# microsoft/SEAL

Hardware: AMD Instinct MI355X
Metric: CKKS multiply+relinearize+rescale ciphertexts/sec @ N=2^16, L=16 (higher is better)
Workload: dtype u64

## Files before the change

include/sealhip.h:

```cpp
#ifndef SEALHIP_H
#define SEALHIP_H

#include <stdbool.h>
#include <stddef.h>
#include <stdint.h>

#ifdef __cplusplus
extern "C" {
#endif

typedef long SHL_HRESULT;
#define SHL_S_OK ((SHL_HRESULT)0L)
#define SHL_S_FALSE ((SHL_HRESULT)1L)
#define SHL_E_POINTER ((SHL_HRESULT)0x80004003L)
#define SHL_E_INVALIDARG ((SHL_HRESULT)0x80070057L)
#define SHL_E_OUTOFMEMORY ((SHL_HRESULT)0x8007000EL)
#define SHL_E_UNEXPECTED ((SHL_HRESULT)0x8000FFFFL)
#define SHL_COR_E_IO ((SHL_HRESULT)0x80131620L)
#define SHL_COR_E_INVALIDOPERATION ((SHL_HRESULT)0x80131509L)
#define SHL_E_INVALID_INDEX ((SHL_HRESULT)0x80070585L)

#define SHL_FUNC SHL_HRESULT


// ... 195 lines not shown
SHL_FUNC ItemMap_Info(void *thisptr, uint64_t *rows, uint64_t *terms, uint64_t *longest_row, uint64_t *first_batch, uint64_t *second_batch);
SHL_FUNC Evaluator_SumItemsMapped(void *thisptr, void *encrypted, void *item_map, void *destination);
SHL_FUNC Evaluator_DotPlainMapped(void *thisptr, void *encrypted, const uint64_t *device_plain, uint64_t plain_count, void *item_map,
                                  double scale, void *destination);
SHL_FUNC Evaluator_DotItemsMapped(void *thisptr, void *encrypted1, void *encrypted2, void *item_map, void *destination);
SHL_FUNC CKKSEncoder_EncodeScalars(void *thisptr, uint64_t count, const double *values, uint64_t *parms_id, double scale, uint64_t *device_words);
SHL_FUNC CKKSEncoder_EncodeIntegerScalars(void *thisptr, uint64_t count, const int64_t *values, uint64_t *parms_id, uint64_t *device_words);
SHL_FUNC Evaluator_LiftScalars(void *thisptr, uint64_t count, const uint64_t *values_mod_t, uint64_t *parms_id, uint64_t *device_words);
SHL_FUNC Evaluator_DotScalarsDevice(void *thisptr, void *encrypted, const uint64_t *device_scalars, uint64_t rows, uint64_t batch, double scale,
                                    void *destination);
SHL_FUNC Evaluator_Square(void *thisptr, void *encrypted, void *destination, void *pool);
SHL_FUNC Evaluator_Relinearize(void *thisptr, void *encrypted, void *relinKeys, void *destination, void *pool);
SHL_FUNC Evaluator_ModSwitchToNext1(void *thisptr, void *encrypted, void *destination, void *pool);
SHL_FUNC Evaluator_ModSwitchTo1(void *thisptr, void *encrypted, uint64_t *parms_id, void *destination, void *pool);
SHL_FUNC Evaluator_RescaleToNext(void *thisptr, void *encrypted, void *destination, void *pool);
SHL_FUNC Evaluator_RescaleTo(void *thisptr, void *encrypted, uint64_t *parms_id, void *destination, void *pool);
SHL_FUNC Evaluator_ModReduceToNext(void *thisptr, void *encrypted, void *destination, void *pool);
SHL_FUNC Evaluator_ModReduceTo(void *thisptr, void *encrypted, uint64_t *parms_id, void *destination, void *pool);
SHL_FUNC Evaluator_TransformToNTT2(void *thisptr, void *encrypted, void *destination_ntt);
SHL_FUNC Evaluator_TransformFromNTT(void *thisptr, void *encrypted_ntt, void *destination);
SHL_FUNC Evaluator_ApplyGalois(void *thisptr, void *encrypted, uint32_t galois_elt, void *galoisKeys, void *destination, void *pool);
SHL_FUNC Evaluator_RotateRows(void *thisptr, void *encrypted, int steps, void *galoisKeys, void *destination, void *pool);
SHL_FUNC Evaluator_RotateColumns(void *thisptr, void *encrypted, void *galois_keys, void *destination, void *pool);
SHL_FUNC Evaluator_RotateVector(void *thisptr, void *encrypted, int steps, void *galoisKeys, void *destination, void *pool);
SHL_FUNC Evaluator_ComplexConjugate(void *thisptr, void *encrypted, void *galoisKeys, void *destination, void *pool);
SHL_FUNC Evaluator_ContextUsingKeyswitching(void *thisptr, bool *using_keyswitching);

SHL_FUNC Evaluator_SwitchKeyAccWords(void *thisptr, void *encrypted, uint64_t *words);
SHL_FUNC Evaluator_RelinearizePartial(void *thisptr, void *encrypted , void *relinKeys, uint64_t digit_first,
                                      uint64_t digit_count, uint64_t *device_acc);
SHL_FUNC Evaluator_RelinearizeFinish(void *thisptr, void *encrypted, uint64_t *device_acc, uint64_t parts);
SHL_FUNC Evaluator_ApplyGaloisPartial(void *thisptr, void *encrypted , uint32_t galois_elt, void *galoisKeys,
                                      uint64_t digit_first, uint64_t digit_count, uint64_t *device_acc);
SHL_FUNC Evaluator_ApplyGaloisFinish(void *thisptr, void *encrypted, uint64_t *device_acc, uint64_t parts);

SHL_FUNC Comm_GetUniqueId(uint8_t *id128);
SHL_FUNC Comm_RcclAvailable(bool *available);
SHL_FUNC Comm_Create(const uint8_t *id128, int nranks, int rank, void **comm);
SHL_FUNC Comm_Destroy(void *comm);
SHL_FUNC Comm_Info(void *comm, int *nranks, int *rank, bool *loopback);
SHL_FUNC Comm_DigitRange(void *comm, uint64_t digits, uint64_t *first, uint64_t *count);
SHL_FUNC Comm_AllReduceWords(void *comm, uint64_t *device_words, uint64_t count, void *hip_stream);
SHL_FUNC Comm_BroadcastWords(void *comm, uint64_t *device_words, uint64_t count, int root, void *hip_stream);
SHL_FUNC Evaluator_RelinearizeDigitParallel(void *thisptr, void *encrypted, void *relinKeys, void *comm, int exchange, void *destination);
SHL_FUNC Evaluator_ApplyGaloisDigitParallel(void *thisptr, void *encrypted, uint32_t galois_elt, void *galoisKeys, void *comm, int exchange,
                                            void *destination);
SHL_FUNC Evaluator_RotateVectorDigitParallel(void *thisptr, void *encrypted, int steps, void *galoisKeys, void *comm, int exchange,
                                             void *destination);
SHL_FUNC Evaluator_BroadcastKeyDigits(void *thisptr, void *kswitch_keys, uint64_t index, uint64_t *device_staging, void *comm, int root);
SHL_FUNC Evaluator_SwitchKeySlots(void *thisptr, void *encrypted, uint64_t nranks, uint64_t *slots);
SHL_FUNC Evaluator_SwitchKeyPackTargets(void *thisptr, void *encrypted, const uint64_t *device_acc, uint64_t nranks, uint64_t *device_send,
                                        uint64_t *device_special);
SHL_FUNC Evaluator_SwitchKeyFinishOwned(void *thisptr, void *encrypted, const uint64_t *device_recv, const uint64_t *device_special,
                                        uint64_t nranks, uint64_t rank, uint64_t *device_own);
SHL_FUNC Evaluator_SwitchKeyAddGathered(void *thisptr, void *encrypted, const uint64_t *device_all, uint64_t nranks);


SHL_FUNC shl_ntt_forward(void *context, uint64_t *data, uint64_t polys, uint64_t comps, uint64_t first_prime, int lazy, void *stream);
SHL_FUNC shl_ntt_inverse(void *context, uint64_t *data, uint64_t polys, uint64_t comps, uint64_t first_prime, int lazy, void *stream);
SHL_FUNC shl_dyadic_product(void *context, const uint64_t *a, const uint64_t *b, uint64_t *r, uint64_t polys, uint64_t comps, uint64_t first_prime, void *stream);
SHL_FUNC shl_reduce_items(void *context, uint64_t chain_index, const uint64_t *a, const uint64_t *plain, uint64_t *r, uint64_t size,
                          uint64_t batch, uint64_t group, uint64_t slices, uint64_t *scratch, uint64_t *slices_used, void *stream);
SHL_FUNC shl_reduce_flush_intervals(uint64_t *sum_terms, uint64_t *dot_terms);
SHL_FUNC shl_dot_items(void *context, uint64_t chain_index, const uint64_t *x, const uint64_t *y, uint64_t *r, uint64_t batch,
                       uint64_t group, uint64_t slices, uint64_t *scratch, uint64_t *slices_used, void *stream);
SHL_FUNC shl_dot_items_flush_interval(uint64_t *items);
SHL_FUNC shl_reduce_mapped(void *context, uint64_t chain_index, int kind, const uint64_t *a, uint64_t a_batch, const uint64_t *b,
                           uint64_t b_batch, uint64_t *r, uint64_t size, void *item_map, uint64_t slices, uint64_t *scratch,
                           uint64_t *slices_used, void *stream);
SHL_FUNC shl_dot_scalars(void *context, uint64_t chain_index, const uint64_t *a, const uint64_t *scalars, uint64_t *r, uint64_t size,
                         uint64_t rows, uint64_t batch, uint64_t slices, uint64_t *slices_used);
SHL_FUNC shl_dot_scalars_tile(void *context, uint64_t chain_index, const uint64_t *a, const uint64_t *scalars, uint64_t *r, uint64_t size,
                              uint64_t rows, uint64_t batch, uint64_t slices, uint64_t *slices_used, uint64_t row_tile, void *stream);
SHL_FUNC shl_dot_scalars_info(uint64_t *row_tile, uint64_t *flush);
SHL_FUNC shl_apply_galois(void *context, uint64_t chain_index, int ntt_form, uint32_t galois_elt, const uint64_t *in, uint64_t *out, uint64_t polys, void *stream);
SHL_FUNC shl_rns_stage(void *context, uint64_t chain_index, int which, const uint64_t *in, uint64_t *out, uint64_t polys, void *stream);
SHL_FUNC Ciphertext_Create4(void *context, uint64_t *parms_id, void *pool, void **cipher);
SHL_FUNC Ciphertext_Create5(void *context, uint64_t *parms_id, uint64_t capacity, void *pool, void **cipher);
SHL_FUNC Ciphertext_Reserve1(void *thisptr, void *context, uint64_t *parms_id, uint64_t size_capacity);
SHL_FUNC Ciphertext_Reserve2(void *thisptr, void *context, uint64_t size_capacity);
SHL_FUNC Ciphertext_Reserve3(void *thisptr, uint64_t size_capacity);
SHL_FUNC Ciphertext_SizeCapacity(void *thisptr, uint64_t *size_capacity);
SHL_FUNC Ciphertext_SetParmsId(void *thisptr, uint64_t *parms_id);
SHL_FUNC Ciphertext_Resize2(void *thisptr, void *context, uint64_t size);
SHL_FUNC Ciphertext_Resize3(void *thisptr, uint64_t size);
SHL_FUNC Ciphertext_Resize4(void *thisptr, uint64_t size, uint64_t polyModulusDegree, uint64_t coeffModCount);
SHL_FUNC Ciphertext_GetDataAt1(void *thisptr, uint64_t index, uint64_t *data);
SHL_FUNC Ciphertext_GetDataAt2(void *thisptr, uint64_t poly_index, uint64_t coeff_index, uint64_t *data);
SHL_FUNC Ciphertext_SetDataAt(void *thisptr, uint64_t index, uint64_t value);
SHL_FUNC Ciphertext_Release(void *thisptr);
SHL_FUNC KSwitchKeys_Create2(void *copy, void **kswitch_keys);
SHL_FUNC KSwitchKeys_Set(void *thisptr, void *assign);
SHL_FUNC KSwitchKeys_RawSize(void *thisptr, uint64_t *key_count);
SHL_FUNC KSwitchKeys_GetKeyList(void *thisptr, uint64_t index, uint64_t *count, void **key_list);
SHL_FUNC KSwitchKeys_ClearDataAndReserve(void *thisptr, uint64_t size);
SHL_FUNC KSwitchKeys_AddKeyList(void *thisptr, uint64_t count, void **key_list);
SHL_FUNC KSwitchKeys_GetParmsId(void *thisptr, uint64_t *parms_id);
SHL_FUNC KSwitchKeys_SetParmsId(void *thisptr, uint64_t *parms_id);
SHL_FUNC SEALContext_ParametersSet(void *thisptr, bool *params_set);
SHL_FUNC SEALContext_ParameterErrorName(void *thisptr, char *outstr, uint64_t *length);
SHL_FUNC SEALContext_ParameterErrorMessage(void *thisptr, char *outstr, uint64_t *length);
SHL_FUNC SEALContext_KeyContextData(void *thisptr, void **context_data);
SHL_FUNC SEALContext_FirstContextData(void *thisptr, void **context_data);
SHL_FUNC SEALContext_LastContextData(void *thisptr, void **context_data);
SHL_FUNC SEALContext_GetContextData(void *thisptr, uint64_t *parms_id, void **context_data);
SHL_FUNC ContextData_Destroy(void *thisptr);
SHL_FUNC ContextData_TotalCoeffModulus(void *thisptr, uint64_t *count, uint64_t *total_coeff_modulus);
SHL_FUNC ContextData_TotalCoeffModulusBitCount(void *thisptr, int *bit_count);
SHL_FUNC ContextData_Parms(void *thisptr, void **parms);
SHL_FUNC ContextData_Qualifiers(void *thisptr, void **epq);
SHL_FUNC ContextData_CoeffDivPlainModulus(void *thisptr, uint64_t *count, uint64_t *coeff_div);
SHL_FUNC ContextData_PlainUpperHalfThreshold(void *thisptr, uint64_t *puht);
SHL_FUNC ContextData_PlainUpperHalfIncrement(void *thisptr, uint64_t *count, uint64_t *puhi);
SHL_FUNC ContextData_UpperHalfThreshold(void *thisptr, uint64_t *count, uint64_t *uht);
SHL_FUNC ContextData_UpperHalfIncrement(void *thisptr, uint64_t *count, uint64_t *uhi);
SHL_FUNC ContextData_PrevContextData(void *thisptr, void **prev_data);
SHL_FUNC ContextData_NextContextData(void *thisptr, void **next_data);
SHL_FUNC ContextData_ChainIndex(void *thisptr, uint64_t *index);
SHL_FUNC ContextData_ParmsId(void *thisptr, uint64_t *parms_id);
SHL_FUNC EPQ_Destroy(void *thisptr);
SHL_FUNC EPQ_ParametersSet(void *thisptr, bool *parameters_set);
SHL_FUNC EPQ_UsingFFT(void *thisptr, bool *using_fft);
SHL_FUNC EPQ_UsingNTT(void *thisptr, bool *using_ntt);
SHL_FUNC EPQ_UsingBatching(void *thisptr, bool *using_batching);
SHL_FUNC EPQ_UsingFastPlainLift(void *thisptr, bool *using_fast_plain_lift);
SHL_FUNC EPQ_UsingDescendingModulusChain(void *thisptr, bool *using_descending_modulus_chain);
SHL_FUNC EPQ_SecLevel(void *thisptr, int *sec_level);
SHL_FUNC EncParams_Create2(void *copy, void **enc_params);
SHL_FUNC EncParams_Set(void *thisptr, void *assign);
SHL_FUNC EncParams_GetParmsId(void *thisptr, uint64_t *parms_id);
SHL_FUNC EncParams_GetPlainModulus(void *thisptr, uint64_t *plain_modulus);
SHL_FUNC EncParams_Equals(void *thisptr, void *otherptr, bool *result);
SHL_FUNC EncParams_SaveSize(void *thisptr, uint8_t compr_mode, int64_t *result);
SHL_FUNC EncParams_Save(void *thisptr, uint8_t *outptr, uint64_t size, uint8_t compr_mode, int64_t *out_bytes);
SHL_FUNC EncParams_Load(void *thisptr, uint8_t *inptr, uint64_t size, int64_t *in_bytes);
SHL_FUNC SecretKey_Create2(void *copy, void **secret_key);
SHL_FUNC SecretKey_Assign(void *thisptr, void *assign);
SHL_FUNC SecretKey_ParmsId(void *thisptr, uint64_t *parms_id);
SHL_FUNC SecretKey_SaveSize(void *thisptr, uint8_t compr_mode, int64_t *result);
SHL_FUNC SecretKey_Save(void *thisptr, uint8_t *outptr, uint64_t size, uint8_t compr_mode, int64_t *out_bytes);
SHL_FUNC PublicKey_Create2(void *copy, void **public_key);
SHL_FUNC PublicKey_Assign(void *thisptr, void *assign);
SHL_FUNC PublicKey_ParmsId(void *thisptr, uint64_t *parms_id);
SHL_FUNC PublicKey_SaveSize(void *thisptr, uint8_t compr_mode, int64_t *result);
SHL_FUNC PublicKey_Save(void *thisptr, uint8_t *outptr, uint64_t size, uint8_t compr_mode, int64_t *out_bytes);
SHL_FUNC SealHip_ReleasePool(void);
SHL_FUNC SealHip_SetStagedHostCopies(bool enabled);
SHL_FUNC SealHip_PoolStats(uint64_t *bytes_held, uint64_t *cross_stream_waits);
SHL_FUNC SealHip_InstallAbortTrace(const char *path);
SHL_FUNC SealHip_KsChunkStats(uint64_t *calls, uint64_t *chunks, uint64_t *scratch_bytes_max);
SHL_FUNC SealHip_TailStats(uint64_t *folded, uint64_t *plain, uint64_t *dropped);
SHL_FUNC SealHip_ProductStats(uint64_t *fused, uint64_t *formed, uint64_t *dropped);
SHL_FUNC SealHip_GaloisStats(uint64_t *gathered, uint64_t *permuted);
SHL_FUNC SealHip_XofStats(uint64_t *polynomials, uint64_t *replaced_words, uint64_t *host_walk_ns, uint64_t *total_ns);
SHL_FUNC shl_device_count(int *count);
SHL_FUNC shl_set_device(int device);
SHL_FUNC shl_stream_create(bool non_blocking, void **hip_stream);
SHL_FUNC shl_stream_destroy(void *hip_stream);
SHL_FUNC shl_malloc(uint64_t bytes, void **device_ptr);
SHL_FUNC shl_free(void *device_ptr);
SHL_FUNC shl_memcpy_h2d(void *device_dst, const void *host_src, uint64_t bytes);
SHL_FUNC KeyGenerator_Create1(void *context, const uint64_t *seed8, void **key_generator);
SHL_FUNC KeyGenerator_Create2(void *context, void *secret_key, const uint64_t *seed8, void **key_generator);
SHL_FUNC KeyGenerator_Destroy(void *thisptr);
SHL_FUNC KeyGenerator_SecretKey(void *thisptr, void *secret_key);
SHL_FUNC KeyGenerator_CreatePublicKey(void *thisptr, void *public_key);
SHL_FUNC KeyGenerator_CreateRelinKeys(void *thisptr, void *relin_keys);
SHL_FUNC KeyGenerator_CreateGaloisKeysFromElts(void *thisptr, uint64_t count, const uint32_t *galois_elts, void *galois_keys);
SHL_FUNC KeyGenerator_CreateGaloisKeysFromSteps(void *thisptr, uint64_t count, const int *steps, void *galois_keys);
SHL_FUNC KeyGenerator_CreateGaloisKeysAll(void *thisptr, void *galois_keys);
SHL_FUNC KeyGenerator_SeededSaveSize(void *thisptr, bool galois, uint64_t key_count, int64_t *result);
SHL_FUNC KeyGenerator_CreateRelinKeysSave(void *thisptr, uint8_t *outptr, uint64_t size, int64_t *out_bytes);
SHL_FUNC KeyGenerator_CreateGaloisKeysFromEltsSave(void *thisptr, uint64_t count, const uint32_t *galois_elts, uint8_t *outptr, uint64_t size,
                                                   int64_t *out_bytes);
SHL_FUNC KeyGenerator_KeyToHost(void *thisptr, uint32_t galois_elt, uint64_t *host_words, uint64_t capacity_words);
SHL_FUNC SecretKey_Get(void *thisptr, uint64_t *host_words);
SHL_FUNC PublicKey_Get(void *thisptr, uint64_t *host_words);
SHL_FUNC shl_memcpy_d2h(void *host_dst, const void *device_src, uint64_t bytes);
SHL_FUNC shl_device_synchronize(void);
SHL_FUNC shl_timer_create(void **timer);
SHL_FUNC shl_timer_destroy(void *timer);
SHL_FUNC shl_timer_start(void *timer, void *stream);
SHL_FUNC shl_timer_stop(void *timer, void *stream, float *milliseconds);

#ifdef __cplusplus
}
#endif
#endif
```

seal_amd/__init__.py:

```python
from .api import (CoeffModulus, PlainModulus, EncryptionParameters, SEALContext, ContextData, Ciphertext, Plaintext, KSwitchKeys,
                  RelinKeys, GaloisKeys, Evaluator, SecretKey, PublicKey, KeyGenerator, Decryptor, Encryptor, BatchEncoder, CKKSEncoder, Graph, ItemMap, DeviceBuffer, HipTimer, ntt_forward, ntt_inverse,
                  dyadic_product, apply_galois, rns_stage, device_synchronize, device_info, release_pool, pool_stats, tail_stats, product_stats, galois_stats, ks_chunk_stats, xof_stats, Stream, Comm, device_count, set_device,
                  set_staged_host_copies, install_abort_trace)
from ._native import SealHipError, InvalidArgument, LogicError, OutOfRange, DeviceError, load

__all__ = [
    "CoeffModulus", "PlainModulus", "EncryptionParameters", "SEALContext", "ContextData", "Ciphertext", "Plaintext", "KSwitchKeys",
    "RelinKeys", "GaloisKeys", "Evaluator", "SecretKey", "PublicKey", "KeyGenerator", "Decryptor", "Encryptor", "BatchEncoder", "CKKSEncoder", "Graph", "ItemMap", "DeviceBuffer", "HipTimer", "ntt_forward", "ntt_inverse",
    "dyadic_product", "apply_galois", "rns_stage", "device_synchronize", "device_info", "release_pool", "pool_stats", "tail_stats", "product_stats", "galois_stats", "ks_chunk_stats", "xof_stats", "Stream", "Comm", "device_count", "set_device", "set_staged_host_copies", "install_abort_trace", "SealHipError",
    "InvalidArgument", "LogicError", "OutOfRange", "DeviceError", "load",
]
```

seal_amd/_native.py:

```python
import ctypes as C
import os

_HERE = os.path.dirname(os.path.abspath(__file__))
DEFAULT_LIB = os.path.join(_HERE, "lib", "libsealhip.so")

S_OK = 0
E_POINTER = 0x80004003
E_INVALIDARG = 0x80070057
E_OUTOFMEMORY = 0x8007000E
E_UNEXPECTED = 0x8000FFFF
COR_E_IO = 0x80131620
COR_E_INVALIDOPERATION = 0x80131509
E_INVALID_INDEX = 0x80070585


class SealHipError(Exception):

    def __init__(self, hr, message):
        super().__init__("%s (HRESULT 0x%08X)" % (message, hr & 0xFFFFFFFF))
        self.hresult = hr & 0xFFFFFFFF
        self.message = message


class InvalidArgument(SealHipError, ValueError):
    pass


class LogicError(SealHipError, RuntimeError):
    pass


class OutOfRange(SealHipError, IndexError):
    pass


class DeviceError(SealHipError, OSError):
    pass


_ERR = {E_INVALIDARG: InvalidArgument, COR_E_INVALIDOPERATION: LogicError, E_INVALID_INDEX: OutOfRange,
        COR_E_IO: DeviceError}

SYMBOLS = """
SealHip_Version SealHip_DeviceInfo SealHip_LastError CoeffModulus_Create1 PlainModulus_Batching
EncParams_Create1 EncParams_Destroy EncParams_SetPolyModulusDegree EncParams_GetPolyModulusDegree
EncParams_SetCoeffModulus EncParams_GetCoeffModulus EncParams_SetPlainModulus2 EncParams_GetScheme
SEALContext_Create SEALContext_Destroy SEALContext_KeyParmsId SEALContext_FirstParmsId SEALContext_LastParmsId
SEALContext_UsingKeyswitching SEALContext_ChainIndex SEALContext_ParmsIdAt SEALContext_CoeffModulusAt
SEALContext_TotalCoeffModulusBitCount SEALContext_SetParmsId SEALContext_NTTRoot SEALContext_BaseBsk
Ciphertext_Create3 Ciphertext_CreateBatch Ciphertext_Create2 Ciphertext_Set Ciphertext_Destroy Ciphertext_Resize1
Ciphertext_Size Ciphertext_BatchCount Ciphertext_PolyModulusDegree Ciphertext_CoeffModulusSize Ciphertext_ParmsId
Ciphertext_IsNTTForm Ciphertext_SetIsNTTForm Ciphertext_Scale Ciphertext_SetScale Ciphertext_CorrectionFactor
Ciphertext_SetCorrectionFactor Ciphertext_IsTransparent Ciphertext_DevicePtr Ciphertext_CopyFromHost
Ciphertext_CopyToHost Ciphertext_CopyWordsToHost Ciphertext_CopyFromDevice
Ciphertext_SaveSize Ciphertext_Save Ciphertext_UnsafeLoad Ciphertext_Load Ciphertext_LoadItem Ciphertext_SaveItem
KSwitchKeys_UnsafeLoad KSwitchKeys_Load KSwitchKeys_SaveSize KSwitchKeys_Save
KeyGenerator_Create1 KeyGenerator_Create2 KeyGenerator_Destroy KeyGenerator_SecretKey KeyGenerator_CreatePublicKey
KeyGenerator_CreateRelinKeys KeyGenerator_CreateGaloisKeysFromSteps KeyGenerator_CreateGaloisKeysAll KeyGenerator_CreateGaloisKeysFromElts KeyGenerator_KeyToHost KeyGenerator_SeededSaveSize KeyGenerator_CreateRelinKeysSave KeyGenerator_CreateGaloisKeysFromEltsSave SecretKey_Get PublicKey_Get
SecretKey_Create SecretKey_Destroy SecretKey_Set SecretKey_UnsafeLoad SecretKey_Load Decryptor_Create Decryptor_Destroy
Decryptor_Decrypt Decryptor_InvariantNoiseBudget Decryptor_DecryptBatchWords Decryptor_DecryptBatch
CKKSEncoder_Create CKKSEncoder_Destroy CKKSEncoder_SlotCount CKKSEncoder_Encode1 CKKSEncoder_Encode2 CKKSEncoder_Encode3 CKKSEncoder_Encode4 CKKSEncoder_Encode5 CKKSEncoder_Decode1 CKKSEncoder_Decode2
CKKSEncoder_EncodeDevice CKKSEncoder_DecodeDevice
BatchEncoder_Create BatchEncoder_Destroy BatchEncoder_GetSlotCount BatchEncoder_Encode1 BatchEncoder_Encode2 BatchEncoder_Decode1
BatchEncoder_Decode2 BatchEncoder_EncodeDevice BatchEncoder_DecodeDevice
PublicKey_Create PublicKey_Destroy PublicKey_Set PublicKey_UnsafeLoad PublicKey_Load Encryptor_Encrypt Encryptor_EncryptZero1 Encryptor_EncryptZero2 Encryptor_EncryptZeroSymmetric2
Encryptor_Create Encryptor_Destroy Encryptor_SetSeed Encryptor_EncryptZeroSymmetric1 Encryptor_EncryptSymmetric
Encryptor_SymmetricSaveSize Encryptor_EncryptZeroSymmetricSave Encryptor_EncryptSymmetricSave
Encryptor_EncryptSymmetricDevice Encryptor_EncryptDevice
Plaintext_Create1 Plaintext_Create5 Plaintext_Destroy Plaintext_Set4 Plaintext_SetFromDevice Plaintext_CoeffCount
Plaintext_IsNTTForm Plaintext_GetParmsId Plaintext_SetParmsId Plaintext_Scale Plaintext_SetScale Plaintext_CopyToHost
Plaintext_SaveSize Plaintext_Save Plaintext_UnsafeLoad Plaintext_Load
Evaluator_AddMany Evaluator_AddPlain Evaluator_SubPlain Evaluator_MultiplyMany Evaluator_MultiplyPlain Evaluator_Exponentiate
Evaluator_TransformToNTT1 Evaluator_ModSwitchToNext2 Evaluator_ModSwitchTo2
Evaluator_AddPlainDevice Evaluator_SubPlainDevice Evaluator_MultiplyPlainDevice Evaluator_TransformPlainToNTTDevice
Evaluator_SumItems Evaluator_DotPlainDevice shl_reduce_items shl_reduce_flush_intervals
Evaluator_DotItems shl_dot_items shl_dot_items_flush_interval
ItemMap_Create ItemMap_Destroy ItemMap_Info Evaluator_SumItemsMapped Evaluator_DotPlainMapped Evaluator_DotItemsMapped shl_reduce_mapped
CKKSEncoder_EncodeScalars CKKSEncoder_EncodeIntegerScalars Evaluator_LiftScalars Evaluator_DotScalarsDevice
shl_dot_scalars shl_dot_scalars_tile shl_dot_scalars_info
KSwitchKeys_Create1 KSwitchKeys_Destroy KSwitchKeys_Size KSwitchKeys_SetKey KSwitchKeys_SetKeyFromDevice
KSwitchKeys_SetKeyDigits KSwitchKeys_HasKey KSwitchKeys_DeviceBytes RelinKeys_GetIndex GaloisKeys_GetIndex GaloisTool_GetEltFromStep
Evaluator_Create Evaluator_Destroy Evaluator_SetStream Evaluator_Synchronize Evaluator_CopyTo Evaluator_SetTransparentCheck
Evaluator_BeginCapture Evaluator_EndCapture Evaluator_LaunchGraph Graph_Destroy
Evaluator_Negate Evaluator_Add Evaluator_Sub Evaluator_Multiply Evaluator_Square Evaluator_Relinearize
Evaluator_ModSwitchToNext1 Evaluator_ModSwitchTo1 Evaluator_RescaleToNext Evaluator_RescaleTo
Evaluator_ModReduceToNext Evaluator_ModReduceTo Evaluator_TransformToNTT2 Evaluator_TransformFromNTT Evaluator_ApplyGalois
Evaluator_RotateRows Evaluator_RotateColumns Evaluator_RotateVector Evaluator_ComplexConjugate
Evaluator_ContextUsingKeyswitching
Evaluator_SwitchKeyAccWords Evaluator_RelinearizePartial Evaluator_RelinearizeFinish Evaluator_ApplyGaloisPartial
Evaluator_ApplyGaloisFinish
Comm_GetUniqueId Comm_RcclAvailable Comm_Create Comm_Destroy Comm_Info Comm_DigitRange Comm_AllReduceWords Comm_BroadcastWords
Evaluator_RelinearizeDigitParallel Evaluator_ApplyGaloisDigitParallel Evaluator_RotateVectorDigitParallel
Evaluator_BroadcastKeyDigits Evaluator_SwitchKeySlots Evaluator_SwitchKeyPackTargets Evaluator_SwitchKeyFinishOwned
Evaluator_SwitchKeyAddGathered
SealHip_ReleasePool SealHip_PoolStats SealHip_TailStats SealHip_ProductStats SealHip_GaloisStats SealHip_XofStats SealHip_KsChunkStats SealHip_SetStagedHostCopies SealHip_InstallAbortTrace shl_stream_create shl_stream_destroy shl_device_count shl_set_device
shl_ntt_forward shl_ntt_inverse shl_dyadic_product shl_apply_galois shl_rns_stage shl_malloc shl_free
shl_memcpy_h2d shl_memcpy_d2h shl_device_synchronize shl_timer_create shl_timer_destroy shl_timer_start
shl_timer_stop
Ciphertext_Create4 Ciphertext_Create5 Ciphertext_GetDataAt1 Ciphertext_GetDataAt2 Ciphertext_Release Ciphertext_Reserve1
Ciphertext_Reserve2 Ciphertext_Reserve3 Ciphertext_Resize2 Ciphertext_Resize3 Ciphertext_Resize4 Ciphertext_SetDataAt
Ciphertext_SetParmsId Ciphertext_SizeCapacity ContextData_ChainIndex ContextData_CoeffDivPlainModulus ContextData_Destroy ContextData_NextContextData
ContextData_Parms ContextData_ParmsId ContextData_PlainUpperHalfIncrement ContextData_PlainUpperHalfThreshold ContextData_PrevContextData ContextData_Qualifiers
ContextData_TotalCoeffModulus ContextData_TotalCoeffModulusBitCount ContextData_UpperHalfIncrement ContextData_UpperHalfThreshold EPQ_Destroy EPQ_ParametersSet
EPQ_SecLevel EPQ_UsingBatching EPQ_UsingDescendingModulusChain EPQ_UsingFFT EPQ_UsingFastPlainLift EPQ_UsingNTT
EncParams_Create2 EncParams_Equals EncParams_GetParmsId EncParams_GetPlainModulus EncParams_Load EncParams_Save
EncParams_SaveSize EncParams_Set KSwitchKeys_AddKeyList KSwitchKeys_ClearDataAndReserve KSwitchKeys_Create2 KSwitchKeys_GetKeyList
KSwitchKeys_GetParmsId KSwitchKeys_RawSize KSwitchKeys_Set KSwitchKeys_SetParmsId PublicKey_Assign PublicKey_Create2
PublicKey_ParmsId PublicKey_Save PublicKey_SaveSize SEALContext_FirstContextData SEALContext_GetContextData SEALContext_KeyContextData
SEALContext_LastContextData SEALContext_ParameterErrorMessage SEALContext_ParameterErrorName SEALContext_ParametersSet SecretKey_Assign SecretKey_Create2
SecretKey_ParmsId SecretKey_Save SecretKey_SaveSize
""".split()

_lib = None
_lib_path = None


def load(path=None):
    global _lib, _lib_path
    want = os.path.abspath(path or DEFAULT_LIB)
    if _lib is not None and _lib_path == want:
        return _lib
    if not os.path.exists(want):
        raise ImportError(
            "seal_amd: %s not found. Build it with `python -c 'import __graft_entry__ as g; g.build()'` "
            "(hipcc --offload-arch=gfx950). There is no CPU fallback." % want)
    lib = C.CDLL(want)
    for name in SYMBOLS:
        getattr(lib, name).restype = C.c_long
    _lib, _lib_path = lib, want
    return lib


def lib():
    return _lib if _lib is not None else load()


def check(hr):
    hr &= 0xFFFFFFFF
    if hr == S_OK:
        return
    n = C.c_uint64(0)
    lib().SealHip_LastError(None, C.byref(n))
    buf = C.create_string_buffer(max(int(n.value), 1))
    lib().SealHip_LastError(buf, C.byref(n))
    cls = _ERR.get(hr, SealHipError)
    if hr == E_OUTOFMEMORY:
        raise MemoryError(buf.value.decode())
    raise cls(hr, buf.value.decode(errors="replace"))
```

seal_amd/api.py:

```python
import ctypes as C
import os

import numpy as np

from . import _native as N

SCHEME = {"none": 0, "bfv": 1, "ckks": 2, "bgv": 3}


def _p(a):
    return a.ctypes.data_as(C.c_void_p)


class CoeffModulus:
    @staticmethod
    def Create(poly_modulus_degree, bit_sizes):
        bits = (C.c_int * len(bit_sizes))(*bit_sizes)
        out = np.zeros(len(bit_sizes), dtype=np.uint64)
        N.check(N.lib().CoeffModulus_Create1(C.c_uint64(poly_modulus_degree), C.c_uint64(len(bit_sizes)), bits, _p(out)))
        return [int(x) for x in out]


class PlainModulus:
    @staticmethod
# ... 1569 lines not shown
        N.check(N.lib().Comm_AllReduceWords(self._h, C.c_void_p(device_ptr), C.c_uint64(words), C.c_void_p(stream or 0)))

    def broadcast(self, device_ptr, words, root=0, stream=None):
        N.check(N.lib().Comm_BroadcastWords(self._h, C.c_void_p(device_ptr), C.c_uint64(words), C.c_int(root), C.c_void_p(stream or 0)))


class DeviceBuffer:

    def __init__(self, words):
        self.words = int(words)
        self._ptr = C.c_void_p()
        N.check(N.lib().shl_malloc(C.c_uint64(self.words * 8), C.byref(self._ptr)))

    def __del__(self):
        if getattr(self, "_ptr", None) and self._ptr.value:
            N.lib().shl_free(self._ptr)
            self._ptr = None

    @property
    def ptr(self):
        return self._ptr.value

    @staticmethod
    def from_numpy(a):
        a = np.ascontiguousarray(a, dtype=np.uint64)
        b = DeviceBuffer(a.size)
        N.check(N.lib().shl_memcpy_h2d(b._ptr, _p(a), C.c_uint64(a.size * 8)))
        return b

    def to_numpy(self, shape):
        out = np.zeros(shape, dtype=np.uint64)
        N.check(N.lib().shl_memcpy_d2h(_p(out), self._ptr, C.c_uint64(out.size * 8)))
        return out

    @staticmethod
    def from_array(a):
        a = np.ascontiguousarray(a)
        if a.dtype.itemsize not in (8, 16):
            raise TypeError("from_array takes 8-byte or complex128 elements, not %s" % a.dtype)
        b = DeviceBuffer(max(a.nbytes // 8, 1))
        N.check(N.lib().shl_memcpy_h2d(b._ptr, _p(a), C.c_uint64(a.nbytes)))
        return b

    def to_array(self, shape, dtype=np.float64):
        out = np.zeros(shape, dtype=dtype)
        N.check(N.lib().shl_memcpy_d2h(_p(out), self._ptr, C.c_uint64(out.nbytes)))
        return out


def ntt_forward(context, buf, polys, comps, first_prime=0, lazy=False, stream=None):
    N.check(N.lib().shl_ntt_forward(context._h, C.c_void_p(buf.ptr), C.c_uint64(polys), C.c_uint64(comps),
                                    C.c_uint64(first_prime), C.c_int(int(lazy)), C.c_void_p(stream or 0)))


def ntt_inverse(context, buf, polys, comps, first_prime=0, lazy=False, stream=None):
    N.check(N.lib().shl_ntt_inverse(context._h, C.c_void_p(buf.ptr), C.c_uint64(polys), C.c_uint64(comps),
                                    C.c_uint64(first_prime), C.c_int(int(lazy)), C.c_void_p(stream or 0)))


def dyadic_product(context, a, b, r, polys, comps, first_prime=0, stream=None):
    N.check(N.lib().shl_dyadic_product(context._h, C.c_void_p(a.ptr), C.c_void_p(b.ptr), C.c_void_p(r.ptr),
                                       C.c_uint64(polys), C.c_uint64(comps), C.c_uint64(first_prime),
                                       C.c_void_p(stream or 0)))


def apply_galois(context, chain_index, ntt_form, galois_elt, src, dst, polys, stream=None):
    N.check(N.lib().shl_apply_galois(context._h, C.c_uint64(chain_index), C.c_int(int(ntt_form)), C.c_uint32(galois_elt),
                                     C.c_void_p(src.ptr), C.c_void_p(dst.ptr), C.c_uint64(polys), C.c_void_p(stream or 0)))


RNS_STAGE = {"fastbconv_m_tilde": 0, "sm_mrq": 1, "fast_floor": 2, "fastbconv_sk": 3,
             "divide_and_round_q_last": 4, "divide_and_round_q_last_ntt": 5}


def rns_stage(context, chain_index, which, src, dst, polys, stream=None):
    N.check(N.lib().shl_rns_stage(context._h, C.c_uint64(chain_index), C.c_int(RNS_STAGE[which]), C.c_void_p(src.ptr),
                                  C.c_void_p(dst.ptr), C.c_uint64(polys), C.c_void_p(stream or 0)))


class Stream:

    def __init__(self, non_blocking=True):
        self._h = C.c_void_p()
        N.check(N.lib().shl_stream_create(C.c_bool(non_blocking), C.byref(self._h)))

    @property
    def handle(self):
        return self._h.value

    def __del__(self):
        if getattr(self, "_h", None) and self._h.value:
            N.lib().shl_stream_destroy(self._h)
            self._h = None


def device_count():
    n = C.c_int()
    N.check(N.lib().shl_device_count(C.byref(n)))
    return n.value


def set_device(index):
    N.check(N.lib().shl_set_device(C.c_int(index)))


def release_pool():
    N.check(N.lib().SealHip_ReleasePool())


def set_staged_host_copies(enabled):
    N.check(N.lib().SealHip_SetStagedHostCopies(C.c_bool(enabled)))


def install_abort_trace(path):
    N.check(N.lib().SealHip_InstallAbortTrace(C.c_char_p(os.fsencode(path))))


def pool_stats():
    a, b = C.c_uint64(), C.c_uint64()
    N.check(N.lib().SealHip_PoolStats(C.byref(a), C.byref(b)))
    return a.value, b.value


def tail_stats():
    a, b, c = C.c_uint64(), C.c_uint64(), C.c_uint64()
    N.check(N.lib().SealHip_TailStats(C.byref(a), C.byref(b), C.byref(c)))
    return a.value, b.value, c.value


def product_stats():
    a, b, c = C.c_uint64(), C.c_uint64(), C.c_uint64()
    N.check(N.lib().SealHip_ProductStats(C.byref(a), C.byref(b), C.byref(c)))
    return a.value, b.value, c.value


def galois_stats():
    a, b = C.c_uint64(), C.c_uint64()
    N.check(N.lib().SealHip_GaloisStats(C.byref(a), C.byref(b)))
    return a.value, b.value


def xof_stats():
    v = [C.c_uint64() for _ in range(4)]
    N.check(N.lib().SealHip_XofStats(*[C.byref(x) for x in v]))
    return tuple(x.value for x in v)


def ks_chunk_stats():
    a, b, c = C.c_uint64(), C.c_uint64(), C.c_uint64()
    N.check(N.lib().SealHip_KsChunkStats(C.byref(a), C.byref(b), C.byref(c)))
    return a.value, b.value, c.value


def device_synchronize():
    N.check(N.lib().shl_device_synchronize())


def device_info():
    name = C.create_string_buffer(256)
    cus = C.c_int()
    mem = C.c_uint64()
    N.check(N.lib().SealHip_DeviceInfo(name, C.c_uint64(256), C.byref(cus), C.byref(mem)))
    return name.value.decode(), cus.value, mem.value


class HipTimer:

    def __init__(self):
        self._h = C.c_void_p()
        N.check(N.lib().shl_timer_create(C.byref(self._h)))

    def __del__(self):
        if getattr(self, "_h", None):
            N.lib().shl_timer_destroy(self._h)
            self._h = None

    def start(self, stream=None):
        N.check(N.lib().shl_timer_start(self._h, C.c_void_p(stream or 0)))

    def stop(self, stream=None):
        ms = C.c_float()
        N.check(N.lib().shl_timer_stop(self._h, C.c_void_p(stream or 0), C.byref(ms)))
        return ms.value
```

seal_amd/csrc/capi_kernels.cpp:

```cpp
#include "capi_common.h"
#include "batch_reduce_kernels.h"
#include <memory>

namespace
{
    template <class Launch>
    SHL_HRESULT raw_reduce(void *context, uint64_t chain_index, const char *shape_error, uint64_t grid_planes, uint64_t out_items,
                           const ItemWalk &walk, uint64_t slices, uint64_t *slices_used, const uint64_t *r, bool operands,
                           const uint64_t *scratch, Launch launch)
    {
        IfNullRet(context, SHL_E_POINTER);
        SHL_TRY
        auto c = as<Context>(context);
        auto l = c->level_by_chain_index(chain_index);
        if (!l)
            throw std::out_of_range("chain_index");
        if (shape_error)
            throw std::invalid_argument(shape_error);
        const size_t words = (size_t)l->K * c->n();
        if (!slices)
            slices = batch_reduce_slices(grid_planes * out_items * words / 2, walk);
        if (slices > walk.longest || slices > 64)
            throw std::invalid_argument("1 <= slices <= min(group or longest row, 64)");
        if (slices_used)
// ... 180 lines not shown
        if (hr != SHL_S_OK || !r)
            return hr;
        SHL_TRY
        hip_ok(hipStreamSynchronize(nullptr), "dot_scalars sync");
        SHL_CATCH
    }
    SHL_FUNC shl_dot_scalars_info(uint64_t *row_tile, uint64_t *flush)
    {
        IfNullRet(row_tile, SHL_E_POINTER);
        IfNullRet(flush, SHL_E_POINTER);
        *row_tile = dot_scalars_row_tile();
        *flush = batch_reduce_dot_flush();
        return SHL_S_OK;
    }
    SHL_FUNC shl_apply_galois(
        void *context, uint64_t chain_index, int ntt_form, uint32_t galois_elt, const uint64_t *in, uint64_t *out, uint64_t polys,
        void *stream)
    {
        IfNullRet(context, SHL_E_POINTER);
        IfNullRet(in, SHL_E_POINTER);
        IfNullRet(out, SHL_E_POINTER);
        SHL_TRY
        auto c = as<Context>(context);
        auto l = c->level_by_chain_index(chain_index);
        if (!l)
            throw std::out_of_range("chain_index");
        if (!(galois_elt & 1) || galois_elt >= 2 * c->n())
            throw std::invalid_argument("Galois element is not valid");
        if (in == out)
            throw std::invalid_argument("result cannot point to the same value as operand");
        PlaneGeom g{ (unsigned)c->log_n(), l->K, (unsigned)polys };
        hip_ok(k_apply_galois(c->dev_mods(), in, out, galois_elt, ntt_form, g, 1, (hipStream_t)stream), "apply_galois");
        SHL_CATCH
    }
    SHL_FUNC shl_rns_stage(void *context, uint64_t chain_index, int which, const uint64_t *in, uint64_t *out, uint64_t polys, void *stream)
    {
        IfNullRet(context, SHL_E_POINTER);
        IfNullRet(in, SHL_E_POINTER);
        IfNullRet(out, SHL_E_POINTER);
        SHL_TRY
        auto c = as<Context>(context);
        auto l = c->level_by_chain_index(chain_index);
        if (!l)
            throw std::out_of_range("chain_index");
        hipStream_t s = (hipStream_t)stream;
        const unsigned n_log = (unsigned)c->log_n();
        if (which >= 0 && which <= 3)
        {
            if (c->scheme() != Scheme::bfv)
                throw std::logic_error("BEHZ stages exist only for BFV contexts");
            hip_ok(k_behz_stage(c->dev_mods(), l->dev, which, in, out, n_log, polys, s), "behz stage");
        }
        else if (which == 4)
        {
            if (l->K < 2)
                throw std::invalid_argument("level has a single modulus");
            hip_ok(k_bfv_modswitch(c->dev_mods(), l->dev, in, out, n_log, polys, s), "divide_and_round_q_last");
        }
        else if (which == 5)
        {
            if (l->K < 2)
                throw std::invalid_argument("level has a single modulus");
            const unsigned K = l->K;
            const size_t N = c->n();
            Scratch copy(polys * K * N), tt(polys * (K - 1) * N);
            hip_ok(hipMemcpyAsync(copy.p, in, polys * K * N * 8, hipMemcpyDeviceToDevice, s), "copy");
            uint64_t *last = copy.p + (size_t)(K - 1) * N;
            NttBatch bi{};
            bi.data = last;
            bi.outer_stride = (size_t)K * N;
            bi.ncomp = 1;
            bi.nouter = (unsigned)polys;
            bi.prime_first = K - 1;
            hip_ok(ntt_inverse(c->ntt_tables(), bi, 0, s), "intt last");
            NttBatch b{};
            b.data = tt.p;
            b.outer_stride = (size_t)(K - 1) * N;
            b.ncomp = K - 1;
            b.nouter = (unsigned)polys;
            b.src = last;
            b.src_outer_stride = (size_t)K * N;
            b.src_ncomp = 1;
            b.src_mode = 2;
            b.src_half = l->dev.half_q_last;
            b.src_q = l->dev.q_last;
            b.src_fix = l->dev.round_fix;
            hip_ok(ntt_forward(c->ntt_tables(), b, 1, s), "ntt correction");
            hip_ok(k_rescale_combine(c->dev_mods(), l->dev.inv_q_last_mod_q, copy.p, tt.p, out, n_log, K, polys, s), "combine");
            hip_ok(hipStreamSynchronize(s), "sync");
        }
        else
            throw std::invalid_argument("unknown stage");
        SHL_CATCH
    }
    SHL_FUNC SealHip_SetStagedHostCopies(bool enabled)
    {
        set_staged_host_copies(enabled);
        return SHL_S_OK;
    }
    SHL_FUNC SealHip_ReleasePool(void)
    {
        SHL_TRY
        DevicePool::global().release_all();
        SHL_CATCH
    }
    SHL_FUNC SealHip_PoolStats(uint64_t *bytes_held, uint64_t *cross_stream_waits)
    {
        SHL_TRY
        if (bytes_held)
            *bytes_held = DevicePool::global().bytes_held();
        if (cross_stream_waits)
            *cross_stream_waits = DevicePool::global().cross_stream_waits();
        SHL_CATCH
    }
    SHL_FUNC SealHip_KsChunkStats(uint64_t *calls, uint64_t *chunks, uint64_t *scratch_bytes_max)
    {
        SHL_TRY
        uint64_t w = 0;
        ks_chunk_stats(calls, chunks, &w);
        if (scratch_bytes_max)
            *scratch_bytes_max = w * 8;
        SHL_CATCH
    }
    SHL_FUNC SealHip_XofStats(uint64_t *polynomials, uint64_t *replaced_words, uint64_t *host_walk_ns, uint64_t *total_ns)
    {
        SHL_TRY
        xof_stats(polynomials, replaced_words, host_walk_ns, total_ns);
        SHL_CATCH
    }
    SHL_FUNC SealHip_ProductStats(uint64_t *fused, uint64_t *formed, uint64_t *dropped)
    {
        SHL_TRY
        uint64_t f, p, d;
        lazy_product_stats(f, p, d);
        if (fused)
            *fused = f;
        if (formed)
            *formed = p;
        if (dropped)
            *dropped = d;
        SHL_CATCH
    }
    SHL_FUNC SealHip_GaloisStats(uint64_t *gathered, uint64_t *permuted)
    {
        SHL_TRY
        uint64_t g, p;
        galois_path_stats(g, p);
        if (gathered)
            *gathered = g;
        if (permuted)
            *permuted = p;
        SHL_CATCH
    }
    SHL_FUNC SealHip_TailStats(uint64_t *folded, uint64_t *plain, uint64_t *dropped)
    {
        SHL_TRY
        uint64_t f, p, d;
        lazy_tail_stats(f, p, d);
        if (folded)
            *folded = f;
        if (plain)
            *plain = p;
        if (dropped)
            *dropped = d;
        SHL_CATCH
    }
    SHL_FUNC shl_device_count(int *count)
    {
        IfNullRet(count, SHL_E_POINTER);
        SHL_TRY
        *count = 0;
        if (hipGetDeviceCount(count) != hipSuccess)
            *count = 0;
        SHL_CATCH
    }
    SHL_FUNC shl_set_device(int device)
    {
        SHL_TRY
        hip_ok(hipSetDevice(device), "hipSetDevice");
        SHL_CATCH
    }
    SHL_FUNC shl_stream_create(bool non_blocking, void **hip_stream)
    {
        IfNullRet(hip_stream, SHL_E_POINTER);
        SHL_TRY
        hipStream_t s = nullptr;
        hip_ok(hipStreamCreateWithFlags(&s, non_blocking ? hipStreamNonBlocking : hipStreamDefault), "hipStreamCreateWithFlags");
        *hip_stream = s;
        SHL_CATCH
    }
    SHL_FUNC shl_stream_destroy(void *hip_stream)
    {
        SHL_TRY
        hip_ok(hipStreamSynchronize((hipStream_t)hip_stream), "hipStreamSynchronize");
        hip_ok(hipStreamDestroy((hipStream_t)hip_stream), "hipStreamDestroy");
        SHL_CATCH
    }
    SHL_FUNC shl_malloc(uint64_t bytes, void **device_ptr)
    {
        IfNullRet(device_ptr, SHL_E_POINTER);
        SHL_TRY
        if (hipMalloc(device_ptr, bytes) != hipSuccess)
            throw std::bad_alloc();
        SHL_CATCH
    }
    SHL_FUNC shl_free(void *device_ptr)
    {
        SHL_TRY
        hip_ok(hipFree(device_ptr), "hipFree");
        SHL_CATCH
    }
    SHL_FUNC shl_memcpy_h2d(void *device_dst, const void *host_src, uint64_t bytes)
    {
        SHL_TRY
        hip_ok(hipMemcpy(device_dst, host_src, bytes, hipMemcpyHostToDevice), "H2D");
        SHL_CATCH
    }
    SHL_FUNC shl_memcpy_d2h(void *host_dst, const void *device_src, uint64_t bytes)
    {
        SHL_TRY
        hip_ok(hipDeviceSynchronize(), "sync");
        hip_ok(hipMemcpy(host_dst, device_src, bytes, hipMemcpyDeviceToHost), "D2H");
        SHL_CATCH
    }
    SHL_FUNC shl_device_synchronize(void)
    {
        SHL_TRY
        hip_ok(hipDeviceSynchronize(), "hipDeviceSynchronize");
        SHL_CATCH
    }
    SHL_FUNC shl_timer_create(void **timer)
    {
        IfNullRet(timer, SHL_E_POINTER);
        SHL_TRY
        auto t = new Timer();
        hip_ok(hipEventCreate(&t->e0), "hipEventCreate");
        hip_ok(hipEventCreate(&t->e1), "hipEventCreate");
        *timer = t;
        SHL_CATCH
    }
    SHL_FUNC shl_timer_destroy(void *timer)
    {
        IfNullRet(timer, SHL_E_POINTER);
        auto t = as<Timer>(timer);
        (void)hipEventDestroy(t->e0);
        (void)hipEventDestroy(t->e1);
        delete t;
        return SHL_S_OK;
    }
    SHL_FUNC shl_timer_start(void *timer, void *stream)
    {
        IfNullRet(timer, SHL_E_POINTER);
        SHL_TRY
        hip_ok(hipEventRecord(as<Timer>(timer)->e0, (hipStream_t)stream), "hipEventRecord");
        SHL_CATCH
    }
    SHL_FUNC shl_timer_stop(void *timer, void *stream, float *milliseconds)
    {
        IfNullRet(timer, SHL_E_POINTER);
        IfNullRet(milliseconds, SHL_E_POINTER);
        SHL_TRY
        auto t = as<Timer>(timer);
        hip_ok(hipEventRecord(t->e1, (hipStream_t)stream), "hipEventRecord");
        hip_ok(hipEventSynchronize(t->e1), "hipEventSynchronize");
        hip_ok(hipEventElapsedTime(milliseconds, t->e0, t->e1), "hipEventElapsedTime");
        SHL_CATCH
    }
}
```

seal_amd/csrc/evaluator.h:

```cpp
#pragma once
#include "context.h"
#include "poly_kernels.h"
#include "pool.h"
#include "comm.h"
#include "ntt2_kernels.h"
#include <functional>
#include <map>
#include <memory>
#include <mutex>
#include <stdexcept>
#include <vector>

namespace sealhip
{
    class Evaluator;
    struct LazyTail
    {
        const Evaluator *owner;
        uint64_t *acc;
        bool with_addend = false;
    };
    class Ciphertext;
    struct LazyProduct
    {
        const Evaluator *owner;
        const Ciphertext *x, *y;
        uint64_t *own;
        const uint64_t *xw() const;
        const uint64_t *yw() const;
    };
    void lazy_product_stats(uint64_t &fused, uint64_t &formed, uint64_t &dropped);
    void galois_path_stats(uint64_t &gathered, uint64_t &permuted);
    void lazy_tail_stats(uint64_t &folded, uint64_t &plain, uint64_t &dropped);
    void ks_chunk_stats(uint64_t *calls, uint64_t *chunks, uint64_t *scratch_words_max);

    struct KsPlan
    {
        unsigned chunk;
        unsigned lanes;
        unsigned chunks(unsigned batch) const { return (batch + chunk - 1) / chunk; }
    };
    struct KsRoute
    {
        bool fused = false;
        unsigned split = 1;
        bool fold = false;
        bool defer = false;
        KsPlan plan{ 0, 1 };
        unsigned j0 = 0, j1 = 0;
        bool takes_product() const { return fused && fold && split == 1; }
        bool reads_through_map() const;
    };
    struct KsAddend
    {
        bool folds = false;
        bool c1_zero = false;
        uint32_t galois_elt = 0;
        const uint64_t *c0 = nullptr;
        const LazyProduct *prod = nullptr;
        static KsAddend nothing() { return {}; }
        static KsAddend planes(bool c1_zero_unwritten = false) { return { true, c1_zero_unwritten, 0, nullptr, nullptr }; }
        static KsAddend galois(uint32_t elt, const uint64_t *operand_c0) { return { true, true, elt, operand_c0, nullptr }; }
        static KsAddend product(const LazyProduct &p) { return { true, false, 0, nullptr, &p }; }
    };

    class Ciphertext
    {
    public:
        explicit Ciphertext(const Context &ctx, size_t batch = 1) : ctx_(&ctx), batch_(batch ? batch : 1) {}
        ~Ciphertext();
        Ciphertext(const Ciphertext &o);
        Ciphertext &operator=(const Ciphertext &o);

        const Context &context() const { return *ctx_; }
        size_t batch() const { return batch_; }
        size_t size() const { return size_; }
        const Level *level() const { return level_; }
        size_t coeff_modulus_size() const { return level_ ? level_->K : 0; }
        size_t poly_modulus_degree() const { return level_ ? ctx_->n() : 0; }
        bool &is_ntt_form() { return is_ntt_form_; }
        bool is_ntt_form() const { return is_ntt_form_; }
        double &scale() { return scale_; }
        double scale() const { return scale_; }
        uint64_t &correction_factor() { return correction_factor_; }
        uint64_t correction_factor() const { return correction_factor_; }
        uint64_t *data()
        {
            settle();
            before_write();
            return data_;
        }
        const uint64_t *data() const
        {
            settle();
            return data_;
        }
        size_t plane_words() const { return level_ ? batch_ * level_->K * ctx_->n() : 0; }
        size_t word_count() const { return size_ * plane_words(); }
        uint64_t *plane(size_t p) { return data() + p * plane_words(); }
        const uint64_t *plane(size_t p) const { return data() + p * plane_words(); }
        bool has_lazy_tail() const { return lazy_ != nullptr; }
        bool has_lazy_product() const { return lazy_prod_ != nullptr; }
        bool has_storage() const { return data_ != nullptr; }

        void resize(const Level *level, size_t size, hipStream_t stream);
        void adopt(const Level *level, size_t size, uint64_t *slab, size_t capacity_words);
        void reshape_uninitialized(const Level *level, size_t size);
        size_t capacity_words() const { return capacity_words_; }
        void release();
        void reserve(const Level *level, size_t size_capacity, hipStream_t stream);
        size_t size_capacity() const { return plane_words() ? capacity_words_ / plane_words() : 0; }
        void set_level_unchecked(const Level *level)
        {
            settle();
            before_write();
            level_ = level;
        }

    private:
        const Context *ctx_;
        size_t batch_;
        size_t size_ = 0;
        const Level *level_ = nullptr;
        bool is_ntt_form_ = false;
        double scale_ = 1.0;
        uint64_t correction_factor_ = 1;
        uint64_t *data_ = nullptr;
        size_t capacity_words_ = 0;
        mutable LazyTail *lazy_ = nullptr;
        void settle() const;
        void drop_lazy();
        mutable LazyProduct *lazy_prod_ = nullptr;
        mutable std::vector<const Ciphertext *> prod_readers_;
        mutable unsigned prod_reader_count_ = 0;
        void settle_product() const;
        void drop_product();
        void before_write() const
        {
            if (__atomic_load_n(&prod_reader_count_, __ATOMIC_ACQUIRE))
                settle_readers();
        }
        void settle_readers() const;
        uint64_t *exchange_slab(const Level *level, size_t size, uint64_t *slab, size_t capacity_words);
        friend class Evaluator;
        friend struct LazyProduct;
        friend void lazy_product_link(const Ciphertext *, const LazyProduct &);
        friend void lazy_product_unlink(const Ciphertext *, const LazyProduct &);
    };

    void lazy_product_link(const Ciphertext *dest, const LazyProduct &p);
    void lazy_product_unlink(const Ciphertext *dest, const LazyProduct &p);

    class Plaintext
    {
    public:
        explicit Plaintext(const Context &ctx) : ctx_(&ctx) {}
        ~Plaintext();
        Plaintext(const Plaintext &o);
        Plaintext &operator=(const Plaintext &o);

        const Context &context() const { return *ctx_; }
        size_t coeff_count() const { return coeff_count_; }
        const Level *level() const { return level_; }
        void set_level(const Level *l) { level_ = l; }
        bool is_ntt_form() const { return level_ != nullptr; }
        double &scale() { return scale_; }
        double scale() const { return scale_; }
        uint64_t *data() { return data_; }
        const uint64_t *data() const { return data_; }
        void resize(size_t coeff_count, hipStream_t stream);
        void set(const uint64_t *words, size_t count, bool from_device);
        void adopt(uint64_t *slab, size_t count, size_t capacity_words);
        void adopt_count(size_t count) { coeff_count_ = count; }

    private:
        const Context *ctx_;
        size_t coeff_count_ = 0;
        const Level *level_ = nullptr;
        double scale_ = 1.0;
        uint64_t *data_ = nullptr;
        size_t capacity_words_ = 0;
    };

    class KSwitchKeys
    {
    public:
        struct Key
        {
            uint64_t *dev = nullptr;
            size_t digits = 0;
            size_t digit0 = 0;
            bool register_order = false;
        };
        ~KSwitchKeys();
        void set_key(const Context &ctx, size_t index, size_t digits, const uint64_t *words, bool from_device, size_t digit0 = 0);
        void set_key_with(const Context &ctx, size_t index, size_t digits, const std::function<void(uint64_t *)> &upload, size_t digit0 = 0);
        void key_words(size_t index, uint64_t *device_out) const;
        void digit_words(size_t index, size_t digit, uint64_t *device_out) const;
        size_t device_bytes() const;
        void clear();
        bool has_key(size_t index) const { return index < keys_.size() && keys_[index].dev != nullptr; }
        const Key &key(size_t index) const { return keys_[index]; }
// ... 237 lines not shown
```

seal_amd/csrc/evaluator_common.h:

```cpp
#pragma once
#include "evaluator.h"
#include "plain_batch_kernels.h"
#include <atomic>
#include <cmath>
#include <cstdio>
#include <cstdlib>
#include <algorithm>
#include <cstring>
#include <limits>

namespace sealhip
{
    namespace
    {
        void ck(hipError_t e, const char *what)
        {
            if (e != hipSuccess)
                throw std::runtime_error(std::string("HIP failure in ") + what + ": " + hipGetErrorString(e));
        }

        bool are_close(double a, double b)
        {
            double scale_factor = std::max({ std::fabs(a), std::fabs(b), 1.0 });
            return std::fabs(a - b) < std::numeric_limits<double>::epsilon() * scale_factor;
        }

        std::vector<int> naf(int value)
        {
            std::vector<int> res;
            bool sign = value < 0;
            value = std::abs(value);
            for (int i = 0; value; i++)
            {
                int zi = (value & 1) ? 2 - (value & 3) : 0;
                value = (value - zi) >> 1;
                if (zi)
                    res.push_back((sign ? -zi : zi) * (1 << i));
            }
            return res;
        }

        void balance_correction_factors(uint64_t factor1, uint64_t factor2, uint64_t t, uint64_t &f, uint64_t &e1, uint64_t &e2)
        {
            const uint64_t c1 = factor1 % t, c2 = factor2 % t;
            if (c1 == 0 || std::__gcd(c1, t) != 1)
                throw std::logic_error("invalid correction factor1");
            const uint64_t rho = host::mulmod(host::invmod(c1, t), c2, t);
            const auto residue = [t](int64_t v) {
                const uint64_t m = static_cast<uint64_t>(v < 0 ? -v : v) % t;
                return (v < 0 && m) ? t - m : m;
            };
            const auto centred_abs = [t](uint64_t x) {
                return static_cast<int64_t>(x > t / 2 ? t - x : x);
            };
            struct Row
            {
                int64_t r, s;
            };
            Row above{ static_cast<int64_t>(t), 0 }, here{ static_cast<int64_t>(rho), 1 };
            e1 = rho;
            e2 = 1;
            int64_t best = centred_abs(e1) + centred_abs(e2);
            while (here.r != 0)
            {
                const int64_t quot = above.r / here.r;
                const Row below{ above.r - quot * here.r, above.s - quot * here.s };
                above = here;
                here = below;
                const uint64_t r = residue(here.r), sc = residue(here.s);
                if (r == 0 || std::__gcd(r, t) != 1)
                    continue;
                const int64_t norm = centred_abs(r) + centred_abs(sc);
                if (norm < best)
                {
                    best = norm;
                    e1 = r;
                    e2 = sc;
                }
            }
            f = host::mulmod(e1, c1, t);
        }

        bool words_overlap(const void *a, size_t a_bytes, const void *b, size_t b_bytes)
        {
            const uintptr_t a0 = (uintptr_t)a, b0 = (uintptr_t)b;
            return a_bytes && b_bytes && a0 < b0 + b_bytes && b0 < a0 + a_bytes;
        }
        BfvPlainConst bfv_plain_const(const Context &ctx, const Level &lvl)
        {
            return BfvPlainConst{ host::make_mod(ctx.plain_modulus()), lvl.dev.q_mod_t, lvl.dev.plain_upper_half_threshold, lvl.dev.delta_mod_q };
        }

        NttBatch plain_batch(uint64_t *data, size_t outer_stride, unsigned ncomp, unsigned nouter, unsigned prime_first)
        {
            NttBatch b{};
            b.data = data;
            b.outer_stride = outer_stride;
            b.ncomp = ncomp;
            b.nouter = nouter;
            b.comp_prime = nullptr;
            b.prime_first = prime_first;
            b.src = nullptr;
            return b;
        }
    }

    struct KsSwitches
    {
        bool eager_tail, no_fold, class_fork, trace, galois_kernels, skip_tensor;
        static unsigned split(unsigned chosen);
        static unsigned chunk(unsigned chosen);
        static unsigned lanes();
        static unsigned scratch_cap_mib();
        static bool lazy_product();
        static bool lazy_product_min_wgs(size_t &min_wgs);
    };
    const KsSwitches &ks_switches();

    extern std::atomic<uint64_t> g_tail_folded, g_tail_plain, g_tail_dropped;
}
```

seal_amd/csrc/evaluator_keyswitch.cpp:

```cpp
#include "evaluator_common.h"
#include <map>
#include <memory>

namespace sealhip
{
    namespace
    {
        KsPlan ks_plan(unsigned batch, size_t words_per_item, size_t wgs_per_item, bool may_chunk, bool may_lane)
        {
            KsPlan p{ batch, 1 };
            if (!may_chunk || batch < 2)
                return p;
            unsigned chunk = (unsigned)((8192 + wgs_per_item - 1) / (wgs_per_item ? wgs_per_item : 1));
            chunk = KsSwitches::chunk(chunk < 8 ? 8 : chunk);
            unsigned lanes = KsSwitches::lanes();
            if (lanes < 1 || !may_lane)
                lanes = 1;
            if (lanes > 4)
                lanes = 4;
            if (chunk == 0 || 2 * chunk > batch + chunk / 2)
                return p;
            const double cap = (double)KsSwitches::scratch_cap_mib() * 1048576.0;
            while (chunk > 1 && (double)lanes * chunk * words_per_item * 8.0 > cap)
            {
                if (lanes > 2)
                    lanes--;
                else
                    chunk = (chunk + 1) / 2;
            }
            p.chunk = chunk;
            p.lanes = lanes;
            if (p.chunks(batch) < p.lanes)
                p.lanes = p.chunks(batch);
            return p;
        }
        struct KsLanes
        {
            static constexpr unsigned kSide = 3;
            hipStream_t stream[kSide] = { nullptr, nullptr, nullptr };
            hipEvent_t join[kSide] = { nullptr, nullptr, nullptr };
            hipEvent_t fork = nullptr;
            unsigned made = 0;
            int device = -1;
            KsLanes() = default;
            KsLanes(const KsLanes &) = delete;
            KsLanes &operator=(const KsLanes &) = delete;
            ~KsLanes()
            {
                for (unsigned i = 0; i < kSide; i++)
                {
                    if (stream[i])
                        (void)hipStreamDestroy(stream[i]);
                    if (join[i])
                        (void)hipEventDestroy(join[i]);
                }
                if (fork)
                    (void)hipEventDestroy(fork);
            }
            bool ensure(unsigned side)
            {
                if (!fork && hipEventCreateWithFlags(&fork, hipEventDisableTiming) != hipSuccess)
                    return false;
                while (made < side && made < kSide)
                {
                    hipStream_t st = nullptr;
                    hipEvent_t ev = nullptr;
                    if (hipStreamCreateWithFlags(&st, hipStreamNonBlocking) != hipSuccess)
                        return false;
                    if (hipEventCreateWithFlags(&ev, hipEventDisableTiming) != hipSuccess)
                    {
                        (void)hipStreamDestroy(st);
                        return false;
                    }
                    stream[made] = st;
                    join[made] = ev;
                    made++;
                }
                return made >= side;
            }
        };
        KsLanes *ks_lanes()
        {
            static thread_local std::map<int, std::unique_ptr<KsLanes>> sets;
            int dev = -1;
            if (hipGetDevice(&dev) != hipSuccess)
                return nullptr;
            std::unique_ptr<KsLanes> &slot = sets[dev];
            if (!slot)
            {
                slot.reset(new KsLanes());
                slot->device = dev;
            }
            return slot.get();
        }
        std::atomic<uint64_t> g_ks_chunked_calls{ 0 }, g_ks_chunks{ 0 }, g_ks_scratch_words_max{ 0 };
    }
    void ks_chunk_stats(uint64_t *calls, uint64_t *chunks, uint64_t *scratch_words_max)
    {
        if (calls)
            *calls = g_ks_chunked_calls.load();
        if (chunks)
            *chunks = g_ks_chunks.load();
        if (scratch_words_max)
            *scratch_words_max = g_ks_scratch_words_max.exchange(0);
    }

    const KsSwitches &ks_switches()
    {
        static const KsSwitches sw{ std::getenv("SEALHIP_KS_EAGER_TAIL") != nullptr,   shl_ab_getenv("SEALHIP_KS_NO_FOLD") != nullptr,
                                    shl_ab_getenv("SEALHIP_KS_CLASS_FORK") != nullptr, shl_ab_getenv("SEALHIP_KS_TRACE") != nullptr,
                                    shl_ab_getenv("SEALHIP_GALOIS_KERNELS") != nullptr, shl_ab_getenv("SEALHIP_AB_SKIP_TENSOR") != nullptr };
        return sw;
    }
    static unsigned env_unsigned(const char *name, unsigned fallback)
    {
        const char *v = std::getenv(name);
        return v && *v ? (unsigned)std::strtoul(v, nullptr, 10) : fallback;
    }
    unsigned KsSwitches::split(unsigned chosen)
    {
        const char *v = std::getenv("SEALHIP_KS_SPLIT");
        return v ? (unsigned)std::atoi(v) : chosen;
    }
    unsigned KsSwitches::chunk(unsigned chosen) { return env_unsigned("SEALHIP_KS_CHUNK", chosen); }
    unsigned KsSwitches::lanes() { return env_unsigned("SEALHIP_KS_LANES", 3); }
    unsigned KsSwitches::scratch_cap_mib() { return env_unsigned("SEALHIP_KS_SCRATCH_CAP_MIB", 16384); }
    bool KsSwitches::lazy_product()
    {
        const char *v = std::getenv("SEALHIP_LAZY_PRODUCT");
        return !(v && std::atoi(v) == 0);
    }
    bool KsSwitches::lazy_product_min_wgs(size_t &min_wgs)
    {
        const char *v = std::getenv("SEALHIP_LAZY_PRODUCT_MIN_WGS");
        if (v)
            min_wgs = (size_t)std::atol(v);
        return v != nullptr;
    }

    unsigned Evaluator::ks_shape_split(const Level &lvl, size_t batch) const
    {
        const size_t wgs = batch * (size_t)(lvl.K + 1) * (context_.n() >> 12);
        return (unsigned)(2048 / (wgs ? wgs : 1));
    }
    KsRoute Evaluator::ks_route(const Level &lvl, size_t batch) const
    {
        const KsSwitches &sw = ks_switches();
        const Scheme sch = context_.scheme();
        KsRoute r;
        r.defer = !sw.eager_tail && (sch == Scheme::ckks || sch == Scheme::bfv) && ntt2_supports(context_.log_n()) && lvl.K >= 2;
        r.fold = r.defer && !sw.no_fold && sch == Scheme::ckks;
        r.plan = KsPlan{ (unsigned)batch, 1 };
        return r;
    }
    KsRoute Evaluator::ks_route(const Level &lvl, size_t batch, const KSwitchKeys &keys, size_t key_index, unsigned j0, unsigned j1,
                                bool digit_parallel) const
    {
        const unsigned K = lvl.K;
        KsRoute r = ks_route(lvl, batch);
        r.j0 = j0;
        r.j1 = j1;
        r.fused = keys.context() == &context_ && key_index < keys.slots() && keys.has_key(key_index) && keys.key(key_index).register_order;
        r.fold = r.fold && r.fused && !digit_parallel;
        if (!r.fused)
            return r;
        if (!digit_parallel)
        {
            const unsigned shape = ks_shape_split(lvl, batch);
            r.split = KsSwitches::split(shape > 4 ? 4 : shape);
            r.split = std::max(1u, std::min({ r.split, 8u, K }));
        }
        r.plan = ks_plan((unsigned)batch, (size_t)(K + 1) * K * context_.n(), (size_t)(K + 1) * (context_.n() >> 12), r.split == 1, !capturing_);
        return r;
    }
    bool KsRoute::reads_through_map() const { return takes_product() && !ks_switches().galois_kernels; }

    void Evaluator::relinearize_inplace(Ciphertext &e, const KSwitchKeys &relin_keys) const
    {
        StreamScope pool_scope(stream_);
        if (&e.context() != &context_ || !e.level())
            throw std::invalid_argument("encrypted is not valid for encryption parameters");
        if (relin_keys.context() != &context_)
            throw std::invalid_argument("relin_keys is not valid for encryption parameters");
        size_t size = e.size();
        const size_t destination_size = 2;
        if (destination_size > size)
            throw std::invalid_argument("destination_size must be at least 2 and less than or equal to current count");
        if (relin_keys.size() < size - 2)
            throw std::invalid_argument("not enough relinearization keys");
        if (destination_size == size)
            return;
        if (size == 3 && e.has_lazy_product() && relinearize_from_product(e, relin_keys))
            return;
        size_t relins_needed = size - destination_size;
        for (size_t I = 0; I < relins_needed; I++)
        {
            const size_t key_index = relin_index(size - 1 - I);
            switch_key_inplace(e, e.plane(size - 1), relin_keys, key_index, ks_route(*e.level(), e.batch(), relin_keys, key_index, 0, e.level()->K));
        }
        e.resize(e.level(), destination_size, stream_);
        throw_if_transparent(e);
    }

    void lazy_product_count_fused();
    bool Evaluator::relinearize_from_product(Ciphertext &e, const KSwitchKeys &relin_keys) const
    {
        const size_t key_index = relin_index(2);
        const LazyProduct *pending = e.lazy_prod_;
        const unsigned K = e.level()->K;
        const KsRoute route = ks_route(*e.level(), e.batch(), relin_keys, key_index, 0, K);
        if (!pending || pending->owner != this || capturing_ || !e.is_ntt_form() || !context_.using_keyswitching() || !route.takes_product())
            return false;
        const KSwitchKeys::Key &key = relin_keys.key(key_index);
        if (key.digit0 != 0 || key.digits < K)
            return false;
        const LazyProduct p = detach_product(e);
        lazy_product_count_fused();
        uint64_t *target = e.data_ + 2 * e.plane_words();
        StreamScope pool_scope(stream_);
        try
        {
            Scratch acc(switch_key_acc_words(e));
            switch_key_partial(e, target, relin_keys, key_index, acc.p, route, KsAddend::product(p));
            defer_tail(e, acc.release(), true);
        }
        catch (...)
        {
            try
            {
                PlaneGeom g{ (unsigned)context_.log_n(), K, (unsigned)e.batch() };
                (void)k_ckks_multiply_2x2(context_.dev_mods(), context_.ntt_tables().fpd, nullptr, p.xw(), p.yw(), e.data_, g, stream_);
            }
            catch (...)
            {
            }
            DevicePool::global().free_words(p.own, stream_);
            throw;
        }
        DevicePool::global().free_words(p.own, stream_);
        e.resize(e.level(), 2, stream_);
        throw_if_transparent(e);
        return true;
    }

    void Evaluator::relinearize_partial(Ciphertext &e, const KSwitchKeys &relin_keys, unsigned j0, unsigned j1, uint64_t *acc) const
    {
        StreamScope pool_scope(stream_);
        if (&e.context() != &context_ || !e.level())
            throw std::invalid_argument("encrypted is not valid for encryption parameters");
        if (relin_keys.context() != &context_ && !(j0 == j1 && !relin_keys.context()))
            throw std::invalid_argument("relin_keys is not valid for encryption parameters");
        if (e.size() != 3)
            throw std::invalid_argument("digit-parallel relinearization takes a size-3 ciphertext");
        switch_key_partial(e, e.plane(2), relin_keys, relin_index(2), acc, ks_route(*e.level(), e.batch(), relin_keys, relin_index(2), j0, j1, true));
    }
    void Evaluator::relinearize_finish(Ciphertext &e, uint64_t *acc, unsigned parts) const
    {
        StreamScope pool_scope(stream_);
        if (&e.context() != &context_ || !e.level() || e.size() != 3)
            throw std::invalid_argument("encrypted is not valid for encryption parameters");
        switch_key_finish(e, acc, parts, false, true);
        e.resize(e.level(), 2, stream_);
        throw_if_transparent(e);
    }
    void Evaluator::apply_galois_partial(
        Ciphertext &e, uint32_t galois_elt, const KSwitchKeys &galois_keys, unsigned j0, unsigned j1, uint64_t *acc) const
    {
        StreamScope pool_scope(stream_);
        check_valid(e, "encrypted");
        if (galois_keys.context() != &context_ && !(j0 == j1 && !galois_keys.context()))
            throw std::invalid_argument("galois_keys is not valid for encryption parameters");
        uint64_t m = 2 * (uint64_t)context_.n();
        if (!(galois_elt & 1) || galois_elt >= m)
            throw std::invalid_argument("Galois element is not valid");
        if (j0 < j1 && !galois_keys.has_key(galois_index(galois_elt)))
            throw std::invalid_argument("Galois key not present");
        if (e.size() != 2)
            throw std::invalid_argument("encrypted size must be 2");
        const Scheme scheme = context_.scheme();
        PlaneGeom g{ (unsigned)context_.log_n(), e.level()->K, (unsigned)e.batch() };
        const int ntt_form = scheme == Scheme::bfv ? 0 : 1;
        check_native_form(e);
        Scratch perm(2 * g.words());
        ck(k_apply_galois(context_.dev_mods(), e.data(), perm.p, galois_elt, ntt_form, g, 2, stream_), "apply_galois");
        ck(hipMemcpyAsync(e.plane(0), perm.p, g.words() * 8, hipMemcpyDeviceToDevice, stream_), "galois copy c0");
        ck(hipMemsetAsync(e.plane(1), 0, g.words() * 8, stream_), "galois zero c1");
        switch_key_partial(e, perm.p + g.words(), galois_keys, galois_index(galois_elt), acc,
                           ks_route(*e.level(), e.batch(), galois_keys, galois_index(galois_elt), j0, j1, true));
    }
    void Evaluator::apply_galois_finish(Ciphertext &e, uint64_t *acc, unsigned parts) const
    {
        StreamScope pool_scope(stream_);
        if (&e.context() != &context_ || !e.level() || e.size() != 2)
            throw std::invalid_argument("encrypted is not valid for encryption parameters");
        switch_key_finish(e, acc, parts, false, true);
        throw_if_transparent(e);
    }

    size_t Evaluator::switch_key_acc_words(const Ciphertext &e) const
    {
        if (&e.context() != &context_ || !e.level())
            throw std::invalid_argument("encrypted is not valid for encryption parameters");
        return (size_t)e.batch() * 2 * (e.level()->K + 1) * context_.n();
    }

    void Evaluator::switch_key_partial(const Ciphertext &e, const uint64_t *target, const KSwitchKeys &keys, size_t key_index, uint64_t *acc_out,
                                       const KsRoute &route, const KsAddend &addend) const
    {
        StreamScope pool_scope(stream_);
        check_valid(e, "encrypted");
        if (!target)
            throw std::invalid_argument("target_iter");
        if (!acc_out)
            throw std::invalid_argument("acc");
        if (!context_.using_keyswitching())
            throw std::logic_error("keyswitching is not supported by the context");
        const unsigned j0 = route.j0, j1 = route.j1, split = route.split;
        if (keys.context() != &context_ && !(j0 == j1 && !keys.context()))
            throw std::invalid_argument("parameter mismatch");
        if (j0 == j1 && j0 <= e.level()->K)
        {
            ck(hipMemsetAsync(acc_out, 0, switch_key_acc_words(e) * 8 * split, stream_), "ks zero partial sums");
            return;
        }
        if (key_index >= keys.slots())
            throw std::out_of_range("kswitch_keys_index");
        const Scheme scheme = context_.scheme();
        check_native_form(e);
        if (!keys.has_key(key_index))
            throw std::invalid_argument("kswitch_keys is not valid for encryption parameters");
        const KSwitchKeys::Key &key = keys.key(key_index);
        const Level &lvl = *e.level();
        const Level &klvl = context_.key_level();
        const unsigned K = lvl.K, L = klvl.K;
        if (j1 > K || j0 > j1)
            throw std::invalid_argument("digit range");
        const bool folds = addend.folds;
        if (folds && !(route.takes_product() && j0 == 0 && j1 == K))
            throw std::invalid_argument("fold_addend");
        if (j0 < j1 && (key.digit0 > j0 || key.digit0 + key.digits < j1))
            throw std::invalid_argument("kswitch_keys inner dimension is too small");
        if (e.size() < 2)
            throw std::invalid_argument("encrypted size must be at least 2");
        const LazyProduct *product = addend.prod;
        if (product && !((!product->x || (product->x->level() == e.level() && product->x->batch() == e.batch())) &&
                         (!product->y || (product->y->level() == e.level() && product->y->batch() == e.batch())) &&
                         (product->own || (product->x && product->y))))
            throw std::invalid_argument("product");
        const uint64_t *prod_xw = product ? product->xw() : nullptr, *prod_yw = product ? product->yw() : nullptr;

        const size_t N = context_.n();
        const unsigned B = (unsigned)e.batch();
        const unsigned n_log = (unsigned)context_.log_n();
        const NttTables &tb = context_.ntt_tables();
        const ModDesc *mods = context_.dev_mods();
        const uint32_t *map = ks_comp_prime(K);
        const size_t poly_words = (size_t)K * N;
        const bool ntt_target = scheme == Scheme::ckks || scheme == Scheme::bgv;
        const bool read_in_place = !ntt_target && route.fused;
        Scratch t(read_in_place ? 1 : (size_t)B * poly_words);
        const uint64_t *digits = read_in_place ? target : t.p;
        const KsPlan &plan = route.plan;
        const bool chunked = plan.chunk < B;
        const bool inverse_in_lane = chunked && !read_in_place && ntt_target;
        const auto inverse_batch = [&](unsigned b0, unsigned nb) {
            NttBatch bt = plain_batch(t.p + b0 * poly_words, poly_words, K, nb, 0);
            bt.src = target + b0 * poly_words;
            bt.src_outer_stride = poly_words;
            bt.src_galois_elt = addend.galois_elt;
            if (product)
            {
                bt.prod_x = prod_xw;
                bt.prod_y = prod_yw;
                bt.prod_batch = B;
                bt.prod_outer0 = 2 * B + b0;
            }
            return bt;
        };
        if (ntt_target && !inverse_in_lane && ntt2_supports(context_.log_n()))
            ck(ntt_inverse(tb, inverse_batch(0, B), 0, stream_), "ks intt target");
        else if (!read_in_place && !inverse_in_lane)
        {
            ck(hipMemcpyAsync(t.p, target, (size_t)B * poly_words * 8, hipMemcpyDeviceToDevice, stream_), "ks copy target");
            if (ntt_target)
                ck(ntt_inverse(tb, plain_batch(t.p, poly_words, K, B, 0), 0, stream_), "ks intt target");
        }

        if (route.fused)
        {
            const KsTargets &kt = ks_targets(K);
            const size_t ks_item_words = (size_t)(K + 1) * poly_words;
            if (ks_switches().trace)
                std::fprintf(stderr, "[ks] split %u (K %u, digits %u..%u)\n", split, K, j0, j1);
            Scratch mid((size_t)plan.lanes * plan.chunk * ks_item_words);
            Scratch inv_mid(inverse_in_lane ? (size_t)plan.lanes * plan.chunk * poly_words : 1);
            {
                uint64_t w = (uint64_t)plan.lanes * plan.chunk * ks_item_words, seen = g_ks_scratch_words_max.load();
                while (w > seen && !g_ks_scratch_words_max.compare_exchange_weak(seen, w))
                    ;
            }
            const auto fused_args = [&](unsigned b0, unsigned nb, unsigned lane) {
                KsFusedArgs ka{};
                ka.t = digits + b0 * poly_words;
                ka.target_ntt = ntt_target && !product ? target + b0 * poly_words : nullptr;
                ka.key = key.dev;
                ka.mid = mid.p + (size_t)lane * plan.chunk * ks_item_words;
                ka.acc = acc_out + (size_t)b0 * 2 * (K + 1) * N;
                ka.targets1 = kt.dev;
                ka.targets2 = kt.dev + 2 * (kt.n_int + kt.n_fp);
                ka.ntargets = kt.n_int + kt.n_fp;
                ka.n_int = kt.n_int;
                ka.K = K;
                ka.L = L;
                ka.batch = nb;
                ka.j0 = j0;
                ka.j1 = j1;
                ka.key_digit0 = (unsigned)key.digit0;
                ka.parts = split;
                if (folds)
                    ka.fold_pm = klvl.dev.inv_q_last_mod_q;
                if (product)
                {
                    ka.fold_x = prod_xw + b0 * poly_words;
                    ka.fold_y = prod_yw + b0 * poly_words;
                    ka.fold_plane = e.plane_words();
                }
                else if (folds)
                {
                    ka.fold_c0 = (addend.galois_elt ? addend.c0 : e.plane(0)) + b0 * poly_words;
                    ka.fold_c1 = addend.c1_zero ? nullptr : e.plane(1) + b0 * poly_words;
                    ka.galois_elt = addend.galois_elt;
                }
                return ka;
            };
            if (!chunked)
                ck(ks_fused(tb, fused_args(0, B, 0), stream_), "ks fused");
            else
            {
                KsLanes *ln = ks_lanes();
                unsigned lanes = plan.lanes;
                if (lanes > 1 && (!ln || !ln->ensure(lanes - 1)))
                    lanes = 1;
                if (ks_switches().trace)
                    std::fprintf(stderr, "[ks] batch %u in chunks of %u on %u lane(s)\n", B, plan.chunk, lanes);
                if (lanes > 1)
                {
                    ck(hipEventRecord(ln->fork, stream_), "ks lanes fork");
                    for (unsigned l = 1; l < lanes; l++)
                        ck(hipStreamWaitEvent(ln->stream[l - 1], ln->fork, 0), "ks lanes fork");
                }
                unsigned c = 0;
                auto join_lanes = [&](bool nothrow) {
                    for (unsigned l = 1; l < lanes; l++)
                    {
                        const hipError_t e1 = hipEventRecord(ln->join[l - 1], ln->stream[l - 1]);
                        const hipError_t e2 = e1 == hipSuccess ? hipStreamWaitEvent(stream_, ln->join[l - 1], 0) : e1;
                        if (e2 != hipSuccess)
                        {
                            if (!nothrow)
                                ck(e2, "ks lanes join");
                            (void)hipStreamSynchronize(ln->stream[l - 1]);
                        }
                    }
                };
                try
                {
                    for (unsigned b0 = 0; b0 < B; b0 += plan.chunk, c++)
                    {
                        const unsigned nb = B - b0 < plan.chunk ? B - b0 : plan.chunk;
                        const unsigned l = c % lanes;
                        hipStream_t st = l == 0 ? stream_ : ln->stream[l - 1];
                        if (inverse_in_lane)
                            ck(ntt2_inverse(tb, inverse_batch(b0, nb), 0, inv_mid.p + (size_t)l * plan.chunk * poly_words, st), "ks intt target (chunk)");
                        KsFusedArgs kc = fused_args(b0, nb, l);
                        kc.order1 = (size_t)B * (j1 - j0) * (N >> 12) >= 4096 ? 1 : 0;
                        kc.no_class_fork = lanes > 1 && !ks_switches().class_fork;
                        ck(ks_fused(tb, kc, st), "ks fused (chunk)");
                    }
                }
                catch (...)
                {
                    join_lanes(true);
                    throw;
                }
                join_lanes(false);
                g_ks_chunked_calls++;
                g_ks_chunks += c;
            }
        }
        else
        {
            Scratch u((size_t)B * (K + 1) * K * N);
            NttBatch b{};
            b.data = u.p;
            b.outer_stride = (size_t)(K + 1) * K * N;
            b.ncomp = (K + 1) * K;
            b.nouter = B;
            b.comp_prime = map;
            b.prime_first = 0;
            b.src = digits;
            b.src_outer_stride = (size_t)K * N;
            b.src_ncomp = K;
            b.src_mode = 1;
            ck(ntt_forward(tb, b, 0, stream_), "ks ntt digits");
            ck(k_keyswitch_mac(mods, u.p, key.dev, acc_out, n_log, K, L, B, j0, j1, (unsigned)key.digit0, stream_), "ks mac");
        }
    }

    void Evaluator::switch_key_finish(Ciphertext &e, uint64_t *acc, unsigned parts, bool acc_has_addend, bool may_defer) const
    {
        StreamScope pool_scope(stream_);
        check_valid(e, "encrypted");
        if (!acc)
            throw std::invalid_argument("acc");
        if (!context_.using_keyswitching())
            throw std::logic_error("keyswitching is not supported by the context");
        if (e.size() < 2)
            throw std::invalid_argument("encrypted size must be at least 2");
        if (parts < 1 || parts > 8)
            throw std::invalid_argument("parts");
        if (acc_has_addend && !(parts == 1 && context_.scheme() == Scheme::ckks && ntt2_supports(context_.log_n())))
            throw std::invalid_argument("acc_has_addend");
        const Scheme scheme = context_.scheme();
        const Level &lvl = *e.level();
        const Level &klvl = context_.key_level();
        const unsigned K = lvl.K, L = klvl.K;
        const size_t N = context_.n();
        const unsigned B = (unsigned)e.batch();
        const unsigned n_log = (unsigned)context_.log_n();
        const NttTables &tb = context_.ntt_tables();
        const ModDesc *mods = context_.dev_mods();
        const uint32_t *map = ks_comp_prime(K);
        if (may_defer && !acc_has_addend && ks_route(lvl, B).fold)
        {
            const size_t words = switch_key_acc_words(e);
            uint64_t *own = DevicePool::global().alloc_words(words, stream_);
            const hipError_t err = k_keyswitch_reduce(mods, acc, n_log, K, L, B, stream_, 1, e.plane(0), e.plane(1),
                                                      klvl.dev.inv_q_last_mod_q, own);
            if (err != hipSuccess)
            {
                DevicePool::global().free_words(own, stream_);
                ck(err, "ks reduce partial sums + addend");
            }
            defer_tail(e, own, true);
            return;
        }
        if (parts > 1)
            ck(k_keyswitch_reduce(mods, acc, n_log, K, L, B, stream_), "ks reduce partial sums");

        const uint64_t P = context_.coeff_modulus()[L - 1];
        if (scheme == Scheme::bgv)
        {
            NttBatch bi = plain_batch(acc + (size_t)K * N, (size_t)(K + 1) * N, 1, 2 * B, L - 1);
            ck(ntt_inverse(tb, bi, 0, stream_), "ks intt special");
            Scratch delta((size_t)B * 2 * K * N);
            ck(k_bgv_delta(mods, host::make_mod(context_.plain_modulus()), klvl.dev.inv_q_last_mod_t, klvl.dev.q_last_mod_q,
                           acc + (size_t)K * N, (size_t)(K + 1) * N, delta.p, n_log, K, (size_t)2 * B, stream_),
               "ks bgv delta");
            bgv_correct_and_combine(delta, acc, (size_t)(K + 1) * N, klvl.dev.inv_q_last_mod_q, K, 2 * B, e.plane(0), e.plane(1),
                                    (size_t)K * N, 2);
        }
        else if (scheme == Scheme::ckks)
        {
            NttBatch bi = plain_batch(acc + (size_t)K * N, (size_t)(K + 1) * N, 1, 2 * B, L - 1);
            ck(ntt_inverse(tb, bi, 0, stream_), "ks intt special");
            Scratch tt(ntt2_supports(context_.log_n()) ? 1 : (size_t)B * 2 * K * N);
            NttBatch b{};
            b.data = tt.p;
            b.outer_stride = (size_t)K * N;
            b.ncomp = K;
            b.nouter = 2 * B;
            b.comp_prime = nullptr;
            b.prime_first = 0;
            b.src = acc + (size_t)K * N;
            b.src_outer_stride = (size_t)(K + 1) * N;
            b.src_ncomp = 1;
            b.src_mode = 2;
            b.src_half = P >> 1;
            b.src_q = P;
            b.src_fix = klvl.dev.round_fix;
            if (ntt2_supports(context_.log_n()))
            {
                b.data = nullptr;
                b.epi = acc_has_addend ? 3 : 2;
                b.epi_a = acc;
                b.epi_a_stride = (size_t)(K + 1) * N;
                b.epi_mul = klvl.dev.inv_q_last_mod_q;
                b.epi_out0 = e.plane(0);
                b.epi_out1 = e.plane(1);
                b.epi_out_stride = (size_t)K * N;
                ck(ntt_forward(tb, b, 1, stream_), "ks ntt correction + tail");
            }
            else
            {
                ck(ntt_forward(tb, b, 1, stream_), "ks ntt correction");
                ck(k_keyswitch_tail_ckks(mods, klvl.dev.inv_q_last_mod_q, e.plane(0), e.plane(1), acc, tt.p, n_log, K, B, stream_),
                   "ks tail");
            }
        }
        else
        {
            NttBatch bi = plain_batch(acc, (size_t)(K + 1) * N, K + 1, 2 * B, 0);
            bi.comp_prime = map + (size_t)(K + 1) * K;
            bi.cls_hint = ks_class_hint(K);
            ck(ntt_inverse(tb, bi, 0, stream_), "ks intt all");
            ck(k_keyswitch_tail_bfv(
                   mods, klvl.dev.inv_q_last_mod_q, klvl.dev.round_fix, P >> 1, P, e.plane(0), e.plane(1), acc, n_log, K, B,
                   stream_),
               "ks tail bfv");
        }
    }

    void Evaluator::switch_key_inplace(Ciphertext &e, const uint64_t *target, const KSwitchKeys &keys, size_t key_index, const KsRoute &route,
                                       const KsAddend &addend) const
    {
        StreamScope pool_scope(stream_);
        if (&e.context() != &context_ || !e.level())
            throw std::invalid_argument("encrypted is not valid for encryption parameters");
        const unsigned K = e.level()->K, split = route.split;
        const bool fold = route.fold;
        if (addend.c1_zero && !fold)
            ck(hipMemsetAsync(e.plane(1), 0, e.plane_words() * 8, stream_), "zero c1");
        Scratch acc(switch_key_acc_words(e) * split);
        const bool own_planes = !addend.galois_elt && !addend.prod;
        switch_key_partial(e, target, keys, key_index, acc.p, route, own_planes && !route.takes_product() ? KsAddend::nothing() : addend);
        if (split > 1)
            ck(k_keyswitch_reduce(context_.dev_mods(), acc.p, (unsigned)context_.log_n(), K, context_.key_level().K, (unsigned)e.batch(),
                                  stream_, split, fold ? e.plane(0) : nullptr, fold && !addend.c1_zero ? e.plane(1) : nullptr,
                                  context_.key_level().dev.inv_q_last_mod_q),
               "ks add digit groups");
        if (route.defer)
            defer_tail(e, acc.release(), fold);
        else
            switch_key_finish(e, acc.p, 1);
    }

    void Evaluator::switch_key_finish_modswitch_bfv(Ciphertext &e, uint64_t *acc_p, const Level *next) const
    {
        StreamScope pool_scope(stream_);
        const Level &lvl = *e.level();
        const Level &klvl = context_.key_level();
        const unsigned K = lvl.K, L = klvl.K;
        const size_t N = context_.n();
        const unsigned B = (unsigned)e.batch();
        const NttTables &tb = context_.ntt_tables();
        const uint64_t P = context_.coeff_modulus()[L - 1];
        if (ks_switches().trace)
            std::fprintf(stderr, "[ks] folded tail (bfv)\n");
        g_tail_folded++;
        NttBatch bi = plain_batch(acc_p, (size_t)(K + 1) * N, K + 1, 2 * B, 0);
        bi.comp_prime = ks_comp_prime(K) + (size_t)(K + 1) * K;
        bi.cls_hint = ks_class_hint(K);
        ck(ntt_inverse(tb, bi, 0, stream_), "ks intt all");
        const size_t words = (size_t)2 * B * (K - 1) * N;
        uint64_t *out = DevicePool::global().alloc_words(words, stream_);
        const uint64_t *c0 = e.data_, *c1 = e.data_ + (size_t)B * K * N;
        hipError_t err = k_keyswitch_tail_modswitch_bfv(context_.dev_mods(), klvl.dev, P >> 1, P, lvl.dev, c0, c1, acc_p, out,
                                                        (unsigned)context_.log_n(), K, B, stream_);
        if (err != hipSuccess)
        {
            DevicePool::global().free_words(out, stream_);
            ck(err, "ks tail + mod switch (bfv)");
        }
        e.adopt(next, 2, out, words);
    }

    void Evaluator::switch_key_finish_rescale(Ciphertext &e, uint64_t *acc_p, const Level *next, double destination_scale, bool acc_has_addend) const
    {
        StreamScope pool_scope(stream_);
        const Level &lvl = *e.level();
        const Level &klvl = context_.key_level();
        const unsigned K = lvl.K, L = klvl.K;
        const size_t N = context_.n();
        const unsigned B = (unsigned)e.batch();
        const NttTables &tb = context_.ntt_tables();
        const uint64_t P = context_.coeff_modulus()[L - 1];
        uint64_t *c0 = e.data_, *c1 = e.data_ + (size_t)B * K * N;
        if (ks_switches().trace)
            std::fprintf(stderr, acc_has_addend ? "[ks] folded tail, addend in the sums\n" : "[ks] folded tail\n");
        g_tail_folded++;

        NttBatch bi = plain_batch(acc_p + (size_t)K * N, (size_t)(K + 1) * N, 1, 2 * B, L - 1);
        bi.out_add = P >> 1;
        ck(ntt_inverse(tb, bi, 0, stream_), "ks intt special");

        if (acc_has_addend)
        {
            NttBatch bw = plain_batch(acc_p + (size_t)(K - 1) * N, (size_t)(K + 1) * N, 1, 2 * B, K - 1);
            ck(ntt_inverse(tb, bw, 0, stream_), "ks intt last component");
            ck(k_ks_last_coeff(context_.dev_mods(), K - 1, klvl.dev.inv_q_last_mod_q + (K - 1), klvl.dev.round_fix + (K - 1),
                               lvl.dev.half_q_last, acc_p, (unsigned)context_.log_n(), K, (size_t)2 * B, stream_),
               "ks last component, coefficient form");
        }
        else
        {
            NttBatch b{};
            b.data = nullptr;
            b.outer_stride = N;
            b.ncomp = 1;
            b.nouter = 2 * B;
            b.comp_prime = nullptr;
            b.prime_first = K - 1;
            b.src = acc_p + (size_t)K * N;
            b.src_outer_stride = (size_t)(K + 1) * N;
            b.src_ncomp = 1;
            b.src_mode = 3;
            b.src_half = P >> 1;
            b.src_q = P;
            b.src_fix = klvl.dev.round_fix + (K - 1);
            b.epi = 2;
            b.epi_a = acc_p + (size_t)(K - 1) * N;
            b.epi_a_stride = (size_t)(K + 1) * N;
            b.epi_mul = klvl.dev.inv_q_last_mod_q + (K - 1);
            b.epi_out0 = c0 + (size_t)(K - 1) * N;
            b.epi_out1 = c1 + (size_t)(K - 1) * N;
            b.epi_out_stride = (size_t)K * N;
            ck(ntt_forward(tb, b, 1, stream_), "ks ntt correction + tail, last component");
        }
        if (!acc_has_addend)
        {
            NttBatch bl = plain_batch(c0 + (size_t)(K - 1) * N, (size_t)K * N, 1, 2 * B, K - 1);
            bl.out_add = lvl.dev.half_q_last;
            ck(ntt_inverse(tb, bl, 0, stream_), "rescale intt last");
        }

        const size_t words = (size_t)2 * B * (K - 1) * N;
        uint64_t *out = DevicePool::global().alloc_words(words);
        try
        {
            NttTail2 t2{};
            t2.src2_0 = c0 + (size_t)(K - 1) * N;
            t2.src2_1 = c1 + (size_t)(K - 1) * N;
            t2.src2_stride = (size_t)K * N;
            t2.src2_half = lvl.dev.half_q_last;
            t2.src2_q = lvl.dev.q_last;
            t2.src2_fix = lvl.dev.round_fix;
            t2.pmul = klvl.dev.inv_q_last_mod_q;
            t2.c0 = c0;
            t2.c1 = c1;
            t2.c_stride = (size_t)K * N;
            t2.halves_added = 1;
            if (acc_has_addend)
            {
                t2.src2_0 = acc_p + (size_t)(K - 1) * N;
                t2.src2_1 = acc_p + (size_t)(K + 1) * N + (size_t)(K - 1) * N;
                t2.src2_stride = (size_t)2 * (K + 1) * N;
                t2.a_has_c = 1;
            }
            NttBatch b{};
            b.data = nullptr;
            b.outer_stride = (size_t)(K - 1) * N;
            b.ncomp = K - 1;
            b.nouter = 2 * B;
            b.comp_prime = nullptr;
            b.prime_first = 0;
            b.src = acc_p + (size_t)K * N;
            b.src_outer_stride = (size_t)(K + 1) * N;
            b.src_ncomp = 1;
            b.src_mode = 3;
            b.src_half = P >> 1;
            b.src_q = P;
            b.src_fix = klvl.dev.round_fix;
            b.epi = 0;
            b.epi_a = acc_p;
            b.epi_a_stride = (size_t)(K + 1) * N;
            b.epi_mul = lvl.dev.inv_q_last_mod_q;
            b.epi_out0 = out;
            b.epi_out1 = out + (size_t)B * (K - 1) * N;
            b.epi_out_stride = (size_t)(K - 1) * N;
            b.tail2 = &t2;
            ck(ntt_forward(tb, b, 1, stream_), "mod-down + rescale in one transform");
        }
        catch (...)
        {
            DevicePool::global().free_words(out);
            throw;
        }
        e.adopt(next, 2, out, words);
        e.scale() = destination_scale;
    }

    unsigned Evaluator::switch_key_slots(const Ciphertext &e, unsigned nranks) const
    {
        if (&e.context() != &context_ || !e.level())
            throw std::invalid_argument("encrypted is not valid for encryption parameters");
        if (nranks < 1 || nranks > 8)
            throw std::invalid_argument("nranks");
        return (e.level()->K + nranks - 1) / nranks;
    }

    void Evaluator::switch_key_pack_targets(const Ciphertext &e, const uint64_t *acc, unsigned nranks, uint64_t *send, uint64_t *sp) const
    {
        StreamScope pool_scope(stream_);
        const unsigned m = switch_key_slots(e, nranks);
        if (!acc || !send || !sp)
            throw std::invalid_argument("buffer");
        ck(k_ks_pack_targets(acc, send, sp, (unsigned)context_.log_n(), e.level()->K, nranks, m, (unsigned)e.batch(), stream_), "ks pack targets");
    }

    void Evaluator::switch_key_finish_owned(
        const Ciphertext &e, const uint64_t *recv, const uint64_t *sp, unsigned nranks, unsigned rank, uint64_t *own) const
    {
        StreamScope pool_scope(stream_);
        const unsigned m = switch_key_slots(e, nranks);
        if (rank >= nranks)
            throw std::invalid_argument("rank");
        if (!recv || !sp || !own)
            throw std::invalid_argument("buffer");
        if (context_.scheme() != Scheme::ckks)
            throw std::logic_error("the reduce-scatter exchange is built for CKKS; BFV / BGV use the all-reduce exchange");
        if (!context_.using_keyswitching())
            throw std::logic_error("keyswitching is not supported by the context");
        const Level &lvl = *e.level();
        const Level &klvl = context_.key_level();
        const unsigned K = lvl.K, L = klvl.K, B = (unsigned)e.batch(), n_log = (unsigned)context_.log_n();
        const size_t N = context_.n();
        const NttTables &tb = context_.ntt_tables();
        const ModDesc *mods = context_.dev_mods();
        unsigned first, count;
        comm_split(K, nranks, rank, first, count);
        if (!count)
        {
            ck(hipMemsetAsync(own, 0, (size_t)m * B * 2 * N * 8, stream_), "ks zero own");
            return;
        }
        Scratch acc3((size_t)B * 2 * (count + 1) * N);
        ck(k_ks_unpack_owned(mods, recv, sp, acc3.p, n_log, L, first, count, B, stream_), "ks unpack owned");
        const uint64_t P = context_.coeff_modulus()[L - 1];
        NttBatch bi = plain_batch(acc3.p + (size_t)count * N, (size_t)(count + 1) * N, 1, 2 * B, L - 1);
        ck(ntt_inverse(tb, bi, 0, stream_), "ks intt special");
        Scratch inc((size_t)2 * B * count * N);
        ck(hipMemsetAsync(inc.p, 0, (size_t)2 * B * count * N * 8, stream_), "ks zero increments");
        Scratch tt(ntt2_supports(context_.log_n()) ? 1 : (size_t)B * 2 * count * N);
        NttBatch b{};
        b.data = tt.p;
        b.outer_stride = (size_t)count * N;
        b.ncomp = count;
        b.nouter = 2 * B;
        b.comp_prime = nullptr;
        b.prime_first = first;
        b.src = acc3.p + (size_t)count * N;
        b.src_outer_stride = (size_t)(count + 1) * N;
        b.src_ncomp = 1;
        b.src_mode = 2;
        b.src_half = P >> 1;
// ... 158 lines not shown
```

seal_amd/csrc/ntt2_kernels.h:

```cpp
#pragma once
#include "ntt_kernels.h"

namespace sealhip
{
    bool ntt2_supports(int log_n);

    size_t ntt2_ring_words(const NttTables &t, const NttBatch &b);
    hipError_t ntt2_forward(const NttTables &t, const NttBatch &b, int out_lazy, uint64_t *mid, hipStream_t stream, uint64_t *ring = nullptr, size_t ring_words = 0);

    struct NttRingRun
    {
        uint64_t *data;
        size_t outer_stride;
        const uint32_t *comp_prime;
        unsigned prime_first, ncomp, c0, nc, nouter;
        int lazy;
        unsigned teams_per_comp;
        uint64_t *ring;
        size_t ring_words;
    };
    unsigned ntt2_ring_teams(unsigned nc, unsigned nouter);
    size_t ntt2_ring_run_words(unsigned nc, unsigned teams_per_comp);
    bool ntt2_ring_stream_ok(hipStream_t stream);
    hipError_t ntt2_ring_launch(const NttTables &t, const NttRingRun &run, hipStream_t stream);

    hipError_t ntt2_inverse(const NttTables &t, const NttBatch &b, int out_lazy, uint64_t *mid, hipStream_t stream);

    struct KsFusedArgs
    {
        const uint64_t *t;
        const uint64_t *target_ntt;
        const uint64_t *key;
        uint64_t *mid;
        uint64_t *acc;
        const uint32_t *targets1, *targets2;
        unsigned ntargets, n_int;
        unsigned K, L, batch;
        unsigned j0, j1, key_digit0;
        unsigned parts;
        const uint64_t *fold_c0 = nullptr, *fold_c1 = nullptr;
        const ShoupOp *fold_pm = nullptr;
        const uint64_t *fold_x = nullptr, *fold_y = nullptr;
        size_t fold_plane = 0;
        uint32_t galois_elt = 0;
        int order1 = -1;
        bool no_class_fork = false;
    };
    hipError_t ks_fused(const NttTables &t, const KsFusedArgs &k, hipStream_t stream);

    inline unsigned key_comp_units(const NttTables &t, unsigned comp)
    {
        return t.fp_host && t.fp_host[comp] ? 2u : 4u;
    }
    inline unsigned key_comp_offset_units(const NttTables &t, unsigned comp)
    {
        unsigned u = 0;
        for (unsigned c = 0; c < comp; c++)
            u += key_comp_units(t, c);
        return u;
    }
    inline unsigned key_digit_units(const NttTables &t, unsigned L)
    {
        return key_comp_offset_units(t, L);
    }
    inline size_t key_register_order_words(const NttTables &t, unsigned L, size_t digits)
    {
        return (digits * key_digit_units(t, L)) << t.log_n;
    }
    hipError_t key_to_register_order(const NttTables &t, const uint64_t *in, uint64_t *out, unsigned L, size_t digits, hipStream_t stream);
    hipError_t key_from_register_order(const NttTables &t, const uint64_t *in, uint64_t *out, unsigned L, size_t digits, hipStream_t stream);
}
```

seal_amd/csrc/ntt2_kernels.hip:

```cpp
#include "ntt2_device.h"
#include <algorithm>
#include <atomic>
#include <cstdio>
#include <mutex>
#include <cstdlib>
#include <type_traits>
#include <vector>



namespace sealhip
{
    namespace
    {

        template <bool FP, int D1, int ICLS = 0, bool PACK = false>
        __device__ __forceinline__ void fwd_p1_body(const FwdArgs &a, unsigned prime, unsigned comp, unsigned outer, uint64_t *lds, unsigned tile)
        {
            typedef Field<FP> F;
            typedef Geo<D1> G;
            const unsigned tid = threadIdx.x, cg = tile;
            const typename F::Mod m = F::make_mod(ld_uniform_mod(&a.t.mods[prime]), ld_uniform_fpd(&a.t.fpd[prime]));
            const typename F::tw_t *tab = tw_table<FP>(a.t, false, prime);
            SrcMap sm{ 0, 0, 0, 0 };
// ... 388 lines not shown
        {
            HIP_DYNAMIC_SHARED(uint64_t, lds)
            const Blk blk = spread_blocks();
            const unsigned comp = blk.y + a.f.comp0, outer = blk.z;
            const unsigned prime = SHL_UNIFORM(a.f.prime_first + comp);
            if constexpr (CLS == 1)
                tail2_p2_body<true, D1, 0>(a, prime, comp, outer, lds, blk.tile);
            else if constexpr (CLS == 0)
                with_int_class(a.f.t, prime, [&](auto ic) { tail2_p2_body<false, D1, decltype(ic)::value>(a, prime, comp, outer, lds, blk.tile); });
            else if (a.f.t.fpd[prime].qi)
                tail2_p2_body<true, D1, 0>(a, prime, comp, outer, lds, blk.tile);
            else
                tail2_p2_body<false, D1, 2>(a, prime, comp, outer, lds, blk.tile);
        }

        __device__ __forceinline__ uint64_t resident_word(uint64_t v)
        {
#if defined(__HIP_DEVICE_COMPILE__)
            asm volatile("" : "+v"(v));
#endif
            return v;
        }

        template <bool FP, int D1, bool TWO, bool SMALL2>
        __device__ __forceinline__ void src_p1t_body(const Tail2Args &t2, unsigned nc, uint64_t *lds)
        {
            static_assert(!SMALL2 || (FP && TWO), "SMALL2 is a property of the double-precision launch of the folded tail");
            typedef Field<FP> F;
            typedef Geo<D1> G;
            const FwdArgs &a = t2.f;
            const unsigned tid = threadIdx.x;
            const unsigned grp = blockIdx.x;
            if (grp >= a.nouter * G::TILES)
                return;
            const unsigned cg = grp % G::TILES, outer = grp / G::TILES;
            const unsigned c = tid & (G::C - 1), rbl = tid >> G::LC;
            const size_t col = (size_t)cg * G::C + c;
            const uint64_t *in1 = a.src + (size_t)outer * a.src_outer_stride + col;
            [[maybe_unused]] const uint64_t *in2 = nullptr;
            if constexpr (TWO)
                in2 = ((outer & 1) ? t2.x.src2_1 : t2.x.src2_0) + (size_t)(outer >> 1) * t2.x.src2_stride + col;
            uint64_t r1[16];
            [[maybe_unused]] uint64_t r2[16];
#pragma unroll
            for (int e = 0; e < 16; e++)
            {
                const unsigned ra = e >> (4 - G::rA), rbh = e & ((1 << (4 - G::rA)) - 1);
                const unsigned R = ra * 16 + (rbh << G::rA) + rbl;
                r1[e] = in1[(size_t)R * 256];
                if constexpr (TWO)
                    r2[e] = in2[(size_t)R * 256];
            }
            const bool add_half = TWO ? !t2.x.halves_added : a.src_mode == 2;
            if (add_half)
            {
#pragma unroll
                for (int e = 0; e < 16; e++)
                {
                    r1[e] = csub(r1[e] + a.src_half, a.src_q);
                    if constexpr (TWO)
                        r2[e] = csub(r2[e] + t2.x.src2_half, t2.x.src2_q);
                }
            }
            if constexpr (SMALL2)
            {
#pragma unroll
                for (int e = 0; e < 16; e++)
                    r2[e] = fp_to_bits(fp_from_u52(r2[e]));
            }
#pragma nounroll
            for (unsigned it = 0; it < nc; it++)
            {
                const unsigned comp = a.comp0 + it;
                const unsigned prime = SHL_UNIFORM(a.comp_prime ? a.comp_prime[comp] : a.prime_first + comp);
                uint64_t *mid_tr = a.mid + (((size_t)outer * a.ncomp + comp) << G::n);
                auto one = [&](auto ic) {
                    constexpr int ICLS = decltype(ic)::value;
                    const typename F::Mod m = F::make_mod(ld_uniform_mod(&a.t.mods[prime]), ld_uniform_fpd(&a.t.fpd[prime]));
                    const typename F::tw_t *tab = tw_table<FP>(a.t, false, prime);
                    TwRegs<FP> tw;
                    p1_load_tw<FP, D1>(tw, tab, tid);
                    const SrcMap s1{ 3, 0, 0, a.src_fix[comp] };
                    typename F::elem x[16];
                    if constexpr (!TWO)
                    {
#pragma unroll
                        for (int e = 0; e < 16; e++)
                            x[e] = map_src<FP>(resident_word(r1[e]), s1, m);
                        p1_tile<FP, D1, 256, SEALHIP_P1_PLAIN_LEAN && FP && G::rA == 4, ICLS>(x, m, tab, tw, lds, mid_tr, cg, tid);
                    }
                    else
                    {
                        const ShoupOp pm = t2.x.pmul[comp];
                        const uint64_t q = a.t.mods[prime].q;
                        if constexpr (FP)
                        {
                            const double pinv = pm.w > q / 2 ? -(double)(q - pm.w) : (double)pm.w;
                            const double f1 = fp_from_u52(s1.fix), f2 = fp_from_u52(t2.x.src2_fix[comp]);
#pragma unroll
                            for (int e = 0; e < 16; e++)
                            {
                                const double v = F::from_any(resident_word(r1[e]), m) + f1;
                                const double u = (SMALL2 ? fp_from_bits(r2[e]) : F::from_any(resident_word(r2[e]), m)) + f2;
                                x[e] = fp_mulmod(v, pinv, m.q, m.qinv) + u;
                                F::fix(x[e], m);
                            }
                        }
                        else
                        {
                            const SrcMap s2{ 3, 0, 0, t2.x.src2_fix[comp] };
#pragma unroll
                            for (int e = 0; e < 16; e++)
                            {
                                const typename F::elem v = map_src<FP>(resident_word(r1[e]), s1, m), u = map_src<FP>(resident_word(r2[e]), s2, m);
                                x[e] = mul_shoup(v, pm.w, pm.wq, q) + u;
                            }
                        }
                        p1_tile<FP, D1, 256, FP && G::rA == 4, ICLS>(x, m, tab, tw, lds, mid_tr, cg, tid);
                    }
                };
                if constexpr (FP)
                    one(std::integral_constant<int, 0>());
                else
                    with_int_class(a.t, prime, one);
            }
        }

#ifndef SEALHIP_SRC_P1T_FP2_WGS
#define SEALHIP_SRC_P1T_FP2_WGS 2
#endif
        template <int D1, int CLS, bool TWO, bool SMALL2 = false>
        __global__ void __launch_bounds__(kThreads, SMALL2 ? SEALHIP_SRC_P1T_FP2_WGS : 2) ntt2_src_p1t(Tail2Args a, unsigned nc)
        {
            static_assert(CLS == 0 || CLS == 1, "single-class runs only");
            HIP_DYNAMIC_SHARED(uint64_t, lds)
            src_p1t_body<CLS == 1, D1, TWO, SMALL2>(a, nc, lds);
        }

        struct InvArgs
        {
            uint64_t *data;
            size_t outer_stride;
            const uint64_t *src;
            size_t src_outer_stride;
            uint64_t *mid;
            const uint32_t *comp_prime;
            int cls_hint;
            unsigned prime_first;
            unsigned ncomp;
            unsigned comp0;
            unsigned nouter;
            int lazy;
            uint64_t out_add;
            const uint64_t *prod_x, *prod_y;
            unsigned prod_batch, prod_outer0;
            uint64_t *prod_out;
            size_t prod_out_stride;
            uint32_t src_gal;
            NttTables t;
        };

        template <int ICLS>
        constexpr int kInvE1 = inv_phase_exp<ICLS>(0, 4, 0);
        template <int ICLS>
        constexpr int kInvE2 = inv_phase_exp<ICLS>(kInvE1<ICLS>, 4, 0);
        template <int ICLS>
        constexpr int kInvE3 = inv_phase_exp<ICLS>(kInvE2<ICLS>, 4, 0);

        template <bool FP, int D1, int ICLS = 2>
        __device__ __forceinline__ void inv_pa_body(const InvArgs &a, unsigned prime, unsigned comp, unsigned outer, uint64_t *lds, unsigned tile)
        {
            typedef Field<FP> F;
            typedef Geo<D1> G;
            const unsigned tid = threadIdx.x, hg = tile;
            const unsigned v = tid & 15, u = tid >> 4, ul = u & 3;
            const unsigned h = hg * 16 + u;
            const typename F::Mod m = F::make_mod(ld_uniform_mod(&a.t.mods[prime]), ld_uniform_fpd(&a.t.fpd[prime]));
            const typename F::tw_t *tab = tw_table<FP>(a.t, true, prime);
            uint64_t *lds_wave = lds + (tid >> 6) * (4 * kRowWords);
            uint64_t raw[16];
            typename F::elem x[16];
            bool have_x = false;
            const size_t rows = ((size_t)comp << G::n) + ((size_t)(hg * 16 + (tid >> 6) * 4) << 8);
            if (a.prod_x)
            {
                const unsigned go = outer + a.prod_outer0, pp = go / a.prod_batch, b = go - pp * a.prod_batch;
                const size_t plane = (size_t)a.prod_batch * a.src_outer_stride, off = (size_t)b * a.src_outer_stride + rows;
                [[maybe_unused]] const ModDesc md = ld_uniform_mod(&a.t.mods[prime]);
                uint64_t rb[16];
                load_rows(raw, lds_wave, a.prod_x + (pp == 2 ? plane : 0) + off, tid);
                load_rows(rb, lds_wave, a.prod_y + (pp == 0 ? 0 : plane) + off, tid);
                if constexpr (FP)
                {
#pragma unroll
                    for (int e = 0; e < 16; e++)
                        x[e] = fp_mulmod(fp_from_u52(raw[e]), fp_from_u52(rb[e]), m.q, m.qinv);
                    if (pp == 1)
                    {
                        uint64_t rc[16];
                        load_rows(rc, lds_wave, a.prod_x + plane + off, tid);
                        load_rows(rb, lds_wave, a.prod_y + off, tid);
#pragma unroll
                        for (int e = 0; e < 16; e++)
                            x[e] += fp_mulmod(fp_from_u52(rc[e]), fp_from_u52(rb[e]), m.q, m.qinv);
                    }
#pragma unroll
                    for (int e = 0; e < 16; e++)
                        F::fix(x[e], m);
                    if (a.prod_out)
                    {
#pragma unroll
                        for (int e = 0; e < 16; e++)
                            raw[e] = fp_to_canon(x[e], m);
                        store_rows(raw, lds_wave, a.prod_out + (size_t)outer * a.prod_out_stride + rows, tid);
                    }
                    have_x = true;
                }
                else
                {
#pragma unroll
                    for (int e = 0; e < 16; e++)
                        raw[e] = mul_mod(raw[e], rb[e], md);
                    if (pp == 1)
                    {
                        uint64_t rc[16];
                        load_rows(rc, lds_wave, a.prod_x + plane + off, tid);
                        load_rows(rb, lds_wave, a.prod_y + off, tid);
#pragma unroll
                        for (int e = 0; e < 16; e++)
                            raw[e] = add_mod(raw[e], mul_mod(rc[e], rb[e], md), md.q);
                    }
                    if (a.prod_out)
                        store_rows(raw, lds_wave, a.prod_out + (size_t)outer * a.prod_out_stride + rows, tid);
                }
            }
            else if (a.src_gal)
                load_rows_galois(raw, lds_wave, a.src + (size_t)outer * a.src_outer_stride + ((size_t)comp << G::n), (hg * 16 + (tid >> 6) * 4) << 8, a.src_gal, G::n, tid);
            else
                load_rows(raw, lds_wave, a.src + (size_t)outer * a.src_outer_stride + rows, tid);
            if (!have_x)
            {
#pragma unroll
                for (int e = 0; e < 16; e++)
                {
                    x[e] = F::from_canon(raw[e], m);
                    F::fix(x[e], m);
                }
            }
            {
                TwRegs<FP> tw;
                load_tw<FP, 4>(tw, tab, [&](int t) { return (1u << (D1 + 4 + t)) + ((h * 16 + v) << t); });
                phase_inv<FP, 4, 0, ICLS, 0>(x, m, [&](int t, int g) { return tw.get((1 << t) + g); });
            }
#pragma unroll
            for (int e = 0; e < 16; e++)
                F::fix(x[e], m);
#pragma unroll
            for (int e = 0; e < 16; e++)
                lds_wave[ul * kRowWords + v * 18 + e] = F::raw(x[e]);
            __builtin_amdgcn_wave_barrier();
#pragma unroll
            for (int e = 0; e < 16; e++)
                x[e] = F::unraw(lds_wave[ul * kRowWords + e * 18 + v]);
            {
                TwRegs<FP> tw;
                load_tw<FP, 4>(tw, tab, [&](int t) { return (1u << (D1 + t)) + (h << t); });
                phase_inv<FP, 4, 0, ICLS, kInvE1<ICLS>>(x, m, [&](int t, int g) { return tw.get((1 << t) + g); });
            }
#pragma unroll
            for (int e = 0; e < 16; e++)
                F::fix(x[e], m);
            uint64_t *mid_tr = a.mid + (((size_t)outer * a.ncomp + comp) << G::n) + ((size_t)hg << 12);
#pragma unroll
            for (int e = 0; e < 16; e++)
                mid_st<8>(mid_tr + e * 256 + tid, F::raw(x[e]));
        }

        template <int D1, int CLS>
        __global__ void __launch_bounds__(kThreads) ntt2_inv_pa(InvArgs a)
        {
            HIP_DYNAMIC_SHARED(uint64_t, lds)
            const Blk blk = spread_blocks();
            const unsigned comp = blk.y + a.comp0, outer = blk.z;
            const unsigned prime = SHL_UNIFORM(a.comp_prime ? a.comp_prime[comp] : a.prime_first + comp);
            if constexpr (CLS == 1)
                inv_pa_body<true, D1>(a, prime, comp, outer, lds, blk.tile);
            else if constexpr (CLS == 0)
                with_int_class(a.t, prime, [&](auto ic) { inv_pa_body<false, D1, decltype(ic)::value>(a, prime, comp, outer, lds, blk.tile); });
            else if (a.t.fpd[prime].qi)
                inv_pa_body<true, D1>(a, prime, comp, outer, lds, blk.tile);
            else
                inv_pa_body<false, D1, 2>(a, prime, comp, outer, lds, blk.tile);
        }

        template <bool FP, int D1, int ICLS = 2>
        __device__ __forceinline__ void inv_pb_body(const InvArgs &a, unsigned prime, unsigned comp, unsigned outer, uint64_t *lds, unsigned tile)
        {
            typedef Field<FP> F;
            typedef Geo<D1> G;
            static_assert(G::rA >= 1, "the N^-1 stage is handled in phase A");
            const unsigned tid = threadIdx.x, cg = tile;
            const unsigned c = tid & (G::C - 1), hi = tid >> G::LC;
            const typename F::Mod m = F::make_mod(ld_uniform_mod(&a.t.mods[prime]), ld_uniform_fpd(&a.t.fpd[prime]));
            const typename F::tw_t *tab = tw_table<FP>(a.t, true, prime);
            const unsigned col = cg * G::C + c;
            const uint64_t *i = a.mid + (((size_t)outer * a.ncomp + comp) << G::n) + ((size_t)(hi * 16 + (col >> 4)) << 8) + (col & 15);
            typename F::elem x[16];
#pragma unroll
            for (int rb = 0; rb < 16; rb++)
                x[rb] = F::unraw(mid_ld<8>(i + rb * 16));
            {
                TwRegs<FP> tw;
                load_tw<FP, 4>(tw, tab, [&](int t) { return (1u << (G::rA + t)) + (hi << t); });
                phase_inv<FP, 4, 0, ICLS, kInvE2<ICLS>>(x, m, [&](int t, int g) { return tw.get((1 << t) + g); });
            }
#pragma unroll
            for (int e = 0; e < 16; e++)
                F::fix(x[e], m);
#pragma unroll
            for (int rb = 0; rb < 16; rb++)
                lds[(hi * 16 + rb) * G::CP + c] = F::raw(x[rb]);
            __syncthreads();
#pragma unroll
            for (int e = 0; e < 16; e++)
            {
                const unsigned ra = e >> (4 - G::rA), rbh = e & ((1 << (4 - G::rA)) - 1);
                const unsigned R = ra * 16 + (rbh << G::rA) + hi;
                x[e] = F::unraw(lds[R * G::CP + c]);
            }
            phase_inv<FP, G::rA, 1, ICLS, kInvE3<ICLS>>(x, m, [&](int t, int g) { return ld_uniform(tab, (1u << t) + g); });
            {
                typename F::tw_t ni, nw;
                if constexpr (FP)
                {
                    ni = ld_uniform(a.t.ninv_d, 2 * prime);
                    nw = ld_uniform(a.t.ninv_d, 2 * prime + 1);
                }
                else
                {
                    ni = ld_uniform(a.t.ninv, 2 * prime);
                    nw = ld_uniform(a.t.ninv, 2 * prime + 1);
                }
                inv_last_stage<FP, G::rA, ICLS, kInvE3<ICLS>>(x, m, ni, nw);
            }
            uint64_t *o = a.data + (size_t)outer * a.outer_stride + ((size_t)comp << G::n);
#pragma unroll
            for (int e = 0; e < 16; e++)
            {
                F::fix(x[e], m);
                const unsigned ra = e >> (4 - G::rA), rbh = e & ((1 << (4 - G::rA)) - 1);
                const unsigned R = ra * 16 + (rbh << G::rA) + hi;
                uint64_t v = a.lazy ? F::inv_to_lazy(x[e], m) : F::inv_to_canon(x[e], m);
                if (a.out_add)
                    v = csub(v + a.out_add, a.t.mods[prime].q);
                mid_st<16>(o + (size_t)R * 256 + col, v);
            }
        }

        template <int D1, int CLS>
        __global__ void __launch_bounds__(kThreads) ntt2_inv_pb(InvArgs a)
        {
            HIP_DYNAMIC_SHARED(uint64_t, lds)
            const Blk blk = spread_blocks();
            const unsigned comp = blk.y + a.comp0, outer = blk.z;
            const unsigned prime = SHL_UNIFORM(a.comp_prime ? a.comp_prime[comp] : a.prime_first + comp);
            if constexpr (CLS == 1)
                inv_pb_body<true, D1>(a, prime, comp, outer, lds, blk.tile);
            else if constexpr (CLS == 0)
                with_int_class(a.t, prime, [&](auto ic) { inv_pb_body<false, D1, decltype(ic)::value>(a, prime, comp, outer, lds, blk.tile); });
            else if (a.t.fpd[prime].qi)
                inv_pb_body<true, D1>(a, prime, comp, outer, lds, blk.tile);
            else
                inv_pb_body<false, D1, 2>(a, prime, comp, outer, lds, blk.tile);
        }

        template <int D1, int TWW = 1>
        struct FusedGeo
        {
            typedef Geo<D1> G;
            static_assert(G::LC >= 6, "pass 1's phase-B row index must be wave-uniform");
            static_assert(G::lds1_words <= kLds2Words, "pass 1's exchange buffer lives in the team's pass-2 area");
            static constexpr int TEAMS = G::TILES;
            static constexpr int BS = 272;
            static constexpr size_t mid_words = (size_t)TEAMS * 16 * BS;
            static constexpr size_t xch_words = (size_t)TEAMS * kLds2Words;
            static constexpr size_t main_words = mid_words > xch_words ? mid_words : xch_words;
            static constexpr size_t lds_bytes = (main_words + (size_t)TEAMS * 240 * TWW) * 8;
        };
#ifndef SEALHIP_FINT_FWD_TWB
#define SEALHIP_FINT_FWD_TWB 0
#endif
#ifndef SEALHIP_FINT_FWD_PF13
#define SEALHIP_FINT_FWD_PF13 0
#endif
#ifndef SEALHIP_FINT_FWD_PF14
#define SEALHIP_FINT_FWD_PF14 1
#endif
#ifndef SEALHIP_FINT_FWD_WAVES
#define SEALHIP_FINT_FWD_WAVES 4
#endif
#ifndef SEALHIP_FINT_INV_TWB
#define SEALHIP_FINT_INV_TWB 1
#endif
#ifndef SEALHIP_FINT_INV_PF
#define SEALHIP_FINT_INV_PF 0
#endif
#ifndef SEALHIP_FINT_INV_WAVES
#define SEALHIP_FINT_INV_WAVES 4
#endif

        template <bool FP, int D1, int ICLS = 0>
        __device__ __forceinline__ void fwd_fused2_body(const FwdArgs &a, unsigned prime, unsigned comp, unsigned outer, uint64_t *lds)
        {
            typedef Field<FP> F;
            typedef Geo<D1> G;
            typedef FusedGeo<D1, F::tw_words> FG;
            typedef typename F::tw_t tw_t;
            constexpr bool TWB_REGS = FP || (D1 == 5 && SEALHIP_FINT_FWD_TWB == 2);
            constexpr bool TWB_EARLY = !FP && D1 == 5 && SEALHIP_FINT_FWD_TWB == 1;
#ifndef SEALHIP_FP_FWD_PF13
#define SEALHIP_FP_FWD_PF13 0
#endif
            constexpr bool PF = FP ? (D1 != 5 || SEALHIP_FP_FWD_PF13) : ((D1 == 6 && SEALHIP_FINT_FWD_PF14) || (D1 == 5 && SEALHIP_FINT_FWD_PF13));
            const unsigned team = threadIdx.x >> 8, tid = threadIdx.x & 255;
            const typename F::Mod m = F::make_mod(ld_uniform_mod(&a.t.mods[prime]), ld_uniform_fpd(&a.t.fpd[prime]));
            const tw_t *tab = tw_table<FP>(a.t, false, prime);
            uint64_t *mid = lds;
            uint64_t *xch = lds + team * kLds2Words;
            uint64_t *lds_wave = xch + (tid >> 6) * (4 * kRowWords);
            tw_t *twa = reinterpret_cast<tw_t *>(lds + FG::main_words) + team * 240;
            stage_twa<D1>(twa, tab, team, tid);
            const unsigned c = tid & (G::C - 1);
            const unsigned hi = SHL_UNIFORM(tid >> G::LC);
            TwRegs<FP> twb, unused;
            if constexpr (TWB_REGS)
            {
                const unsigned h = team * 16 + (tid >> 4), v = tid & 15;
                load_tw<FP, 4>(twb, tab, [&](int t) { return (1u << (D1 + 4 + t)) + ((h * 16 + v) << t); });
            }
            uint64_t *base = a.data + ((size_t)comp << G::n);
            const uint64_t *in_base = a.src ? a.src + ((size_t)(comp % a.src_ncomp) << G::n) : base;
            const size_t in_stride = a.src ? a.src_outer_stride : a.outer_stride;
            uint64_t nxt[16];
            auto fetch = [&](unsigned z) {
                const uint64_t *in = in_base + (size_t)z * in_stride + team * G::C + c;
#pragma unroll
                for (int e = 0; e < 16; e++)
                {
                    const unsigned ra = e >> (4 - G::rA), rbh = e & ((1 << (4 - G::rA)) - 1);
                    const unsigned R = ra * 16 + (rbh << G::rA) + hi;
                    nxt[e] = in[(size_t)R * 256];
                }
            };
            const unsigned ostride = gridDim.z;
            if constexpr (PF)
                fetch(outer);
            for (; outer < a.nouter; outer += ostride)
            {
                typename F::elem x[16];
                if constexpr (!PF)
                    fetch(outer);
#pragma unroll
                for (int e = 0; e < 16; e++)
                    x[e] = F::from_canon(nxt[e], m);
                if constexpr (PF)
                {
                    if (outer + ostride < a.nouter)
                        fetch(outer + ostride);
                }
                phase_fwd_end<FP, G::rA, true, ICLS, 4>(x, m, [&](int t, int g) { return ld_uniform(tab, (1u << t) + g); });
                __syncthreads();
#pragma unroll
                for (int e = 0; e < 16; e++)
                {
                    const unsigned ra = e >> (4 - G::rA), rbh = e & ((1 << (4 - G::rA)) - 1);
                    const unsigned R = ra * 16 + (rbh << G::rA) + hi;
                    xch[R * G::CP + c] = F::raw(x[e]);
                }
                __syncthreads();
#pragma unroll
                for (int rb = 0; rb < 16; rb++)
                    x[rb] = F::unraw(xch[(hi * 16 + rb) * G::CP + c]);
                phase_fwd_end<FP, 4, true, ICLS, IntBounds<ICLS>::fwd_after(4, G::rA)>(
                    x, m, [&](int t, int g) { return ld_uniform(tab, (1u << (G::rA + t)) + (hi << t) + g); });
                __syncthreads();
                {
                    const unsigned col = team * G::C + c;
                    uint64_t *o = mid + (size_t)(hi * 16 + (col >> 4)) * FG::BS + (col & 15);
#pragma unroll
                    for (int rb = 0; rb < 16; rb++)
                        o[rb * 16] = F::raw(x[rb]);
                }
                __syncthreads();
                {
                    const uint64_t *mp = mid + (size_t)(team * 16) * FG::BS + tid;
#pragma unroll
                    for (int e = 0; e < 16; e++)
                        x[e] = F::unraw(mp[e * FG::BS]);
                }
                if constexpr (TWB_EARLY)
                {
                    const unsigned h = team * 16 + (tid >> 4), v = tid & 15;
                    load_tw<FP, 4>(twb, tab, [&](int t) { return (1u << (D1 + 4 + t)) + ((h * 16 + v) << t); });
                }
                __syncthreads();
                if constexpr (TWB_REGS || TWB_EARLY)
                    p2_tile<FP, D1, false, false, true, true, false, ICLS, kP1Out<ICLS, D1>>(x, m, tab, twa, nullptr, lds_wave, team, tid, &unused, &twb);
// ... 2 lines not shown
                uint64_t val[16];
#pragma unroll
                for (int e = 0; e < 16; e++)
                    val[e] = a.lazy ? fwd_out_lazy<FP, ICLS, kP2Out<ICLS, D1>>(x[e], m) : fwd_out_canon<FP, ICLS, kP2Out<ICLS, D1>>(x[e], m);
                store_rows(val, lds_wave, base + (size_t)outer * a.outer_stride + ((size_t)(team * 16 + (tid >> 6) * 4) << 8), tid);
            }
        }

        template <int D1, int CLS>
        __global__ void __launch_bounds__(FusedGeo<D1>::TEAMS *kThreads, CLS == 1 ? 4 : SEALHIP_FINT_FWD_WAVES) ntt2_fwd_fused2(FwdArgs a)
        {
            HIP_DYNAMIC_SHARED(uint64_t, lds)
            const unsigned comp = blockIdx.y + a.comp0, outer = blockIdx.z;
            const unsigned prime = SHL_UNIFORM(a.comp_prime ? a.comp_prime[comp] : a.prime_first + comp);
            if constexpr (CLS == 1)
                fwd_fused2_body<true, D1>(a, prime, comp, outer, lds);
            else
                with_int_class(a.t, prime, [&](auto ic) { fwd_fused2_body<false, D1, decltype(ic)::value>(a, prime, comp, outer, lds); });
        }

        template <bool FP, int D1, int ICLS = 2>
        __device__ __forceinline__ void inv_fused2_body(const InvArgs &a, unsigned prime, unsigned comp, unsigned outer, uint64_t *lds)
        {
            typedef Field<FP> F;
            typedef Geo<D1> G;
            typedef FusedGeo<D1, F::tw_words> FG;
            typedef typename F::tw_t tw_t;
            static_assert(G::rA >= 1, "the N^-1 stage is handled in phase A");
#ifndef SEALHIP_FP_INV_PF
#define SEALHIP_FP_INV_PF 0
#endif
            constexpr bool PF = FP ? (SEALHIP_FP_INV_PF || D1 != 5) : (D1 == 5 && SEALHIP_FINT_INV_PF);
            const unsigned team = threadIdx.x >> 8, tid = threadIdx.x & 255;
            const unsigned v = tid & 15, u = tid >> 4, ul = u & 3, lane = tid & 63;
            const unsigned h = team * 16 + u;
            const typename F::Mod m = F::make_mod(ld_uniform_mod(&a.t.mods[prime]), ld_uniform_fpd(&a.t.fpd[prime]));
            const tw_t *tab = tw_table<FP>(a.t, true, prime);
            uint64_t *mid = lds;
            uint64_t *xch = lds + team * kLds2Words;
            uint64_t *lds_wave = xch + (tid >> 6) * (4 * kRowWords);
            tw_t *twa = reinterpret_cast<tw_t *>(lds + FG::main_words) + team * 240;
            stage_twa<D1>(twa, tab, team, tid);
            const unsigned c = tid & (G::C - 1);
            const unsigned hi = SHL_UNIFORM(tid >> G::LC);
            const unsigned col = team * G::C + c;
            tw_t ni, nw;
            if constexpr (FP)
            {
                ni = ld_uniform(a.t.ninv_d, 2 * prime);
                nw = ld_uniform(a.t.ninv_d, 2 * prime + 1);
            }
            else
            {
                ni = ld_uniform(a.t.ninv, 2 * prime);
                nw = ld_uniform(a.t.ninv, 2 * prime + 1);
            }
            const size_t comp_off = (size_t)comp << G::n;
            const size_t row_off = comp_off + ((size_t)(team * 16 + (tid >> 6) * 4) << 8);
            uint64_t nxt[16];
            auto fetch = [&](unsigned z) {
                const uint64_t *rows = a.src + (size_t)z * a.src_outer_stride + row_off;
#pragma unroll
                for (int k = 0; k < 16; k++)
                    nxt[k] = rows[(k >> 2) * 256 + (k & 3) * 64 + lane];
            };
            const unsigned ostride = gridDim.z;
            if constexpr (PF)
                fetch(outer);
            __syncthreads();
            for (; outer < a.nouter; outer += ostride)
            {
                if constexpr (!PF)
                    fetch(outer);
                TwRegs<FP> twb_early;
                if constexpr (!FP && SEALHIP_FINT_INV_TWB == 1)
                    load_tw<FP, 4>(twb_early, tab, [&](int t) { return (1u << (D1 + 4 + t)) + ((h * 16 + v) << t); });
#pragma unroll
                for (int k = 0; k < 16; k++)
                {
                    const unsigned row = k >> 2, cc = (k & 3) * 64 + lane;
                    lds_wave[row * kRowWords + cc + 2 * (cc >> 4)] = nxt[k];
                }
                __builtin_amdgcn_wave_barrier();
                typename F::elem x[16];
#pragma unroll
                for (int e = 0; e < 16; e++)
                {
                    x[e] = F::from_canon(lds_wave[ul * kRowWords + v * 18 + e], m);
                    F::fix(x[e], m);
                }
                __builtin_amdgcn_wave_barrier();
                {
                    if constexpr (FP)
                    {
                        TwRegs<FP> twb;
                        load_tw<FP, 4>(twb, tab, [&](int t) { return (1u << (D1 + 4 + t)) + ((h * 16 + v) << t); });
                        phase_inv<FP, 4, 0, ICLS, 0>(x, m, [&](int t, int g) { return twb.get((1 << t) + g); });
                    }
                    else if constexpr (SEALHIP_FINT_INV_TWB == 1)
                        phase_inv<FP, 4, 0, ICLS, 0>(x, m, [&](int t, int g) { return twb_early.get((1 << t) + g); });
                    else
                        phase_inv<FP, 4, 0, ICLS, 0>(x, m, [&](int t, int g) { return tab[(1u << (D1 + 4 + t)) + ((h * 16 + v) << t) + g]; });
                }
#pragma unroll
                for (int e = 0; e < 16; e++)
                    F::fix(x[e], m);
                if constexpr (PF)
                {
                    if (outer + ostride < a.nouter)
                        fetch(outer + ostride);
                }
#pragma unroll
                for (int e = 0; e < 16; e++)
                    lds_wave[ul * kRowWords + v * 18 + e] = F::raw(x[e]);
                __builtin_amdgcn_wave_barrier();
#pragma unroll
                for (int e = 0; e < 16; e++)
                    x[e] = F::unraw(lds_wave[ul * kRowWords + e * 18 + v]);
                phase_inv<FP, 4, 0, ICLS, kInvE1<ICLS>>(x, m, [&](int t, int g) { return twa[(16u << t) - 16u + (u << t) + g]; });
#pragma unroll
                for (int e = 0; e < 16; e++)
                    F::fix(x[e], m);
                __syncthreads();
#pragma unroll
                for (int e = 0; e < 16; e++)
                    mid[(size_t)(team * 16 + e) * FG::BS + tid] = F::raw(x[e]);
                __syncthreads();
                {
                    const uint64_t *i = mid + (size_t)(hi * 16 + (col >> 4)) * FG::BS + (col & 15);
#pragma unroll
                    for (int rb = 0; rb < 16; rb++)
                        x[rb] = F::unraw(i[rb * 16]);
                }
                phase_inv<FP, 4, 0, ICLS, kInvE2<ICLS>>(x, m, [&](int t, int g) { return ld_uniform(tab, (1u << (G::rA + t)) + (hi << t) + g); });
#pragma unroll
                for (int e = 0; e < 16; e++)
                    F::fix(x[e], m);
                __syncthreads();
#pragma unroll
                for (int rb = 0; rb < 16; rb++)
                    xch[(hi * 16 + rb) * G::CP + c] = F::raw(x[rb]);
                __syncthreads();
#pragma unroll
                for (int e = 0; e < 16; e++)
                {
                    const unsigned ra = e >> (4 - G::rA), rbh = e & ((1 << (4 - G::rA)) - 1);
                    const unsigned R = ra * 16 + (rbh << G::rA) + hi;
                    x[e] = F::unraw(xch[R * G::CP + c]);
                }
                __syncthreads();
                phase_inv<FP, G::rA, 1, ICLS, kInvE3<ICLS>>(x, m, [&](int t, int g) { return ld_uniform(tab, (1u << t) + g); });
                inv_last_stage<FP, G::rA, ICLS, kInvE3<ICLS>>(x, m, ni, nw);
                uint64_t *o = a.data + (size_t)outer * a.outer_stride + comp_off;
#pragma unroll
                for (int e = 0; e < 16; e++)
                {
                    F::fix(x[e], m);
                    const unsigned ra = e >> (4 - G::rA), rbh = e & ((1 << (4 - G::rA)) - 1);
                    const unsigned R = ra * 16 + (rbh << G::rA) + hi;
                    uint64_t v = a.lazy ? F::inv_to_lazy(x[e], m) : F::inv_to_canon(x[e], m);
                    if (a.out_add)
                        v = csub(v + a.out_add, a.t.mods[prime].q);
                    o[(size_t)R * 256 + col] = v;
                }
            }
        }

        template <int D1, int CLS>
        __global__ void __launch_bounds__(FusedGeo<D1>::TEAMS *kThreads, CLS == 1 ? 4 : SEALHIP_FINT_INV_WAVES) ntt2_inv_fused2(InvArgs a)
        {
            HIP_DYNAMIC_SHARED(uint64_t, lds)
            const unsigned comp = blockIdx.y + a.comp0, outer = blockIdx.z;
            const unsigned prime = SHL_UNIFORM(a.comp_prime ? a.comp_prime[comp] : a.prime_first + comp);
            if constexpr (CLS == 1)
                inv_fused2_body<true, D1>(a, prime, comp, outer, lds);
            else
                with_int_class(a.t, prime, [&](auto ic) { inv_fused2_body<false, D1, decltype(ic)::value>(a, prime, comp, outer, lds); });
        }

#ifdef SEALHIP_KS_LEAN_OFF
        template <int D1>
        constexpr bool kLeanKs = false;
#else
        template <int D1>
        constexpr bool kLeanKs = D1 == 8;
#endif
        constexpr double kLeanEntry = 1.13;

        struct Ks1Args
        {
            const uint64_t *t;
            uint64_t *mid;
            const uint32_t *targets;
            unsigned ntargets;
            unsigned K;
            unsigned batch;
            unsigned j0, j1;
            unsigned parts;
            int skip_diag;
            NttTables tb;
        };

        template <bool FP, int D1>
        __device__ __forceinline__ void ks1_map(const uint64_t (&nxt)[16], typename Field<FP>::elem (&x)[16], uint64_t src_q, const typename Field<FP>::Mod &m)
        {
            typedef Field<FP> F;
            if constexpr (FP)
            {
                if (src_q >> 52)
                {
#pragma unroll
                    for (int e = 0; e < 16; e++)
                    {
                        x[e] = F::from_any(nxt[e], m);
                        if constexpr (kLeanKs<D1>)
                            F::fix(x[e], m);
                    }
                }
                else
                {
#pragma unroll
                    for (int e = 0; e < 16; e++)
                        x[e] = fp_from_u52(nxt[e]);
                    if (!kLeanKs<D1> || (double)src_q > kLeanEntry * m.q)
                    {
#pragma unroll
                        for (int e = 0; e < 16; e++)
                            F::fix(x[e], m);
                    }
                }
            }
            else
            {
                if (src_q < 4 * m.q)
                {
#pragma unroll
                    for (int e = 0; e < 16; e++)
                        x[e] = nxt[e];
                }
                else
                {
#pragma unroll
                    for (int e = 0; e < 16; e++)
                        x[e] = F::from_any(nxt[e], m);
                }
            }
        }

        template <bool FP, int D1, int ICLS = 0>
        __device__ __forceinline__ void ks1_body(const Ks1Args &a, uint64_t *lds, unsigned I, unsigned prime, unsigned b, unsigned cg, unsigned j0, unsigned j1)
        {
            typedef Field<FP> F;
            typedef Geo<D1> G;
            const unsigned tid = threadIdx.x;
            const typename F::Mod m = F::make_mod(ld_uniform_mod(&a.tb.mods[prime]), ld_uniform_fpd(&a.tb.fpd[prime]));
            const typename F::tw_t *tab = tw_table<FP>(a.tb, false, prime);
            TwRegs<FP> tw;
            p1_load_tw<FP, D1>(tw, tab, tid);
            const unsigned c = tid & (G::C - 1), rbl = tid >> G::LC;
            const uint64_t *in0 = a.t + (((size_t)b * a.K) << G::n) + cg * G::C + c;
            uint64_t nxt[16];
            auto fetch = [&](unsigned J) {
                const uint64_t *in = in0 + ((size_t)J << G::n);
#pragma unroll
                for (int e = 0; e < 16; e++)
                {
                    const unsigned ra = e >> (4 - G::rA), rbh = e & ((1 << (4 - G::rA)) - 1);
                    const unsigned R = ra * 16 + (rbh << G::rA) + rbl;
#ifdef SEALHIP_KS_NOMEM
                    nxt[e] = (uint64_t)((tid << 4) + (unsigned)e + J * 4099u + R);
#else
                    nxt[e] = in[(size_t)R * 256];
#endif
                }
            };
            const unsigned Jskip = a.skip_diag ? I : ~0u;
            unsigned J = Jskip == j0 ? j0 + 1 : j0;
            if (J < j1)
                fetch(J);
            while (J < j1)
            {
                const uint64_t src_q = a.tb.mods[J].q;
                typename F::elem x[16];
                ks1_map<FP, D1>(nxt, x, src_q, m);
                unsigned Jn = J + 1;
                if (Jn == Jskip)
                    Jn++;
                if (Jn < j1)
                    fetch(Jn);
                uint64_t *mid_tr = a.mid + ((((size_t)b * (a.K + 1) + I) * a.K + J) << G::n);
                p1_tile<FP, D1, 256, FP && kLeanKs<D1>, ICLS>(x, m, tab, tw, lds, mid_tr, cg, tid);
                J = Jn;
            }
        }

        template <bool FP, int D1>
        __global__ void __launch_bounds__(kThreads) ks1_kernel(Ks1Args a)
        {
            typedef Geo<D1> G;
            HIP_DYNAMIC_SHARED(uint64_t, lds)
            const unsigned bid = blockIdx.x;
            const unsigned low = bid & 7, rest = bid >> 3;
            const unsigned it = rest % a.ntargets, grp = (rest / a.ntargets) * 8 + low;
            if (grp >= a.batch * a.parts * G::TILES)
                return;
            const unsigned vb = grp / G::TILES, cg = grp % G::TILES;
            const unsigned b = vb % a.batch, dg = vb / a.batch;
            const unsigned jlen = (a.j1 - a.j0 + a.parts - 1) / a.parts;
            const unsigned j0 = a.j0 + dg * jlen, j1 = j0 + jlen < a.j1 ? j0 + jlen : a.j1;
            const unsigned I = SHL_UNIFORM(a.targets[2 * it]), prime = SHL_UNIFORM(a.targets[2 * it + 1]);
            if constexpr (FP)
                ks1_body<FP, D1>(a, lds, I, prime, b, cg, j0, j1);
            else
                with_int_class(a.tb, prime, [&](auto ic) { ks1_body<FP, D1, decltype(ic)::value>(a, lds, I, prime, b, cg, j0, j1); });
        }

        template <bool FP, int D1, bool SMALL = false>
        __global__ void __launch_bounds__(kThreads, 2) ks1t_kernel(Ks1Args a)
        {
            static_assert(FP || !SMALL, "SMALL is a property of the double-precision launch");
            typedef Field<FP> F;
            typedef Geo<D1> G;
            HIP_DYNAMIC_SHARED(uint64_t, lds)
            const unsigned tid = threadIdx.x;
            const unsigned ndig = a.j1 - a.j0;
            const unsigned grp = blockIdx.x;
            if (grp >= a.batch * ndig * G::TILES)
                return;
            const unsigned cg = grp % G::TILES, bj = grp / G::TILES;
            const unsigned J = a.j0 + bj % ndig, b = bj / ndig;
            const unsigned c = tid & (G::C - 1), rbl = tid >> G::LC;
            const uint64_t *in = a.t + (((size_t)b * a.K + J) << G::n) + cg * G::C + c;
            uint64_t raw[16];
#pragma unroll
            for (int e = 0; e < 16; e++)
            {
                const unsigned ra = e >> (4 - G::rA), rbh = e & ((1 << (4 - G::rA)) - 1);
                const unsigned R = ra * 16 + (rbh << G::rA) + rbl;
                raw[e] = in[(size_t)R * 256];
            }
            const uint64_t src_q = a.tb.mods[J].q;
            const bool as_doubles = SMALL || (FP && !(src_q >> 52));
            if (as_doubles)
            {
#pragma unroll
                for (int e = 0; e < 16; e++)
                    raw[e] = fp_to_bits(fp_from_u52(raw[e]));
            }
#pragma nounroll
            for (unsigned it = 0; it < a.ntargets; it++)
            {
                const unsigned I = SHL_UNIFORM(a.targets[2 * it]), prime = SHL_UNIFORM(a.targets[2 * it + 1]);
                if (a.skip_diag && I == J)
                    continue;
                uint64_t *mid_tr = a.mid + ((((size_t)b * (a.K + 1) + I) * a.K + J) << G::n);
                auto one = [&](auto ic) {
                    constexpr int ICLS = decltype(ic)::value;
                    const typename F::Mod m = F::make_mod(ld_uniform_mod(&a.tb.mods[prime]), ld_uniform_fpd(&a.tb.fpd[prime]));
                    const typename F::tw_t *tab = tw_table<FP>(a.tb, false, prime);
                    TwRegs<FP> tw;
                    p1_load_tw<FP, D1>(tw, tab, tid);
                    typename F::elem x[16];
                    if constexpr (FP)
                    {
                        if (as_doubles)
                        {
#pragma unroll
                            for (int e = 0; e < 16; e++)
                                x[e] = fp_from_bits(raw[e]);
                            if (!kLeanKs<D1> || (double)src_q > kLeanEntry * m.q)
                            {
#pragma unroll
                                for (int e = 0; e < 16; e++)
                                    F::fix(x[e], m);
                            }
                        }
                        else if constexpr (!SMALL)
                            ks1_map<FP, D1>(raw, x, src_q, m);
                    }
                    else
                        ks1_map<FP, D1>(raw, x, src_q, m);
                    p1_tile<FP, D1, 256, FP && kLeanKs<D1>, ICLS>(x, m, tab, tw, lds, mid_tr, cg, tid);
                };
                if constexpr (FP)
                    one(std::integral_constant<int, 0>());
                else
                    with_int_class(a.tb, prime, one);
            }
        }

        struct Ks2Args
        {
            const uint64_t *mid;
            const uint64_t *target;
            const uint64_t *key;
            size_t key_digit_words;
            uint64_t *acc;
            const uint32_t *targets;
            unsigned ntargets;
            unsigned K, L;
            unsigned batch;
            unsigned j0, j1, key_digit0;
            unsigned parts;
            const uint64_t *fold_c0, *fold_c1;
            const ShoupOp *fold_pm;
            const uint64_t *fold_x, *fold_y;
            size_t fold_plane;
            uint32_t gal;
            NttTables tb;
        };

#ifndef SEALHIP_KS2_INT_TWB3
#define SEALHIP_KS2_INT_TWB3 1
#endif
        template <bool FP, int D1, int ICLS = 0>
        __device__ __forceinline__ void ks2_body(const Ks2Args &a, uint64_t *lds, unsigned I, unsigned prime, unsigned koff, unsigned b, unsigned hg,
                                                 unsigned j0, unsigned j1, uint64_t *acc_part)
        {
            typedef Field<FP> F;
            typedef Geo<D1> G;
            const unsigned tid = threadIdx.x;
            const typename F::Mod m = F::make_mod(ld_uniform_mod(&a.tb.mods[prime]), ld_uniform_fpd(&a.tb.fpd[prime]));
            const typename F::tw_t *tab = tw_table<FP>(a.tb, false, prime);

            uint64_t *lds_wave = lds + (tid >> 6) * (4 * kRowWords);
            const typename F::tw_t *twa = nullptr, *twb = nullptr;
            if constexpr (!FP)
            {
                typename F::tw_t *la = reinterpret_cast<typename F::tw_t *>(lds + kLds2Words);
                if (tid < 240)
                {
                    const unsigned t = 31 - __builtin_clz(tid / 16 + 1);
                    const unsigned r = tid - ((16u << t) - 16u);
                    la[tid] = tab[(1u << (D1 + t)) + ((hg * 16) << t) + r];
                }
                twa = la;
#if SEALHIP_KS2_INT_TWB3
                typename F::tw_t *lb = la + 240;
#pragma unroll
                for (int g = 0; g < 8; g++)
                    lb[g * 256 + tid] = tab[(1u << (D1 + 7)) + ((hg * 256 + tid) << 3) + g];
                twb = lb;
#endif
                __syncthreads();
            }
            if constexpr (FP)
            {
                typename F::tw_t *la = reinterpret_cast<typename F::tw_t *>(lds + kLds2Words);
                typename F::tw_t *lb = la + 240;
                if (tid < 240)
                {
                    const unsigned t = 31 - __builtin_clz(tid / 16 + 1);
                    const unsigned r = tid - ((16u << t) - 16u);
                    la[tid] = tab[(1u << (D1 + t)) + ((hg * 16) << t) + r];
                }
#pragma unroll
                for (int t = 0; t < 4; t++)
#pragma unroll
                    for (int g = 0; g < (1 << t); g++)
                        lb[((256u << t) - 256u) + g * 256 + tid] = tab[(1u << (D1 + 4 + t)) + ((hg * 256 + tid) << t) + g];
                twa = la;
                twb = lb;
                __syncthreads();
            }

            typedef typename std::conditional<FP, typename F::Acc, uint64_t>::type acc_t;
            constexpr unsigned kAccRun = ICLS == 2 ? 1 : IntBounds<ICLS>::lim / 4 - 1;
            acc_t acc0[16], acc1[16];
#pragma unroll
            for (int e = 0; e < 16; e++)
            {
                if constexpr (FP)
                {
                    acc0[e] = F::acc_zero();
                    acc1[e] = F::acc_zero();
                }
                else
                {
                    acc0[e] = 0;
                    acc1[e] = 0;
                }
            }
            const size_t N = (size_t)1 << G::n;
            const uint64_t *mid0 = a.mid + ((((size_t)b * (a.K + 1) + I) * a.K) << G::n) + ((size_t)hg << 12);
            const uint64_t *mid0_lane = mid0 + mid_lane(tid);
            const bool diag_prod = a.fold_x && !a.target && I < a.K;
            const bool has_diag = (a.target || diag_prod) && I < a.K;
            const size_t diag_off = (((size_t)b * a.K + I) << G::n) + ((size_t)hg << 12);
            const UniformView diag_view = uniform_view(diag_prod ? a.fold_x + a.fold_plane + diag_off : has_diag ? a.target + diag_off : a.mid);
            uint64_t nxt[16];
            auto fetch = [&](unsigned J) {
                if (has_diag && J == I)
// ... 632 lines not shown
                        const unsigned z = ntt2_ring_teams(r.nc, nouter);
                        if (z && ntt2_ring_run_words(r.nc, z) <= a.ring_words && ntt2_ring_stream_ok(st))
                        {
                            const NttRingRun run{ a.data, a.outer_stride, a.comp_prime, a.prime_first, a.ncomp, r.c0, r.nc, nouter, a.lazy, z, a.ring, a.ring_words };
                            return ntt2_ring_launch(a.t, run, st);
                        }
                    }
                }
                if constexpr (D1 == 8)
                {
                    if (g.mid_pack)
                    {
                        hipLaunchKernelGGL((ntt2_fwd_p1<D1, 5>), grid, dim3(kThreads), l1, st, g);
                        hipError_t ep = hipGetLastError();
                        if (ep != hipSuccess)
                            return ep;
                        hipLaunchKernelGGL((ntt2_fwd_p2<D1, 5>), grid, dim3(kThreads), (kLds2Words + 240) * 8, st, g);
                        return hipGetLastError();
                    }
                }
                if (a.src && (a.src_mode == 2 || a.src_mode == 3) && a.src_ncomp == 1 && src_resident(G::TILES, nouter, r))
                {
                    hipError_t e1 = launch_src_p1t<D1, false>(Tail2Args{ g, NttTail2{} }, r, nouter, st);
                    if (e1 != hipSuccess)
                        return e1;
                }
                else if (r.cls == 1)
                    hipLaunchKernelGGL((ntt2_fwd_p1<D1, 1>), grid, dim3(kThreads), l1, st, g);
                else if (r.cls == 0)
                    hipLaunchKernelGGL((ntt2_fwd_p1<D1, 0>), grid, dim3(kThreads), l1, st, g);
                else
                    hipLaunchKernelGGL((ntt2_fwd_p1<D1, 2>), grid, dim3(kThreads), l1, st, g);
                hipError_t e = hipGetLastError();
                if (e != hipSuccess)
                    return e;
                static const int p2_hoist = shl_ab_getenv("SEALHIP_P2_HOIST") ? std::atoi(shl_ab_getenv("SEALHIP_P2_HOIST")) : 4;
                if (r.cls == 1 && a.epi == 0 && chunks < nouter && p2_hoist == 4)
                    hipLaunchKernelGGL((ntt2_fwd_p2<D1, 4>), grid, dim3(kThreads), (kLds2Words + 240) * 8, st, g);
                else if (r.cls == 1 && a.epi == 0 && chunks < nouter && p2_hoist == 3)
                    hipLaunchKernelGGL((ntt2_fwd_p2<D1, 3>), grid, dim3(kThreads), kLds2Words * 8, st, g);
                else if (r.cls == 1)
                    hipLaunchKernelGGL((ntt2_fwd_p2<D1, 1>), grid, dim3(kThreads), kLds2Words * 8, st, g);
                else if (r.cls == 0)
                    hipLaunchKernelGGL((ntt2_fwd_p2<D1, 0>), grid, dim3(kThreads), kLds2Words * 8, st, g);
                else
                    hipLaunchKernelGGL((ntt2_fwd_p2<D1, 2>), grid, dim3(kThreads), kLds2Words * 8, st, g);
                return hipGetLastError();
            }, !(fused && fused_int()) || (D1 == 6 && SEALHIP_FUSED_FORK14));
        }

        template <int D1>
        hipError_t launch_tail2(const Tail2Args &a, unsigned nouter, hipStream_t s)
        {
            typedef Geo<D1> G;
            unsigned per = G::TILES * a.f.ncomp;
#ifndef SEALHIP_TAIL2_WG_TARGET
#define SEALHIP_TAIL2_WG_TARGET 4096
#endif
            unsigned chunks = (SEALHIP_TAIL2_WG_TARGET + per - 1) / per;
            if (chunks > nouter)
                chunks = nouter;
            if (chunks > 65535)
                chunks = 65535;
            const size_t l1 = G::rA > 0 ? G::lds1_words * 8 : 8;
            return launch_runs(comp_runs(a.f.t, nullptr, a.f.prime_first, a.f.ncomp), s, [&](const CompRun &r, hipStream_t st) {
                Tail2Args g = a;
                g.f.comp0 = r.c0;
                dim3 grid(G::TILES, r.nc, chunks);
                if (src_resident(G::TILES, nouter, r))
                {
                    hipError_t e1 = launch_src_p1t<D1, true>(g, r, nouter, st);
                    if (e1 != hipSuccess)
                        return e1;
                }
                else if (r.cls == 1)
                    hipLaunchKernelGGL((ntt2_tail2_p1<D1, 1>), grid, dim3(kThreads), l1, st, g);
                else if (r.cls == 0)
                    hipLaunchKernelGGL((ntt2_tail2_p1<D1, 0>), grid, dim3(kThreads), l1, st, g);
                else
                    hipLaunchKernelGGL((ntt2_tail2_p1<D1, 2>), grid, dim3(kThreads), l1, st, g);
                hipError_t e = hipGetLastError();
                if (e != hipSuccess)
                    return e;
                if (r.cls == 1)
                    hipLaunchKernelGGL((ntt2_tail2_p2<D1, 1>), grid, dim3(kThreads), kLds2Words * 8, st, g);
                else if (r.cls == 0)
                    hipLaunchKernelGGL((ntt2_tail2_p2<D1, 0>), grid, dim3(kThreads), kLds2Words * 8, st, g);
                else
                    hipLaunchKernelGGL((ntt2_tail2_p2<D1, 2>), grid, dim3(kThreads), kLds2Words * 8, st, g);
                return hipGetLastError();
            });
        }

        template <int D1>
        hipError_t launch_inv(const InvArgs &a, unsigned nouter, hipStream_t s)
        {
            typedef Geo<D1> G;
            bool fused = false;
            unsigned fchunks = 1;
            if constexpr (D1 == 5 || D1 == 6)
            {
                static const bool fused_ok = !shl_ab_getenv("SEALHIP_NTT_NOFUSED");
                if (fused_ok && !a.prod_x && !a.src_gal)
                {
                    static bool raised = false;
                    if (!raised)
                    {
                        if (hipFuncSetAttribute(reinterpret_cast<const void *>(&ntt2_inv_fused2<D1, 1>), hipFuncAttributeMaxDynamicSharedMemorySize, (int)FusedGeo<D1>::lds_bytes) != hipSuccess ||
                            hipFuncSetAttribute(reinterpret_cast<const void *>(&ntt2_inv_fused2<D1, 0>), hipFuncAttributeMaxDynamicSharedMemorySize, (int)(FusedGeo<D1, 2>::lds_bytes)) != hipSuccess)
                            return hipErrorInvalidValue;
                        raised = true;
                    }
                    fused = true;
                    const unsigned want = D1 == 5 ? 2048 : 1024;
                    fchunks = (want + a.ncomp - 1) / a.ncomp;
                    if (D1 == 5 && nouter / 4 > fchunks)
                        fchunks = nouter / 4;
                    if (const char *f = std::getenv("SEALHIP_NTT_FCHUNKS"))
                        fchunks = (unsigned)std::atoi(f) ? (unsigned)std::atoi(f) : 1;
                    if (fchunks > nouter)
                        fchunks = nouter;
                    if (fchunks > 65535)
                        fchunks = 65535;
                }
            }
            return launch_runs(comp_runs(a.t, a.comp_prime, a.prime_first, a.ncomp, a.cls_hint), s, [&](const CompRun &r, hipStream_t st) {
                InvArgs g = a;
                g.comp0 = r.c0;
                g.nouter = nouter;
                if constexpr (D1 == 5 || D1 == 6)
                {
                    if (fused && r.cls == 1)
                    {
                        hipLaunchKernelGGL((ntt2_inv_fused2<D1, 1>), dim3(1, r.nc, fchunks), dim3(FusedGeo<D1>::TEAMS * kThreads), FusedGeo<D1>::lds_bytes, st, g);
                        return hipGetLastError();
                    }
                    if (fused && r.cls == 0 && fused_int())
                    {
                        constexpr size_t lds_int = FusedGeo<D1, 2>::lds_bytes;
                        hipLaunchKernelGGL((ntt2_inv_fused2<D1, 0>), dim3(1, r.nc, fchunks), dim3(FusedGeo<D1>::TEAMS * kThreads), lds_int, st, g);
                        return hipGetLastError();
                    }
                }
                dim3 grid(G::TILES, r.nc, nouter);
                if (r.cls == 1)
                    hipLaunchKernelGGL((ntt2_inv_pa<D1, 1>), grid, dim3(kThreads), kLds2Words * 8, st, g);
                else if (r.cls == 0)
                    hipLaunchKernelGGL((ntt2_inv_pa<D1, 0>), grid, dim3(kThreads), kLds2Words * 8, st, g);
                else
                    hipLaunchKernelGGL((ntt2_inv_pa<D1, 2>), grid, dim3(kThreads), kLds2Words * 8, st, g);
                hipError_t e = hipGetLastError();
                if (e != hipSuccess)
                    return e;
                static const char *skip_env = shl_ab_getenv("SEALHIP_AB_SKIP_INV_PB");
                static long skip_after = skip_env ? std::atol(skip_env) : -1;
                static std::atomic<long> inv_launches{ 0 };
                if (skip_after >= 0 && inv_launches.fetch_add(1) >= skip_after)
                    return (hipError_t)hipSuccess;
                if (r.cls == 1)
                    hipLaunchKernelGGL((ntt2_inv_pb<D1, 1>), grid, dim3(kThreads), G::lds1_words * 8, st, g);
                else if (r.cls == 0)
                    hipLaunchKernelGGL((ntt2_inv_pb<D1, 0>), grid, dim3(kThreads), G::lds1_words * 8, st, g);
                else
                    hipLaunchKernelGGL((ntt2_inv_pb<D1, 2>), grid, dim3(kThreads), G::lds1_words * 8, st, g);
                return hipGetLastError();
            }, !(fused && fused_int()) || (D1 == 6 && SEALHIP_FUSED_FORK14));
        }

        template <int D1>
        hipError_t launch_ks(const Ks1Args &a1, const Ks2Args &a2, unsigned batch, unsigned n_int, hipStream_t s, int order1, bool no_class_fork)
        {
            typedef Geo<D1> G;
            if (a1.ntargets == 0)
                return hipSuccess;
            const size_t l1 = G::rA > 0 ? G::lds1_words * 8 : 8;
            const unsigned vbatch = batch * a1.parts;
            const unsigned groups = vbatch * G::TILES;
            const unsigned n_fp = a1.ntargets - n_int;
            const size_t l2_fp = kLds2Words * 8 + (240 + 3840) * sizeof(double);
            const size_t l2_int = kLds2Words * 8 + (240 + (SEALHIP_KS2_INT_TWB3 ? 2048 : 0)) * sizeof(ShoupOp);
            if (n_int && l2_int > 65536)
            {
                static bool raised_int = false;
                if (!raised_int)
                {
                    if (hipFuncSetAttribute(reinterpret_cast<const void *>(&ks2_kernel<D1, 0>), hipFuncAttributeMaxDynamicSharedMemorySize, (int)l2_int) != hipSuccess)
                        return hipErrorInvalidValue;
                    raised_int = true;
                }
            }
            if (n_fp && l2_fp > 65536)
            {
                static bool raised = false;
                if (!raised)
                {
                    if (hipFuncSetAttribute(reinterpret_cast<const void *>(&ks2_kernel<D1, 1>), hipFuncAttributeMaxDynamicSharedMemorySize, (int)l2_fp) != hipSuccess)
                        return hipErrorInvalidValue;
                    raised = true;
                }
            }
            auto run_class = [&](bool fp, hipStream_t st) -> hipError_t {
                const unsigned t0 = fp ? n_int : 0, nt = fp ? n_fp : n_int;
                if (!nt)
                    return hipSuccess;
                Ks1Args c1 = a1;
                c1.targets = a1.targets + 2 * t0;
                c1.ntargets = nt;
                const dim3 g1(((groups + 7) / 8) * nt * 8);
                static const char *order_env = shl_ab_getenv("SEALHIP_KS1_ORDER");
                const unsigned g1t = batch * (a1.j1 - a1.j0) * G::TILES;
                const bool digit_resident = order_env ? order_env[0] == '1' : order1 >= 0 ? (order1 == 1 && a1.parts == 1) : (a1.parts == 1 && g1t >= 4096);
                if (digit_resident && fp)
                {
                    const unsigned char *small = a1.tb.fp_host;
                    for (unsigned ja = a1.j0; ja < a1.j1;)
                    {
                        const bool sm = small && small[ja];
                        unsigned jb = ja + 1;
                        while (jb < a1.j1 && (small && small[jb]) == sm)
                            jb++;
                        Ks1Args cr = c1;
                        cr.j0 = ja;
                        cr.j1 = jb;
                        const dim3 gr(batch * (jb - ja) * G::TILES);
                        if (sm)
                            hipLaunchKernelGGL((ks1t_kernel<true, D1, true>), gr, dim3(kThreads), l1, st, cr);
                        else
                            hipLaunchKernelGGL((ks1t_kernel<true, D1, false>), gr, dim3(kThreads), l1, st, cr);
                        ja = jb;
                    }
                }
                else if (digit_resident)
                    hipLaunchKernelGGL((ks1t_kernel<false, D1>), dim3(g1t), dim3(kThreads), l1, st, c1);
                else if (fp)
                    hipLaunchKernelGGL((ks1_kernel<true, D1>), g1, dim3(kThreads), l1, st, c1);
                else
                    hipLaunchKernelGGL((ks1_kernel<false, D1>), g1, dim3(kThreads), l1, st, c1);
                hipError_t e = hipGetLastError();
                if (e != hipSuccess)
                    return e;
                Ks2Args c2 = a2;
                c2.targets = a2.targets + 4 * t0;
                c2.ntargets = nt;
                const unsigned ntile = nt * G::TILES;
                if (fp)
                    hipLaunchKernelGGL((ks2_kernel<D1, 1>), dim3(((ntile + 7) / 8) * vbatch * 8), dim3(kThreads), l2_fp, st, c2);
                else
                    hipLaunchKernelGGL((ks2_kernel<D1, 0>), dim3(((ntile + 7) / 8) * vbatch * 8), dim3(kThreads), l2_int, st, c2);
                return hipGetLastError();
            };
            SideStream &ss = side_stream();
            static const bool fork_ok = !shl_ab_getenv("SEALHIP_KS_NOFORK");
            hipError_t e;
            if (n_int && n_fp && ss.ok && fork_ok && !no_class_fork)
            {
                if ((e = hipEventRecord(ss.fork, s)) != hipSuccess || (e = hipStreamWaitEvent(ss.stream, ss.fork, 0)) != hipSuccess)
                    return e;
                if ((e = run_class(false, ss.stream)) != hipSuccess || (e = hipEventRecord(ss.join, ss.stream)) != hipSuccess)
                    return e;
                if ((e = run_class(true, s)) != hipSuccess)
                    return e;
                return hipStreamWaitEvent(s, ss.join, 0);
            }
            if ((e = run_class(false, s)) != hipSuccess)
                return e;
            return run_class(true, s);
        }
    }

    bool ntt2_supports(int log_n)
    {
        return log_n >= 13 && log_n <= 16;
    }

    size_t ntt2_ring_words(const NttTables &t, const NttBatch &b)
    {
        if (t.log_n != 16 || b.src || b.epi || b.tail2 || b.ncomp == 0 || b.nouter == 0)
            return 0;
        if (!ntt2_ring_teams(1, b.nouter))
            return 0;
        size_t words = 0;
        for (const CompRun &r : comp_runs(t, b.comp_prime, b.prime_first, b.ncomp, b.cls_hint))
            if (r.cls == 1)
            {
                const unsigned z = ntt2_ring_teams(r.nc, b.nouter);
                if (z)
                    words = std::max(words, ntt2_ring_run_words(r.nc, z));
            }
        return words;
    }

    hipError_t ntt2_forward(const NttTables &t, const NttBatch &b, int out_lazy, uint64_t *mid, hipStream_t stream, uint64_t *ring, size_t ring_words)
    {
        if (b.ncomp == 0 || b.nouter == 0)
            return hipSuccess;
        FwdArgs a;
        a.ring = ring;
        a.ring_words = ring ? ring_words : 0;
        a.data = b.data;
        a.outer_stride = b.outer_stride;
        a.mid = mid;
        a.src = b.src;
        a.src_outer_stride = b.src_outer_stride;
        a.src_ncomp = b.src_ncomp ? b.src_ncomp : 1;
        a.src_mode = b.src ? b.src_mode : 0;
        a.src_half = b.src_half;
        a.src_q = b.src_q;
        a.src_fix = b.src_fix;
        a.comp_prime = b.comp_prime;
        a.cls_hint = b.cls_hint;
        a.prime_first = b.prime_first;
        a.ncomp = b.ncomp;
        a.comp0 = 0;
        a.nouter = b.nouter;
        a.lazy = out_lazy;
        a.epi = b.epi;
        a.epi_a = b.epi_a;
        a.epi_a_stride = b.epi_a_stride;
        a.epi_mul = b.epi_mul;
        a.epi_out0 = b.epi_out0;
        a.epi_out1 = b.epi_out1;
        a.epi_out_stride = b.epi_out_stride;
        a.mid_pack = 0;
        a.t = t;
        if (b.tail2)
        {
            if (!b.src || (b.src_mode != 2 && b.src_mode != 3) || b.comp_prime || !b.epi_a || !b.epi_mul || !b.epi_out0 || !b.epi_out1)
                return hipErrorInvalidValue;
            Tail2Args t2{ a, *b.tail2 };
            switch (t.log_n)
            {
            case 13:
                return launch_tail2<5>(t2, b.nouter, stream);
            case 14:
                return launch_tail2<6>(t2, b.nouter, stream);
            case 15:
                return launch_tail2<7>(t2, b.nouter, stream);
            case 16:
                return launch_tail2<8>(t2, b.nouter, stream);
            default:
                return hipErrorInvalidValue;
            }
        }
        switch (t.log_n)
        {
        case 13:
            return launch_fwd<5>(a, b.nouter, stream);
        case 14:
            return launch_fwd<6>(a, b.nouter, stream);
        case 15:
            return launch_fwd<7>(a, b.nouter, stream);
        case 16:
            return launch_fwd<8>(a, b.nouter, stream);
        default:
            return hipErrorInvalidValue;
        }
    }

    hipError_t ntt2_inverse(const NttTables &t, const NttBatch &b, int out_lazy, uint64_t *mid, hipStream_t stream)
    {
        if (b.ncomp == 0 || b.nouter == 0)
            return hipSuccess;
        InvArgs a;
        a.data = b.data;
        a.outer_stride = b.outer_stride;
        a.src = b.src ? b.src : b.data;
        a.src_outer_stride = b.src ? b.src_outer_stride : b.outer_stride;
        a.mid = mid;
        a.comp_prime = b.comp_prime;
        a.cls_hint = b.cls_hint;
        a.prime_first = b.prime_first;
        a.ncomp = b.ncomp;
        a.comp0 = 0;
        a.nouter = 0;
        a.lazy = out_lazy;
        if (b.out_add && out_lazy)
            return hipErrorInvalidValue;
        a.out_add = b.out_add;
        a.prod_x = b.prod_x;
        a.prod_y = b.prod_y;
        a.prod_batch = b.prod_batch;
        a.prod_outer0 = b.prod_outer0;
        a.prod_out = b.prod_out;
        a.prod_out_stride = b.prod_out_stride;
        a.src_gal = b.src_galois_elt;
        if (b.src_galois_elt && (!b.src || b.prod_x || !(b.src_galois_elt & 1)))
            return hipErrorInvalidValue;
        if (b.prod_x && (!b.prod_y || !b.prod_batch || (size_t)b.nouter + b.prod_outer0 > (size_t)3 * b.prod_batch || !b.src_outer_stride))
            return hipErrorInvalidValue;
        if (b.prod_x && !b.prod_outer0 && b.nouter != 3 * b.prod_batch)
            return hipErrorInvalidValue;
        if (b.prod_out && (!b.prod_x || !b.prod_out_stride))
            return hipErrorInvalidValue;
        if (b.prod_x)
            a.src_outer_stride = b.src_outer_stride;
        a.t = t;
        const unsigned zmax = 65535;
        for (unsigned z0 = 0; z0 < b.nouter; z0 += zmax)
        {
            unsigned nz = b.nouter - z0 < zmax ? b.nouter - z0 : zmax;
            InvArgs az = a;
            az.prod_outer0 = b.prod_outer0 + z0;
            if (az.prod_out)
                az.prod_out = a.prod_out + (size_t)z0 * a.prod_out_stride;
            az.data = a.data + (size_t)z0 * a.outer_stride;
            az.src = a.src + (size_t)z0 * a.src_outer_stride;
            az.mid = a.mid + (((size_t)z0 * a.ncomp) << t.log_n);
            hipError_t e;
            switch (t.log_n)
            {
            case 13:
                e = launch_inv<5>(az, nz, stream);
                break;
            case 14:
                e = launch_inv<6>(az, nz, stream);
                break;
            case 15:
                e = launch_inv<7>(az, nz, stream);
                break;
            case 16:
                e = launch_inv<8>(az, nz, stream);
                break;
            default:
                return hipErrorInvalidValue;
            }
            if (e != hipSuccess)
                return e;
        }
        return hipSuccess;
    }

    hipError_t ks_fused(const NttTables &t, const KsFusedArgs &k, hipStream_t stream)
    {
        Ks1Args a1;
        a1.t = k.t;
        a1.mid = k.mid;
        a1.targets = k.targets1;
        a1.ntargets = k.ntargets;
        a1.K = k.K;
        a1.batch = k.batch;
        a1.skip_diag = k.target_ntt != nullptr || k.fold_x != nullptr;
        a1.j0 = k.j0;
        a1.j1 = k.j1;
        a1.parts = k.parts ? k.parts : 1;
        a1.tb = t;
        if (k.fold_c0 && (a1.parts > 1 || !k.fold_pm || k.j0 != 0 || k.j1 != k.K))
            return hipErrorInvalidValue;
        if (k.fold_x && (k.fold_c0 || !k.fold_y || !k.fold_plane || !k.fold_pm || a1.parts > 1 || k.j0 != 0 || k.j1 != k.K))
            return hipErrorInvalidValue;
        Ks2Args a2;
        a2.mid = k.mid;
        a2.target = k.target_ntt;
        a2.key = k.key;
        a2.key_digit_words = (size_t)key_digit_units(t, k.L) << t.log_n;
        a2.acc = k.acc;
        a2.targets = k.targets2;
        a2.ntargets = k.ntargets;
        a2.K = k.K;
        a2.L = k.L;
        a2.batch = k.batch;
        a2.j0 = k.j0;
        a2.j1 = k.j1;
        a2.key_digit0 = k.key_digit0;
        a2.parts = a1.parts;
        a2.fold_c0 = k.fold_c0;
        a2.fold_c1 = k.fold_c1;
        a2.fold_pm = k.fold_pm;
        a2.fold_x = k.fold_x;
        a2.fold_y = k.fold_y;
        a2.fold_plane = k.fold_plane;
        a2.gal = k.galois_elt;
        if (k.galois_elt && (!(k.galois_elt & 1) || !k.target_ntt || !k.fold_c0 || k.fold_c1 || k.fold_x))
            return hipErrorInvalidValue;
        a2.tb = t;
        switch (t.log_n)
        {
        case 13:
            return launch_ks<5>(a1, a2, k.batch, k.n_int, stream, k.order1, k.no_class_fork);
        case 14:
            return launch_ks<6>(a1, a2, k.batch, k.n_int, stream, k.order1, k.no_class_fork);
        case 15:
            return launch_ks<7>(a1, a2, k.batch, k.n_int, stream, k.order1, k.no_class_fork);
        case 16:
            return launch_ks<8>(a1, a2, k.batch, k.n_int, stream, k.order1, k.no_class_fork);
        default:
            return hipErrorInvalidValue;
        }
    }

    hipError_t key_to_register_order(const NttTables &t, const uint64_t *in, uint64_t *out, unsigned L, size_t digits, hipStream_t stream)
    {
        if (L > kMaxKeyComps)
            return hipErrorInvalidValue;
        const size_t polys = 2 * digits;
        size_t total = (polys * L) << t.log_n;
        size_t blocks = (total + kThreads - 1) / kThreads;
        if (blocks > 4096)
            blocks = 4096;
        hipLaunchKernelGGL(key_layout_kernel, dim3((unsigned)blocks), dim3(kThreads), 0, stream, in, out, t.fpd, t.mods, L, (unsigned)t.log_n, polys);
        return hipGetLastError();
    }
    hipError_t key_from_register_order(const NttTables &t, const uint64_t *in, uint64_t *out, unsigned L, size_t digits, hipStream_t stream)
    {
        if (L > kMaxKeyComps)
            return hipErrorInvalidValue;
        const size_t polys = 2 * digits;
        size_t total = (polys * L) << t.log_n;
        size_t blocks = (total + kThreads - 1) / kThreads;
        if (blocks > 4096)
            blocks = 4096;
        hipLaunchKernelGGL(key_unlayout_kernel, dim3((unsigned)blocks), dim3(kThreads), 0, stream, in, out, t.fpd, L, (unsigned)t.log_n, polys);
        return hipGetLastError();
    }
}
```

seal_amd/csrc/ntt_kernels.h:

```cpp
#pragma once
#include "field.h"

namespace sealhip
{
    struct NttTables
    {
        const ModDesc *mods;
        const ShoupOp *fwd;
        const ShoupOp *inv;
        const ShoupOp *ninv;
        const FpDesc *fpd;
        const double *fwd_d;
        const double *inv_d;
        const double *ninv_d;
        const unsigned char *fp_host;
        int log_n;
    };

    struct NttTail2
    {
        const uint64_t *src2_0, *src2_1;
        size_t src2_stride;
        uint64_t src2_half, src2_q;
        const uint64_t *src2_fix;
        const ShoupOp *pmul;
        const uint64_t *c0, *c1;
        size_t c_stride;
        int halves_added;
        int a_has_c = 0;
    };

    struct NttBatch
    {
        uint64_t *data;
        size_t outer_stride;
        unsigned ncomp;
        unsigned nouter;
        const uint32_t *comp_prime;
        unsigned prime_first;
        const uint64_t *src;
        size_t src_outer_stride;
        unsigned src_ncomp;
        int src_mode;
        uint64_t src_half;
        uint64_t src_q;
        const uint64_t *src_fix;
        int epi;
        const uint64_t *epi_a;
        size_t epi_a_stride;
        const ShoupOp *epi_mul;
        uint64_t *epi_out0, *epi_out1;
        size_t epi_out_stride;
        const NttTail2 *tail2 = nullptr;
        uint64_t out_add = 0;
        const uint64_t *prod_x = nullptr, *prod_y = nullptr;
        unsigned prod_batch = 0;
        unsigned prod_outer0 = 0;
        uint64_t *prod_out = nullptr;
        size_t prod_out_stride = 0;
        uint32_t src_galois_elt = 0;
        int cls_hint = -1;
    };

    hipError_t ntt_forward(const NttTables &t, const NttBatch &b, int out_lazy, hipStream_t stream);
    hipError_t ntt_inverse(const NttTables &t, const NttBatch &b, int out_lazy, hipStream_t stream);
}
```

seal_amd/csrc/ntt_kernels.hip:

```cpp
#include "ntt_kernels.h"
#include "ntt2_kernels.h"
#include "pool.h"

namespace sealhip
{
    namespace
    {
        struct PassArgs
        {
            uint64_t *data;
            const uint64_t *src;
            size_t outer_stride;
            size_t src_outer_stride;
            unsigned src_ncomp;
            uint64_t src_half;
            uint64_t src_q;
            const uint64_t *src_fix;
            const uint32_t *comp_prime;
            unsigned prime_first;
            const ModDesc *mods;
            const ShoupOp *tw;
            const ShoupOp *ninv;
            int log_n;
            int s0;
// ... 478 lines not shown

        template <int D, int R, bool LAST, bool INV>
        hipError_t launch_pass(PassArgs a, unsigned ncomp, unsigned nouter, hipStream_t stream)
        {
            constexpr int TPS_LOG = D - R > 0 ? D - R : 0;
            const int n = a.log_n;
            const int c = n - a.s0 - D;
            int avail_log = LAST ? a.s0 : c;
            int log_wd = 8 - TPS_LOG;
            if (log_wd < 0)
                log_wd = 0;
            if (log_wd > avail_log)
                log_wd = avail_log;
            a.log_wd = log_wd;
            unsigned threads = 1u << (TPS_LOG + log_wd);
            unsigned tiles = LAST ? (1u << (a.s0 - log_wd)) : (1u << (a.s0 + c - log_wd));
            size_t shmem = lds_words<D, R, LAST>(log_wd) * sizeof(uint64_t);
            dim3 grid(tiles, ncomp, nouter);
            if (INV)
                hipLaunchKernelGGL((ntt_inv_pass<D, R, LAST>), grid, dim3(threads), shmem, stream, a);
            else
                hipLaunchKernelGGL((ntt_fwd_pass<D, R, LAST>), grid, dim3(threads), shmem, stream, a);
            return hipGetLastError();
        }

        template <bool LAST, bool INV>
        hipError_t dispatch_pass(int D, const PassArgs &a, unsigned ncomp, unsigned nouter, hipStream_t stream)
        {
            switch (D)
            {
            case 6:
                return launch_pass<6, 3, LAST, INV>(a, ncomp, nouter, stream);
            case 7:
                return launch_pass<7, 4, LAST, INV>(a, ncomp, nouter, stream);
            case 8:
                return launch_pass<8, 4, LAST, INV>(a, ncomp, nouter, stream);
            case 9:
                return launch_pass<9, 3, LAST, INV>(a, ncomp, nouter, stream);
            case 10:
                return launch_pass<10, 5, LAST, INV>(a, ncomp, nouter, stream);
            case 11:
                return launch_pass<11, 4, LAST, INV>(a, ncomp, nouter, stream);
            case 12:
                return launch_pass<12, 4, LAST, INV>(a, ncomp, nouter, stream);
            case 13:
                return launch_pass<13, 4, LAST, INV>(a, ncomp, nouter, stream);
            default:
                return hipErrorInvalidValue;
            }
        }

        hipError_t run(const NttTables &t, const NttBatch &b, int out_lazy, bool inverse, hipStream_t stream)
        {
            if (b.ncomp == 0 || b.nouter == 0)
                return hipSuccess;
            PassArgs a;
            a.data = b.data;
            a.src = inverse ? nullptr : b.src;
            a.outer_stride = b.outer_stride;
            a.src_outer_stride = b.src_outer_stride;
            a.src_ncomp = b.src_ncomp ? b.src_ncomp : 1;
            a.src_half = b.src_half;
            a.src_q = b.src_q;
            a.src_fix = b.src_fix;
            a.comp_prime = b.comp_prime;
            a.prime_first = b.prime_first;
            a.mods = t.mods;
            a.tw = inverse ? t.inv : t.fwd;
            a.ninv = t.ninv;
            a.log_n = t.log_n;
            a.s0 = 0;
            a.log_wd = 0;
            const int lazy = out_lazy ? F_LAZY : 0;
            const int srcflag = !a.src ? 0 : (b.src_mode == 2 ? F_ROUND_SRC : (b.src_mode == 1 ? F_REDUCE_SRC : 0));
            const Plan plan = make_plan(t.log_n);
            const unsigned zmax = 65535;
            for (unsigned z0 = 0; z0 < b.nouter; z0 += zmax)
            {
                unsigned nz = b.nouter - z0 < zmax ? b.nouter - z0 : zmax;
                PassArgs az = a;
                az.data = a.data + (size_t)z0 * a.outer_stride;
                if (az.src)
                    az.src = a.src + (size_t)z0 * a.src_outer_stride;
                hipError_t e = hipSuccess;
                if (plan.passes == 0)
                {
                    az.flags = lazy | F_FINAL | srcflag;
                    unsigned N = 1u << t.log_n;
                    unsigned threads = N / 2 < 64 ? 64 : N / 2;
                    hipLaunchKernelGGL(ntt_small, dim3(1, b.ncomp, nz), dim3(threads), N * sizeof(uint64_t), stream, az, inverse ? 1 : 0);
                    e = hipGetLastError();
                }
                else if (plan.passes == 1)
                {
                    az.flags = lazy | F_FINAL | srcflag;
                    az.s0 = 0;
                    e = inverse ? dispatch_pass<true, true>(plan.d_last, az, b.ncomp, nz, stream)
                                : dispatch_pass<true, false>(plan.d_last, az, b.ncomp, nz, stream);
                }
                else if (!inverse)
                {
                    az.flags = srcflag;
                    az.s0 = 0;
                    e = dispatch_pass<false, false>(plan.d_col, az, b.ncomp, nz, stream);
                    if (e != hipSuccess)
                        return e;
                    az.src = nullptr;
                    az.flags = lazy | F_FINAL;
                    az.s0 = plan.d_col;
                    e = dispatch_pass<true, false>(plan.d_last, az, b.ncomp, nz, stream);
                }
                else
                {
                    az.flags = 0;
                    az.s0 = plan.d_col;
                    e = dispatch_pass<true, true>(plan.d_last, az, b.ncomp, nz, stream);
                    if (e != hipSuccess)
                        return e;
                    az.flags = lazy | F_FINAL;
                    az.s0 = 0;
                    e = dispatch_pass<false, true>(plan.d_col, az, b.ncomp, nz, stream);
                }
                if (e != hipSuccess)
                    return e;
            }
            return hipSuccess;
        }
    }

    hipError_t ntt_forward(const NttTables &t, const NttBatch &b, int out_lazy, hipStream_t stream)
    {
        if ((b.epi || b.tail2) && !ntt2_supports(t.log_n))
            return hipErrorInvalidValue;
        if (ntt2_supports(t.log_n))
        {
            Scratch mid(((size_t)b.nouter * b.ncomp) << t.log_n);
            const size_t ring_words = ntt2_ring_words(t, b);
            if (ring_words)
            {
                Scratch ring(ring_words);
                return ntt2_forward(t, b, out_lazy, mid.p, stream, ring.p, ring_words);
            }
            return ntt2_forward(t, b, out_lazy, mid.p, stream);
        }
        return run(t, b, out_lazy, false, stream);
    }
    hipError_t ntt_inverse(const NttTables &t, const NttBatch &b, int out_lazy, hipStream_t stream)
    {
        if (ntt2_supports(t.log_n))
        {
            Scratch mid(((size_t)b.nouter * b.ncomp) << t.log_n);
            return ntt2_inverse(t, b, out_lazy, mid.p, stream);
        }
        if (b.src || b.out_add || b.prod_x)
            return hipErrorInvalidValue;
        return run(t, b, out_lazy, true, stream);
    }
}
```

Measured before the change: 10260.

## Fuse inverse-NTT pass B into keyswitch pass 1 and fold last-component fixup into INTT

Adds an optional path (SEALHIP_KS_FUSE_PB) where the target's inverse NTT stops after pass A and the digit-resident ks1 kernel performs pass B in registers, avoiding a separate pass over the target. Separately, the keyswitch last-component coefficient correction is folded into the inverse NTT output epilogue via out_sub/out_sub_mul/out_sub_fix, removing a standalone kernel and its memory traffic. Pass-1/pass-2 launches are split so the fused pass 1 can run before the class fork. Adds counters for fused/unfused pass-1 launches. The fused path is opt-in and adds strict validation that may reject configurations.

After: 10240. About the same (-0.2%).

```diff
diff --git a/include/sealhip.h b/include/sealhip.h
--- a/include/sealhip.h
+++ b/include/sealhip.h
@@ -371,6 +371,7 @@
 SHL_FUNC SealHip_TailStats(uint64_t *folded, uint64_t *plain, uint64_t *dropped);
 SHL_FUNC SealHip_ProductStats(uint64_t *fused, uint64_t *formed, uint64_t *dropped);
 SHL_FUNC SealHip_GaloisStats(uint64_t *gathered, uint64_t *permuted);
+SHL_FUNC SealHip_KsPass1Stats(uint64_t *fused, uint64_t *unfused);
 SHL_FUNC SealHip_XofStats(uint64_t *polynomials, uint64_t *replaced_words, uint64_t *host_walk_ns, uint64_t *total_ns);
 SHL_FUNC shl_device_count(int *count);
 SHL_FUNC shl_set_device(int device);
diff --git a/seal_amd/__init__.py b/seal_amd/__init__.py
--- a/seal_amd/__init__.py
+++ b/seal_amd/__init__.py
@@ -1,12 +1,12 @@
 from .api import (CoeffModulus, PlainModulus, EncryptionParameters, SEALContext, ContextData, Ciphertext, Plaintext, KSwitchKeys,
                   RelinKeys, GaloisKeys, Evaluator, SecretKey, PublicKey, KeyGenerator, Decryptor, Encryptor, BatchEncoder, CKKSEncoder, Graph, ItemMap, DeviceBuffer, HipTimer, ntt_forward, ntt_inverse,
-                  dyadic_product, apply_galois, rns_stage, device_synchronize, device_info, release_pool, pool_stats, tail_stats, product_stats, galois_stats, ks_chunk_stats, xof_stats, Stream, Comm, device_count, set_device,
+                  dyadic_product, apply_galois, rns_stage, device_synchronize, device_info, release_pool, pool_stats, tail_stats, product_stats, galois_stats, ks_chunk_stats, ks_pass1_stats, xof_stats, Stream, Comm, device_count, set_device,
                   set_staged_host_copies, install_abort_trace)
 from ._native import SealHipError, InvalidArgument, LogicError, OutOfRange, DeviceError, load
 
 __all__ = [
     "CoeffModulus", "PlainModulus", "EncryptionParameters", "SEALContext", "ContextData", "Ciphertext", "Plaintext", "KSwitchKeys",
     "RelinKeys", "GaloisKeys", "Evaluator", "SecretKey", "PublicKey", "KeyGenerator", "Decryptor", "Encryptor", "BatchEncoder", "CKKSEncoder", "Graph", "ItemMap", "DeviceBuffer", "HipTimer", "ntt_forward", "ntt_inverse",
-    "dyadic_product", "apply_galois", "rns_stage", "device_synchronize", "device_info", "release_pool", "pool_stats", "tail_stats", "product_stats", "galois_stats", "ks_chunk_stats", "xof_stats", "Stream", "Comm", "device_count", "set_device", "set_staged_host_copies", "install_abort_trace", "SealHipError",
+    "dyadic_product", "apply_galois", "rns_stage", "device_synchronize", "device_info", "release_pool", "pool_stats", "tail_stats", "product_stats", "galois_stats", "ks_chunk_stats", "ks_pass1_stats", "xof_stats", "Stream", "Comm", "device_count", "set_device", "set_staged_host_copies", "install_abort_trace", "SealHipError",
     "InvalidArgument", "LogicError", "OutOfRange", "DeviceError", "load",
 ]
diff --git a/seal_amd/_native.py b/seal_amd/_native.py
--- a/seal_amd/_native.py
+++ b/seal_amd/_native.py
@@ -93,7 +93,7 @@
 Evaluator_RelinearizeDigitParallel Evaluator_ApplyGaloisDigitParallel Evaluator_RotateVectorDigitParallel
 Evaluator_BroadcastKeyDigits Evaluator_SwitchKeySlots Evaluator_SwitchKeyPackTargets Evaluator_SwitchKeyFinishOwned
 Evaluator_SwitchKeyAddGathered
-SealHip_ReleasePool SealHip_PoolStats SealHip_TailStats SealHip_ProductStats SealHip_GaloisStats SealHip_XofStats SealHip_KsChunkStats SealHip_SetStagedHostCopies SealHip_InstallAbortTrace shl_stream_create shl_stream_destroy shl_device_count shl_set_device
+SealHip_ReleasePool SealHip_PoolStats SealHip_TailStats SealHip_ProductStats SealHip_GaloisStats SealHip_XofStats SealHip_KsChunkStats SealHip_KsPass1Stats SealHip_SetStagedHostCopies SealHip_InstallAbortTrace shl_stream_create shl_stream_destroy shl_device_count shl_set_device
 shl_ntt_forward shl_ntt_inverse shl_dyadic_product shl_apply_galois shl_rns_stage shl_malloc shl_free
 shl_memcpy_h2d shl_memcpy_d2h shl_device_synchronize shl_timer_create shl_timer_destroy shl_timer_start
 shl_timer_stop
diff --git a/seal_amd/api.py b/seal_amd/api.py
--- a/seal_amd/api.py
+++ b/seal_amd/api.py
@@ -1745,6 +1745,12 @@
     return a.value, b.value, c.value
 
 
+def ks_pass1_stats():
+    a, b = C.c_uint64(), C.c_uint64()
+    N.check(N.lib().SealHip_KsPass1Stats(C.byref(a), C.byref(b)))
+    return a.value, b.value
+
+
 def device_synchronize():
     N.check(N.lib().shl_device_synchronize())
 
diff --git a/seal_amd/csrc/capi_kernels.cpp b/seal_amd/csrc/capi_kernels.cpp
--- a/seal_amd/csrc/capi_kernels.cpp
+++ b/seal_amd/csrc/capi_kernels.cpp
@@ -356,6 +356,17 @@
             *permuted = p;
         SHL_CATCH
     }
+    SHL_FUNC SealHip_KsPass1Stats(uint64_t *fused, uint64_t *unfused)
+    {
+        SHL_TRY
+        uint64_t f, u;
+        ks_pass1_stats(f, u);
+        if (fused)
+            *fused = f;
+        if (unfused)
+            *unfused = u;
+        SHL_CATCH
+    }
     SHL_FUNC SealHip_TailStats(uint64_t *folded, uint64_t *plain, uint64_t *dropped)
     {
         SHL_TRY
diff --git a/seal_amd/csrc/evaluator.h b/seal_amd/csrc/evaluator.h
--- a/seal_amd/csrc/evaluator.h
+++ b/seal_amd/csrc/evaluator.h
@@ -48,6 +48,7 @@
         bool defer = false;
         KsPlan plan{ 0, 1 };
         unsigned j0 = 0, j1 = 0;
+        bool fuse_pb = false;
         bool takes_product() const { return fused && fold && split == 1; }
         bool reads_through_map() const;
     };
diff --git a/seal_amd/csrc/evaluator_common.h b/seal_amd/csrc/evaluator_common.h
--- a/seal_amd/csrc/evaluator_common.h
+++ b/seal_amd/csrc/evaluator_common.h
@@ -114,6 +114,8 @@
         static unsigned scratch_cap_mib();
         static bool lazy_product();
         static bool lazy_product_min_wgs(size_t &min_wgs);
+        static bool fuse_pb();
+        static int ks1_order();
     };
     const KsSwitches &ks_switches();
 
diff --git a/seal_amd/csrc/evaluator_keyswitch.cpp b/seal_amd/csrc/evaluator_keyswitch.cpp
--- a/seal_amd/csrc/evaluator_keyswitch.cpp
+++ b/seal_amd/csrc/evaluator_keyswitch.cpp
@@ -130,6 +130,16 @@
         const char *v = std::getenv("SEALHIP_LAZY_PRODUCT");
         return !(v && std::atoi(v) == 0);
     }
+    bool KsSwitches::fuse_pb()
+    {
+        const char *v = std::getenv("SEALHIP_KS_FUSE_PB");
+        return v && std::atoi(v) != 0;
+    }
+    int KsSwitches::ks1_order()
+    {
+        static const char *v = shl_ab_getenv("SEALHIP_KS1_ORDER");
+        return v && (v[0] == '0' || v[0] == '1') ? v[0] - '0' : -1;
+    }
     bool KsSwitches::lazy_product_min_wgs(size_t &min_wgs)
     {
         const char *v = std::getenv("SEALHIP_LAZY_PRODUCT_MIN_WGS");
@@ -171,6 +181,11 @@
             r.split = std::max(1u, std::min({ r.split, 8u, K }));
         }
         r.plan = ks_plan((unsigned)batch, (size_t)(K + 1) * K * context_.n(), (size_t)(K + 1) * (context_.n() >> 12), r.split == 1, !capturing_);
+        const Scheme sch = context_.scheme();
+        const int forced = KsSwitches::ks1_order();
+        const bool digit_resident = forced >= 0 ? forced == 1 : batch * (size_t)(j1 - j0) * (context_.n() >> 12) >= 4096;
+        r.fuse_pb = KsSwitches::fuse_pb() && !digit_parallel && r.split == 1 && j0 == 0 && j1 == K && digit_resident &&
+                    (sch == Scheme::ckks || sch == Scheme::bgv);
         return r;
     }
     bool KsRoute::reads_through_map() const { return takes_product() && !ks_switches().galois_kernels; }
@@ -377,9 +392,11 @@
             }
             return bt;
         };
-        if (ntt_target && !inverse_in_lane && ntt2_supports(context_.log_n()))
+        const bool fuse_pb = route.fuse_pb && route.fused && ntt_target && ntt2_inverse_two_pass(tb, inverse_batch(0, B));
+        const bool inverse_below = inverse_in_lane || fuse_pb;
+        if (ntt_target && !inverse_below && ntt2_supports(context_.log_n()))
             ck(ntt_inverse(tb, inverse_batch(0, B), 0, stream_), "ks intt target");
-        else if (!read_in_place && !inverse_in_lane)
+        else if (!read_in_place && !inverse_below)
         {
             ck(hipMemcpyAsync(t.p, target, (size_t)B * poly_words * 8, hipMemcpyDeviceToDevice, stream_), "ks copy target");
             if (ntt_target)
@@ -393,7 +410,21 @@
             if (ks_switches().trace)
                 std::fprintf(stderr, "[ks] split %u (K %u, digits %u..%u)\n", split, K, j0, j1);
             Scratch mid((size_t)plan.lanes * plan.chunk * ks_item_words);
-            Scratch inv_mid(inverse_in_lane ? (size_t)plan.lanes * plan.chunk * poly_words : 1);
+            Scratch inv_mid(inverse_in_lane || fuse_pb ? (size_t)plan.lanes * plan.chunk * poly_words : 1);
+            const auto inverse_into_lane = [&](unsigned b0, unsigned nb, unsigned lane, hipStream_t st) {
+                NttBatch bt = inverse_batch(b0, nb);
+                bt.stop_after_pass_a = fuse_pb;
+                ck(ntt2_inverse(tb, bt, 0, inv_mid.p + (size_t)lane * plan.chunk * poly_words, st), "ks intt target (chunk)");
+            };
+            const auto with_pb = [&](KsFusedArgs ka, unsigned b0, unsigned lane) {
+                if (fuse_pb)
+                {
+                    ka.pb_mid = inv_mid.p + (size_t)lane * plan.chunk * poly_words;
+                    ka.pb_t = t.p + b0 * poly_words;
+                    ka.order1 = 1;
+                }
+                return ka;
+            };
             {
                 uint64_t w = (uint64_t)plan.lanes * plan.chunk * ks_item_words, seen = g_ks_scratch_words_max.load();
                 while (w > seen && !g_ks_scratch_words_max.compare_exchange_weak(seen, w))
@@ -434,7 +465,11 @@
                 return ka;
             };
             if (!chunked)
-                ck(ks_fused(tb, fused_args(0, B, 0), stream_), "ks fused");
+            {
+                if (fuse_pb)
+                    inverse_into_lane(0, B, 0, stream_);
+                ck(ks_fused(tb, with_pb(fused_args(0, B, 0), 0, 0), stream_), "ks fused");
+            }
             else
             {
                 KsLanes *ln = ks_lanes();
@@ -471,9 +506,10 @@
                         const unsigned l = c % lanes;
                         hipStream_t st = l == 0 ? stream_ : ln->stream[l - 1];
                         if (inverse_in_lane)
-                            ck(ntt2_inverse(tb, inverse_batch(b0, nb), 0, inv_mid.p + (size_t)l * plan.chunk * poly_words, st), "ks intt target (chunk)");
+                            inverse_into_lane(b0, nb, l, st);
                         KsFusedArgs kc = fused_args(b0, nb, l);
                         kc.order1 = (size_t)B * (j1 - j0) * (N >> 12) >= 4096 ? 1 : 0;
+                        kc = with_pb(kc, b0, l);
                         kc.no_class_fork = lanes > 1 && !ks_switches().class_fork;
                         ck(ks_fused(tb, kc, st), "ks fused (chunk)");
                     }
@@ -687,10 +723,11 @@
         if (acc_has_addend)
         {
             NttBatch bw = plain_batch(acc_p + (size_t)(K - 1) * N, (size_t)(K + 1) * N, 1, 2 * B, K - 1);
-            ck(ntt_inverse(tb, bw, 0, stream_), "ks intt last component");
-            ck(k_ks_last_coeff(context_.dev_mods(), K - 1, klvl.dev.inv_q_last_mod_q + (K - 1), klvl.dev.round_fix + (K - 1),
-                               lvl.dev.half_q_last, acc_p, (unsigned)context_.log_n(), K, (size_t)2 * B, stream_),
-               "ks last component, coefficient form");
+            bw.out_sub = acc_p + (size_t)K * N;
+            bw.out_sub_mul = klvl.dev.inv_q_last_mod_q + (K - 1);
+            bw.out_sub_fix = klvl.dev.round_fix + (K - 1);
+            bw.out_add = lvl.dev.half_q_last;
+            ck(ntt_inverse(tb, bw, 0, stream_), "ks intt last component, coefficient form");
         }
         else
         {
diff --git a/seal_amd/csrc/ntt2_kernels.h b/seal_amd/csrc/ntt2_kernels.h
--- a/seal_amd/csrc/ntt2_kernels.h
+++ b/seal_amd/csrc/ntt2_kernels.h
@@ -25,6 +25,7 @@
     hipError_t ntt2_ring_launch(const NttTables &t, const NttRingRun &run, hipStream_t stream);
 
     hipError_t ntt2_inverse(const NttTables &t, const NttBatch &b, int out_lazy, uint64_t *mid, hipStream_t stream);
+    bool ntt2_inverse_two_pass(const NttTables &t, const NttBatch &b);
 
     struct KsFusedArgs
     {
@@ -45,8 +46,11 @@
         uint32_t galois_elt = 0;
         int order1 = -1;
         bool no_class_fork = false;
+        const uint64_t *pb_mid = nullptr;
+        uint64_t *pb_t = nullptr;
     };
     hipError_t ks_fused(const NttTables &t, const KsFusedArgs &k, hipStream_t stream);
+    void ks_pass1_stats(uint64_t &fused, uint64_t &unfused);
 
     inline unsigned key_comp_units(const NttTables &t, unsigned comp)
     {
diff --git a/seal_amd/csrc/ntt2_kernels.hip b/seal_amd/csrc/ntt2_kernels.hip
--- a/seal_amd/csrc/ntt2_kernels.hip
+++ b/seal_amd/csrc/ntt2_kernels.hip
@@ -564,11 +564,15 @@
             unsigned nouter;
             int lazy;
             uint64_t out_add;
+            const uint64_t *out_sub;
+            const ShoupOp *out_sub_mul;
+            const uint64_t *out_sub_fix;
             const uint64_t *prod_x, *prod_y;
             unsigned prod_batch, prod_outer0;
             uint64_t *prod_out;
             size_t prod_out_stride;
             uint32_t src_gal;
+            bool stop_after_pa;
             NttTables t;
         };
 
@@ -705,57 +709,85 @@
                 inv_pa_body<false, D1, 2>(a, prime, comp, outer, lds, blk.tile);
         }
 
+        __device__ __forceinline__ uint64_t inv_out_word(uint64_t v, const InvArgs &a, unsigned prime, const uint64_t *sub)
+        {
+            if (sub)
+            {
+                const ModDesc md = a.t.mods[prime];
+                const ShoupOp pm = *a.out_sub_mul;
+                const uint64_t s = barrett64(*sub, md) + *a.out_sub_fix;
+                v = sub_mod(v, mul_shoup(s, pm.w, pm.wq, md.q), md.q);
+            }
+            if (a.out_add)
+                v = csub(v + a.out_add, a.t.mods[prime].q);
+            return v;
+        }
+
         template <bool FP, int D1, int ICLS = 2>
-        __device__ __forceinline__ void inv_pb_body(const InvArgs &a, unsigned prime, unsigned comp, unsigned outer, uint64_t *lds, unsigned tile)
+        __device__ __forceinline__ void inv_pb_regs(typename Field<FP>::elem (&x)[16], const NttTables &tb, const typename Field<FP>::Mod &m, unsigned prime,
+                                                    const uint64_t *mid_poly, uint64_t *lds, unsigned cg)
         {
             typedef Field<FP> F;
             typedef Geo<D1> G;
             static_assert(G::rA >= 1, "the N^-1 stage is handled in phase A");
+            const unsigned tid = threadIdx.x;
+            const unsigned c = tid & (G::C - 1), hi = tid >> G::LC;
+            const typename F::tw_t *tab = tw_table<FP>(tb, true, prime);
+            const unsigned col = cg * G::C + c;
+            const uint64_t *i = mid_poly + ((size_t)(hi * 16 + (col >> 4)) << 8) + (col & 15);
+#pragma unroll
+            for (int rb = 0; rb < 16; rb++)
+                x[rb] = F::unraw(mid_ld<8>(i + rb * 16));
+            {
+                TwRegs<FP> tw;
+                load_tw<FP, 4>(tw, tab, [&](int t) { return (1u << (G::rA + t)) + (hi << t); });
+                phase_inv<FP, 4, 0, ICLS, kInvE2<ICLS>>(x, m, [&](int t, int g) { return tw.get((1 << t) + g); });
+            }
+#pragma unroll
+            for (int e = 0; e < 16; e++)
+                F::fix(x[e], m);
+#pragma unroll
+            for (int rb = 0; rb < 16; rb++)
+                lds[(hi * 16 + rb) * G::CP + c] = F::raw(x[rb]);
+            __syncthreads();
+#pragma unroll
+            for (int e = 0; e < 16; e++)
+            {
+                const unsigned ra = e >> (4 - G::rA), rbh = e & ((1 << (4 - G::rA)) - 1);
+                const unsigned R = ra * 16 + (rbh << G::rA) + hi;
+                x[e] = F::unraw(lds[R * G::CP + c]);
+            }
+            phase_inv<FP, G::rA, 1, ICLS, kInvE3<ICLS>>(x, m, [&](int t, int g) { return ld_uniform(tab, (1u << t) + g); });
+            {
+                typename F::tw_t ni, nw;
+                if constexpr (FP)
+                {
+                    ni = ld_uniform(tb.ninv_d, 2 * prime);
+                    nw = ld_uniform(tb.ninv_d, 2 * prime + 1);
+                }
+                else
+                {
+                    ni = ld_uniform(tb.ninv, 2 * prime);
+                    nw = ld_uniform(tb.ninv, 2 * prime + 1);
+                }
+                inv_last_stage<FP, G::rA, ICLS, kInvE3<ICLS>>(x, m, ni, nw);
+            }
+        }
+
+        template <bool FP, int D1, int ICLS = 2>
+        __device__ __forceinline__ void inv_pb_body(const InvArgs &a, unsigned prime, unsigned comp, unsigned outer, uint64_t *lds, unsigned tile)
+        {
+            typedef Field<FP> F;
+            typedef Geo<D1> G;
             const unsigned tid = threadIdx.x, cg = tile;
             const unsigned c = tid & (G::C - 1), hi = tid >> G::LC;
             const typename F::Mod m = F::make_mod(ld_uniform_mod(&a.t.mods[prime]), ld_uniform_fpd(&a.t.fpd[prime]));
-            const typename F::tw_t *tab = tw_table<FP>(a.t, true, prime);
             const unsigned col = cg * G::C + c;
-            const uint64_t *i = a.mid + (((size_t)outer * a.ncomp + comp) << G::n) + ((size_t)(hi * 16 + (col >> 4)) << 8) + (col & 15);
             typename F::elem x[16];
-#pragma unroll
-            for (int rb = 0; rb < 16; rb++)
-                x[rb] = F::unraw(mid_ld<8>(i + rb * 16));
-            {
-                TwRegs<FP> tw;
-                load_tw<FP, 4>(tw, tab, [&](int t) { return (1u << (G::rA + t)) + (hi << t); });
-                phase_inv<FP, 4, 0, ICLS, kInvE2<ICLS>>(x, m, [&](int t, int g) { return tw.get((1 << t) + g); });
-            }
-#pragma unroll
-            for (int e = 0; e < 16; e++)
-                F::fix(x[e], m);
-#pragma unroll
-            for (int rb = 0; rb < 16; rb++)
-                lds[(hi * 16 + rb) * G::CP + c] = F::raw(x[rb]);
-            __syncthreads();
-#pragma unroll
-            for (int e = 0; e < 16; e++)
-            {
-                const unsigned ra = e >> (4 - G::rA), rbh = e & ((1 << (4 - G::rA)) - 1);
-                const unsigned R = ra * 16 + (rbh << G::rA) + hi;
-                x[e] = F::unraw(lds[R * G::CP + c]);
-            }
-            phase_inv<FP, G::rA, 1, ICLS, kInvE3<ICLS>>(x, m, [&](int t, int g) { return ld_uniform(tab, (1u << t) + g); });
-            {
-                typename F::tw_t ni, nw;
-                if constexpr (FP)
-                {
-                    ni = ld_uniform(a.t.ninv_d, 2 * prime);
-                    nw = ld_uniform(a.t.ninv_d, 2 * prime + 1);
-                }
-                else
-                {
-                    ni = ld_uniform(a.t.ninv, 2 * prime);
-                    nw = ld_uniform(a.t.ninv, 2 * prime + 1);
-                }
-                inv_last_stage<FP, G::rA, ICLS, kInvE3<ICLS>>(x, m, ni, nw);
-            }
-            uint64_t *o = a.data + (size_t)outer * a.outer_stride + ((size_t)comp << G::n);
+            inv_pb_regs<FP, D1, ICLS>(x, a.t, m, prime, a.mid + (((size_t)outer * a.ncomp + comp) << G::n), lds, cg);
+            const size_t poly = (size_t)outer * a.outer_stride + ((size_t)comp << G::n);
+            uint64_t *o = a.data + poly;
+            const uint64_t *sub = a.out_sub ? a.out_sub + poly : nullptr;
 #pragma unroll
             for (int e = 0; e < 16; e++)
             {
@@ -763,8 +795,7 @@
                 const unsigned ra = e >> (4 - G::rA), rbh = e & ((1 << (4 - G::rA)) - 1);
                 const unsigned R = ra * 16 + (rbh << G::rA) + hi;
                 uint64_t v = a.lazy ? F::inv_to_lazy(x[e], m) : F::inv_to_canon(x[e], m);
-                if (a.out_add)
-                    v = csub(v + a.out_add, a.t.mods[prime].q);
+                v = inv_out_word(v, a, prime, sub ? sub + (size_t)R * 256 + col : nullptr);
                 mid_st<16>(o + (size_t)R * 256 + col, v);
             }
         }
@@ -1073,6 +1104,7 @@
                 phase_inv<FP, G::rA, 1, ICLS, kInvE3<ICLS>>(x, m, [&](int t, int g) { return ld_uniform(tab, (1u << t) + g); });
                 inv_last_stage<FP, G::rA, ICLS, kInvE3<ICLS>>(x, m, ni, nw);
                 uint64_t *o = a.data + (size_t)outer * a.outer_stride + comp_off;
+                const uint64_t *sub = a.out_sub ? a.out_sub + (size_t)outer * a.outer_stride + comp_off : nullptr;
 #pragma unroll
                 for (int e = 0; e < 16; e++)
                 {
@@ -1080,8 +1112,7 @@
                     const unsigned ra = e >> (4 - G::rA), rbh = e & ((1 << (4 - G::rA)) - 1);
                     const unsigned R = ra * 16 + (rbh << G::rA) + hi;
                     uint64_t v = a.lazy ? F::inv_to_lazy(x[e], m) : F::inv_to_canon(x[e], m);
-                    if (a.out_add)
-                        v = csub(v + a.out_add, a.t.mods[prime].q);
+                    v = inv_out_word(v, a, prime, sub ? sub + (size_t)R * 256 + col : nullptr);
                     o[(size_t)R * 256 + col] = v;
                 }
             }
@@ -1119,6 +1150,8 @@
             unsigned j0, j1;
             unsigned parts;
             int skip_diag;
+            const uint64_t *pb_mid;
+            uint64_t *pb_t;
             NttTables tb;
         };
 
@@ -1236,10 +1269,11 @@
                 with_int_class(a.tb, prime, [&](auto ic) { ks1_body<FP, D1, decltype(ic)::value>(a, lds, I, prime, b, cg, j0, j1); });
         }
 
-        template <bool FP, int D1, bool SMALL = false>
+        template <bool FP, int D1, bool SMALL = false, bool PB = false>
         __global__ void __launch_bounds__(kThreads, 2) ks1t_kernel(Ks1Args a)
         {
             static_assert(FP || !SMALL, "SMALL is a property of the double-precision launch");
+            static_assert(SMALL || !PB, "the prologue is built for the double-precision digits");
             typedef Field<FP> F;
             typedef Geo<D1> G;
             HIP_DYNAMIC_SHARED(uint64_t, lds)
@@ -1251,14 +1285,35 @@
             const unsigned cg = grp % G::TILES, bj = grp / G::TILES;
             const unsigned J = a.j0 + bj % ndig, b = bj / ndig;
             const unsigned c = tid & (G::C - 1), rbl = tid >> G::LC;
-            const uint64_t *in = a.t + (((size_t)b * a.K + J) << G::n) + cg * G::C + c;
+            const size_t tile0 = (((size_t)b * a.K + J) << G::n) + cg * G::C + c;
             uint64_t raw[16];
-#pragma unroll
-            for (int e = 0; e < 16; e++)
-            {
-                const unsigned ra = e >> (4 - G::rA), rbh = e & ((1 << (4 - G::rA)) - 1);
-                const unsigned R = ra * 16 + (rbh << G::rA) + rbl;
-                raw[e] = in[(size_t)R * 256];
+            if constexpr (PB)
+            {
+                const unsigned Ju = SHL_UNIFORM(J);
+                const typename F::Mod mj = F::make_mod(ld_uniform_mod(&a.tb.mods[Ju]), ld_uniform_fpd(&a.tb.fpd[Ju]));
+                typename F::elem x[16];
+                inv_pb_regs<true, D1>(x, a.tb, mj, Ju, a.pb_mid + (((size_t)b * a.K + J) << G::n), lds, cg);
+                uint64_t *out = a.pb_t + tile0;
+#pragma unroll
+                for (int e = 0; e < 16; e++)
+                {
+                    F::fix(x[e], mj);
+                    const unsigned ra = e >> (4 - G::rA), rbh = e & ((1 << (4 - G::rA)) - 1);
+                    const unsigned R = ra * 16 + (rbh << G::rA) + rbl;
+                    raw[e] = F::inv_to_canon(x[e], mj);
+                    mid_st<16>(out + (size_t)R * 256, raw[e]);
+                }
+            }
+            else
+            {
+                const uint64_t *in = a.t + tile0;
+#pragma unroll
+                for (int e = 0; e < 16; e++)
+                {
+                    const unsigned ra = e >> (4 - G::rA), rbh = e & ((1 << (4 - G::rA)) - 1);
+                    const unsigned R = ra * 16 + (rbh << G::rA) + rbl;
+                    raw[e] = in[(size_t)R * 256];
+                }
             }
             const uint64_t src_q = a.tb.mods[J].q;
             const bool as_doubles = SMALL || (FP && !(src_q >> 52));
@@ -2197,6 +2252,8 @@
                 hipError_t e = hipGetLastError();
                 if (e != hipSuccess)
                     return e;
+                if (a.stop_after_pa && r.cls == 1)
+                    return (hipError_t)hipSuccess;
                 static const char *skip_env = shl_ab_getenv("SEALHIP_AB_SKIP_INV_PB");
                 static long skip_after = skip_env ? std::atol(skip_env) : -1;
                 static std::atomic<long> inv_launches{ 0 };
@@ -2212,6 +2269,8 @@
             }, !(fused && fused_int()) || (D1 == 6 && SEALHIP_FUSED_FORK14));
         }
 
+        std::atomic<uint64_t> g_ks1_fused{ 0 }, g_ks1_unfused{ 0 };
+
         template <int D1>
         hipError_t launch_ks(const Ks1Args &a1, const Ks2Args &a2, unsigned batch, unsigned n_int, hipStream_t s, int order1, bool no_class_fork)
         {
@@ -2244,7 +2303,8 @@
                     raised = true;
                 }
             }
-            auto run_class = [&](bool fp, hipStream_t st) -> hipError_t {
+            const bool fuse_pb = a1.pb_mid != nullptr;
+            auto run_pass1 = [&](bool fp, hipStream_t st) -> hipError_t {
                 const unsigned t0 = fp ? n_int : 0, nt = fp ? n_fp : n_int;
                 if (!nt)
                     return hipSuccess;
@@ -2255,6 +2315,8 @@
                 static const char *order_env = shl_ab_getenv("SEALHIP_KS1_ORDER");
                 const unsigned g1t = batch * (a1.j1 - a1.j0) * G::TILES;
                 const bool digit_resident = order_env ? order_env[0] == '1' : order1 >= 0 ? (order1 == 1 && a1.parts == 1) : (a1.parts == 1 && g1t >= 4096);
+                if (fuse_pb && !digit_resident)
+                    return hipErrorInvalidValue;
                 if (digit_resident && fp)
                 {
                     const unsigned char *small = a1.tb.fp_host;
@@ -2268,22 +2330,30 @@
                         cr.j0 = ja;
                         cr.j1 = jb;
                         const dim3 gr(batch * (jb - ja) * G::TILES);
-                        if (sm)
+                        if (sm && fuse_pb)
+                            hipLaunchKernelGGL((ks1t_kernel<true, D1, true, true>), gr, dim3(kThreads), l1, st, cr);
+                        else if (sm)
                             hipLaunchKernelGGL((ks1t_kernel<true, D1, true>), gr, dim3(kThreads), l1, st, cr);
                         else
                             hipLaunchKernelGGL((ks1t_kernel<true, D1, false>), gr, dim3(kThreads), l1, st, cr);
+                        (sm && fuse_pb ? g_ks1_fused : g_ks1_unfused)++;
                         ja = jb;
                     }
-                }
-                else if (digit_resident)
+                    return hipGetLastError();
+                }
+                if (digit_resident)
                     hipLaunchKernelGGL((ks1t_kernel<false, D1>), dim3(g1t), dim3(kThreads), l1, st, c1);
                 else if (fp)
                     hipLaunchKernelGGL((ks1_kernel<true, D1>), g1, dim3(kThreads), l1, st, c1);
                 else
                     hipLaunchKernelGGL((ks1_kernel<false, D1>), g1, dim3(kThreads), l1, st, c1);
-                hipError_t e = hipGetLastError();
-                if (e != hipSuccess)
-                    return e;
+                g_ks1_unfused++;
+                return hipGetLastError();
+            };
+            auto run_pass2 = [&](bool fp, hipStream_t st) -> hipError_t {
+                const unsigned t0 = fp ? n_int : 0, nt = fp ? n_fp : n_int;
+                if (!nt)
+                    return hipSuccess;
                 Ks2Args c2 = a2;
                 c2.targets = a2.targets + 4 * t0;
                 c2.ntargets = nt;
@@ -2297,25 +2367,38 @@
             SideStream &ss = side_stream();
             static const bool fork_ok = !shl_ab_getenv("SEALHIP_KS_NOFORK");
             hipError_t e;
+            if (fuse_pb && (e = run_pass1(true, s)) != hipSuccess)
+                return e;
             if (n_int && n_fp && ss.ok && fork_ok && !no_class_fork)
             {
                 if ((e = hipEventRecord(ss.fork, s)) != hipSuccess || (e = hipStreamWaitEvent(ss.stream, ss.fork, 0)) != hipSuccess)
                     return e;
-                if ((e = run_class(false, ss.stream)) != hipSuccess || (e = hipEventRecord(ss.join, ss.stream)) != hipSuccess)
+                if ((e = run_pass1(false, ss.stream)) != hipSuccess || (e = run_pass2(false, ss.stream)) != hipSuccess ||
+                    (e = hipEventRecord(ss.join, ss.stream)) != hipSuccess)
                     return e;
-                if ((e = run_class(true, s)) != hipSuccess)
+                if ((!fuse_pb && (e = run_pass1(true, s)) != hipSuccess) || (e = run_pass2(true, s)) != hipSuccess)
                     return e;
                 return hipStreamWaitEvent(s, ss.join, 0);
             }
-            if ((e = run_class(false, s)) != hipSuccess)
+            if ((e = run_pass1(false, s)) != hipSuccess || (e = run_pass2(false, s)) != hipSuccess)
                 return e;
-            return run_class(true, s);
+            if (!fuse_pb && (e = run_pass1(true, s)) != hipSuccess)
+                return e;
+            return run_pass2(true, s);
         }
     }
 
     bool ntt2_supports(int log_n)
     {
         return log_n >= 13 && log_n <= 16;
+    }
+
+    bool ntt2_inverse_two_pass(const NttTables &t, const NttBatch &b)
+    {
+        if (t.log_n == 15 || t.log_n == 16)
+            return true;
+        static const bool fused_ok = !shl_ab_getenv("SEALHIP_NTT_NOFUSED");
+        return (t.log_n == 13 || t.log_n == 14) && (!fused_ok || b.prod_x || b.src_galois_elt);
     }
 
     size_t ntt2_ring_words(const NttTables &t, const NttBatch &b)
@@ -2422,6 +2505,11 @@
         if (b.out_add && out_lazy)
             return hipErrorInvalidValue;
         a.out_add = b.out_add;
+        if (b.out_sub && (out_lazy || b.ncomp != 1 || !b.out_sub_mul || !b.out_sub_fix || b.stop_after_pass_a))
+            return hipErrorInvalidValue;
+        a.out_sub = b.out_sub;
+        a.out_sub_mul = b.out_sub_mul;
+        a.out_sub_fix = b.out_sub_fix;
         a.prod_x = b.prod_x;
         a.prod_y = b.prod_y;
         a.prod_batch = b.prod_batch;
@@ -2429,6 +2517,9 @@
         a.prod_out = b.prod_out;
         a.prod_out_stride = b.prod_out_stride;
         a.src_gal = b.src_galois_elt;
+        a.stop_after_pa = b.stop_after_pass_a;
+        if (b.stop_after_pass_a && (!ntt2_inverse_two_pass(t, b) || out_lazy || b.out_add || b.comp_prime))
+            return hipErrorInvalidValue;
         if (b.src_galois_elt && (!b.src || b.prod_x || !(b.src_galois_elt & 1)))
             return hipErrorInvalidValue;
         if (b.prod_x && (!b.prod_y || !b.prod_batch || (size_t)b.nouter + b.prod_outer0 > (size_t)3 * b.prod_batch || !b.src_outer_stride))
@@ -2475,6 +2566,12 @@
         return hipSuccess;
     }
 
+    void ks_pass1_stats(uint64_t &fused, uint64_t &unfused)
+    {
+        fused = g_ks1_fused.load();
+        unfused = g_ks1_unfused.load();
+    }
+
     hipError_t ks_fused(const NttTables &t, const KsFusedArgs &k, hipStream_t stream)
     {
         Ks1Args a1;
@@ -2488,6 +2585,10 @@
         a1.j0 = k.j0;
         a1.j1 = k.j1;
         a1.parts = k.parts ? k.parts : 1;
+        a1.pb_mid = k.pb_mid;
+        a1.pb_t = k.pb_t;
+        if (k.pb_mid && (k.pb_t != k.t || a1.parts > 1 || k.j0 != 0 || k.j1 != k.K || k.order1 != 1))
+            return hipErrorInvalidValue;
         a1.tb = t;
         if (k.fold_c0 && (a1.parts > 1 || !k.fold_pm || k.j0 != 0 || k.j1 != k.K))
             return hipErrorInvalidValue;
diff --git a/seal_amd/csrc/ntt_kernels.h b/seal_amd/csrc/ntt_kernels.h
--- a/seal_amd/csrc/ntt_kernels.h
+++ b/seal_amd/csrc/ntt_kernels.h
@@ -53,6 +53,9 @@
         size_t epi_out_stride;
         const NttTail2 *tail2 = nullptr;
         uint64_t out_add = 0;
+        const uint64_t *out_sub = nullptr;
+        const ShoupOp *out_sub_mul = nullptr;
+        const uint64_t *out_sub_fix = nullptr;
         const uint64_t *prod_x = nullptr, *prod_y = nullptr;
         unsigned prod_batch = 0;
         unsigned prod_outer0 = 0;
@@ -60,6 +63,7 @@
         size_t prod_out_stride = 0;
         uint32_t src_galois_elt = 0;
         int cls_hint = -1;
+        bool stop_after_pass_a = false;
     };
 
     hipError_t ntt_forward(const NttTables &t, const NttBatch &b, int out_lazy, hipStream_t stream);
diff --git a/seal_amd/csrc/ntt_kernels.hip b/seal_amd/csrc/ntt_kernels.hip
--- a/seal_amd/csrc/ntt_kernels.hip
+++ b/seal_amd/csrc/ntt_kernels.hip
@@ -654,7 +654,7 @@
             Scratch mid(((size_t)b.nouter * b.ncomp) << t.log_n);
             return ntt2_inverse(t, b, out_lazy, mid.p, stream);
         }
-        if (b.src || b.out_add || b.prod_x)
+        if (b.src || b.out_add || b.out_sub || b.prod_x)
             return hipErrorInvalidValue;
         return run(t, b, out_lazy, true, stream);
     }
```
